# PoseLib/PoseLib

Measured on AMD Instinct MI355X. Metric: scored RANSAC hypotheses/sec (P3P@5k corrs, 5pt@5k corrs), higher is better.
Workload: dtype f64; 1 GPU; p3p_5000; correspondences=5000, problems_in_flight_per_gpu=128, distinct_scenes=64

## Files before the change

### __graft_entry__.py

```python
import os
import subprocess
import sys

ROOT = os.path.dirname(os.path.abspath(__file__))
sys.path.insert(0, ROOT)
sys.path.insert(0, os.path.join(ROOT, "tests"))


def build() -> None:
    import poselib_amd

    poselib_amd.build()
    assert os.path.exists(poselib_amd.LIB_PATH)
    subprocess.check_call(["make", "-C", os.path.join(ROOT, "oracle"), "-s", "liboracle.so"])
    subprocess.check_call(["make", "-C", os.path.join(ROOT, "tests", "hostmath"), "-s", "libhostmath.so"])
    subprocess.check_call(["make", "-C", os.path.join(ROOT, "tests", "hostmath_trig"), "-s", "libhostmath_trig.so"])
    subprocess.check_call(["make", "-C", os.path.join(ROOT, "tests", "hostmath_tangent"), "-s", "libhostmath_tangent.so"])
    subprocess.check_call(["make", "-C", os.path.join(ROOT, "tests", "hostmath_radial1d"), "-s", "libhostmath_radial1d.so"])
    if os.path.isdir("/root/reference/PoseLib"):
        subprocess.check_call(["make", "-C", os.path.join(ROOT, "oracle"), "-s", "-j8", "-f", "Makefile.ref"])
        subprocess.check_call(["make", "-C", os.path.join(ROOT, "oracle"), "-s", "-j8", "-f", "Makefile.ref", "VARIANT=fma"])
        import ref_lib

        subprocess.check_call(["make", "-C", os.path.join(ROOT, "oracle"), "-s", "-f", "Makefile.integration",
                               f"REF={ref_lib.REFERENCE_ROOT}"])
    from poselib_amd import _lib

    lib = _lib.lib()
    for sym in _lib.EXPORTED_SYMBOLS:
        getattr(lib, sym)


def smoke() -> None:
    import numpy as np

    import oracle_lib as O
    import poselib_amd as P
    from poselib_amd import synth

    d = synth.absolute_pose_scene(1500, 0.5, 4242)
    opt = {"ransac": {"seed": 3}}
    img, info = P.estimate_absolute_pose(d["p2d"], d["p3d"], d["camera"], opt)
    pose, mask, st = O.estimate_absolute_pose(d["p2d"], d["p3d"], d["camera"], opt)
    assert info["iterations"] == st["iterations"], (info["iterations"], st["iterations"])
    assert info["num_inliers"] == st["num_inliers"], (info["num_inliers"], st["num_inliers"])
    assert (np.array(info["inliers"]) == mask).all()
    got = np.r_[img.pose.q, img.pose.t]
    assert np.abs(got - pose).max() < 1e-6, np.abs(got - pose).max()
    print("smoke ok: iterations", info["iterations"], "inliers", info["num_inliers"], "max |pose diff|",
          float(np.abs(got - pose).max()))


if __name__ == "__main__":
    build()
    if len(sys.argv) > 1 and sys.argv[1] == "smoke":
        smoke()
```

### include/poselib_amd.h

```cpp
#ifndef POSELIB_AMD_H_
#define POSELIB_AMD_H_
#include <stddef.h>
#include <stdint.h>

#ifdef __cplusplus
extern "C" {
#endif

#define PL_OK 0
#define PL_ERR_NO_DEVICE (-1)
#define PL_ERR_HIP (-2)
#define PL_ERR_INVALID (-3)
#define PL_ERR_UNSUPPORTED (-4)
#define PL_ERR_COMM (-5)

typedef struct {
    uint64_t max_iterations;
    uint64_t min_iterations;
    double dyn_num_trials_mult;
    double success_prob;
    uint64_t seed;
    int32_t progressive_sampling;
    int32_t score_initial_model;
    uint64_t max_prosac_iterations;
// ... 82 lines not shown
                                  const pl_camera *camera1, const pl_camera *camera2, const pl_robust_options *opt,
                                  pl_camera_pose *pose, uint8_t *inliers, pl_ransac_stats *stats);
int pl_estimate_fundamental_dev(const pl_device_points *points2D_1, const pl_device_points *points2D_2, size_t n,
                                const pl_robust_options *opt, double *F , uint8_t *inliers,
                                pl_ransac_stats *stats);
int pl_estimate_homography_dev(const pl_device_points *points2D_1, const pl_device_points *points2D_2, size_t n,
                               const pl_robust_options *opt, double *H , uint8_t *inliers,
                               pl_ransac_stats *stats);
int pl_debug_check_device_points(const pl_device_points *d, size_t n, int cols);
int pl_debug_point_stats_dev(const pl_device_points *x1, const pl_device_points *x2, size_t n, int centroid, double *out);

int pl_undistort_points(const pl_camera *camera, const double *points2D, size_t n, double *out);

typedef struct {
    int32_t kind;
    int32_t status;
    const double *a;
    const double *b;
    size_t n;
    const pl_robust_options *opt;
    pl_camera *camera1;
    const pl_camera *camera2;
    void *model;
    uint8_t *inliers;
    pl_ransac_stats *stats;
} pl_batch_item;
int pl_estimate_batch(pl_batch_item *items, size_t count, int max_in_flight);
int pl_estimate_batch_devices(pl_batch_item *items, size_t count, const int *devices, int num_devices, int max_in_flight);
typedef struct {
    int32_t kind;
    int32_t status;
    pl_device_points a;
    pl_device_points b;
    size_t n;
    const pl_robust_options *opt;
    pl_camera *camera1;
    const pl_camera *camera2;
    void *model;
    uint8_t *inliers;
    pl_ransac_stats *stats;
} pl_batch_item_dev;
int pl_estimate_batch_dev(pl_batch_item_dev *items, size_t count, int max_in_flight);
int pl_debug_point_stats_group_dev(const pl_device_points *x1, const pl_device_points *x2, const size_t *n, size_t count, int centroid,
                                   double *out);
typedef struct {
    uint64_t items;
    uint64_t grouped;
    uint64_t focal_grouped;
    uint64_t solo;
    uint64_t fallback;
} pl_batch_report;
void pl_last_batch_report(pl_batch_report *out);

int pl_ransac_pnp(const double *x, const double *X, size_t n, const pl_robust_options *opt, pl_camera_pose *pose,
                  uint8_t *inliers, pl_ransac_stats *stats);
int pl_ransac_pnpf(const double *x, const double *X, size_t n, const pl_robust_options *opt, pl_camera_pose *pose, double *focal,
                   uint8_t *inliers, pl_ransac_stats *stats);
int pl_ransac_relpose(const double *x1, const double *x2, size_t n, const pl_robust_options *opt, pl_camera_pose *pose,
                      uint8_t *inliers, pl_ransac_stats *stats);
int pl_ransac_shared_focal_relpose(const double *x1, const double *x2, size_t n, const pl_robust_options *opt, pl_camera_pose *pose,
                                   double *focal, uint8_t *inliers, pl_ransac_stats *stats);
int pl_refine_shared_focal_relpose(const double *x1, const double *x2, size_t n, const pl_bundle_options *opt, pl_camera_pose *pose,
                                   double *focal, uint32_t *lm_iterations);

int pl_ransac_fundamental(const double *x1, const double *x2, size_t n, const pl_robust_options *opt, double *F,
                          uint8_t *inliers, pl_ransac_stats *stats);
int pl_ransac_homography(const double *x1, const double *x2, size_t n, const pl_robust_options *opt, double *H,
                         uint8_t *inliers, pl_ransac_stats *stats);
int pl_estimate_1D_radial_absolute_pose(const double *points2D, const double *points3D, size_t n, const pl_robust_options *opt,
                                        pl_camera_pose *pose, uint8_t *inliers, pl_ransac_stats *stats);
int pl_ransac_1D_radial_pnp(const double *x, const double *X, size_t n, const pl_robust_options *opt, pl_camera_pose *pose,
                            uint8_t *inliers, pl_ransac_stats *stats);

typedef struct pl_problem pl_problem;
int pl_problem_create(int kind, const double *a, const double *b, size_t n, pl_problem **out);
int pl_problem_create_tangent(const double *x1, const double *x2, size_t n, const pl_camera *camera1, const pl_camera *camera2,
                              pl_problem **out);
int pl_problem_create_dev(int kind, const pl_device_points *a, const pl_device_points *b, size_t n, pl_problem **out);
int pl_problem_create_tangent_dev(const pl_device_points *x1, const pl_device_points *x2, size_t n, const pl_camera *camera1,
                                  const pl_camera *camera2, pl_problem **out);
void pl_problem_destroy(pl_problem *p);
int pl_ransac_run(pl_problem *p, const pl_robust_options *opt, void *model, uint8_t *inliers, pl_ransac_stats *stats);

typedef struct {
    pl_problem *problem;
    const pl_robust_options *opt;
    void *model;
    uint8_t *inliers;
    pl_ransac_stats *stats;
    int32_t status;
    int32_t reserved;
} pl_ransac_item;
int pl_ransac_batch(pl_ransac_item *items, size_t count, int max_in_flight, int group_size);

typedef int (*pl_allgather_fn)(void *user, const void *send, void *recv, size_t bytes);
typedef struct pl_shard {
    int32_t rank, world;
    pl_allgather_fn allgather;
    void *user;
} pl_shard;
int pl_ransac_run_sharded(pl_problem *p, const pl_robust_options *opt, const pl_shard *shard, void *model,
                          uint8_t *inliers, pl_ransac_stats *stats);

int pl_score_model(pl_problem *p, const void *model, double max_error, uint64_t *inlier_count, double *score);
int pl_debug_inlier_mask(pl_problem *p, const void *model, double max_error, uint8_t *mask);
int pl_debug_tangent_chunk(void);
int pl_debug_radial1d_chunk(void);
int pl_debug_group_slices(int kind, uint32_t n_points, uint32_t iterations, uint32_t launch_chunks);
int pl_debug_radial1d_generate(pl_problem *p, const uint32_t *samples, size_t num_iters, uint32_t slots_per_iter, double *models,
                               uint32_t *num_models, uint32_t *totals);
int pl_debug_generate(pl_problem *p, const uint32_t *samples, uint64_t seed, uint64_t pos_base, const uint32_t *positions, size_t num_iters,
                      uint32_t slots_per_iter, int real_focal_check, int route, double *models, uint32_t *num_models, uint32_t *nan_bits,
                      uint32_t *blk_tot, uint32_t *blk_nan, uint32_t *flags);
int pl_debug_score_stream(pl_problem *p, const void *models, size_t n, double max_error, uint32_t *counts,
                          double *scores, int32_t *path_used);
int pl_debug_score_shape(int kind, uint32_t n_points, int matrix_core, int group_form, uint32_t *chunks,
                         uint32_t *points_per_lane);
typedef struct pl_debug_score_member {
    pl_problem *problem;
    const void *models;
    size_t n;
    double max_error;
    uint32_t *counts;
    double *scores;
    uint32_t slices;
    uint32_t slices_used;
    uint32_t chunks;
    int32_t path_used;
} pl_debug_score_member;
int pl_debug_score_stream_ex(int route, pl_debug_score_member *members, size_t num_members, uint32_t *idle_changed);
typedef struct pl_debug_prune_member {
    pl_problem *problem;
    const void *models;
    size_t n;
    double max_error;
    double init_min;
    uint32_t init_max;
    uint32_t cand_cap;
    uint32_t *counts;
    double *scores;
    uint8_t *kept;
    uint32_t *cand;
    uint32_t num_cand;
    uint32_t cstar, chunks, chunk_points;
    uint32_t lead;
    uint32_t lead_max;
    uint32_t num_live, num_selected;
    uint32_t slices, num_preselected;
    double lead_min;
} pl_debug_prune_member;
int pl_debug_score_pruned(int route, pl_debug_prune_member *members, size_t num_members, uint32_t *idle_changed);
int pl_debug_score_survivors(int route, pl_debug_prune_member *members, size_t num_members, uint32_t *const *survivors,
                             uint32_t *idle_changed, uint32_t *guard_changed);
int pl_debug_score_prune_gate(int kind, uint32_t n_points, uint32_t iterations);
typedef struct pl_debug_sampler_shape_info {
    uint64_t window;
    uint32_t build, tile;
    uint32_t small_flags, small_doubling, small_segments;
    uint32_t large_flags, large_doubling, large_segments;
} pl_debug_sampler_shape_info;
int pl_debug_sampler_shape(int K, uint64_t N, uint32_t B, uint64_t window, pl_debug_sampler_shape_info *out);
typedef struct pl_debug_sampler_member {
    uint64_t seed, pos_base, N;
    uint32_t B, M;
    const uint8_t *planted;
    uint32_t *positions;
    uint8_t *delta;
    uint64_t *flagbits;
    uint64_t pos_after;
    uint32_t orbit_error, M_used, build_used;
    int32_t delta_guard, ctl_clear, pad;
} pl_debug_sampler_member;
int pl_debug_sample_positions(int route, int K, int build, pl_debug_sampler_member *members, size_t num_members, uint32_t *idle_changed);
int pl_debug_device_math(int fn, const double *x, size_t n, double *out);
int pl_debug_device_math2(int fn, const double *x, const double *y, size_t n, double *out);
int pl_refine_model(pl_problem *p, const pl_bundle_options *opt, const pl_camera *camera, const uint8_t *mask,
                    void *model, uint32_t *lm_iterations);

int pl_bundle_adjust_camera(pl_problem *p, const pl_bundle_options *opt, pl_camera *camera, const uint8_t *mask,
                            pl_camera_pose *pose, uint32_t *lm_iterations);

int pl_p3p(const double *x , const double *X , pl_camera_pose *out );
int pl_p5lp_radial(const double *x , const double *X , pl_camera_pose *out , int *count );
int pl_relpose_5pt(const double *x1 , const double *x2 , pl_camera_pose *out );
int pl_essential_matrix_5pt(const double *x1, const double *x2, double *E );
int pl_relpose_7pt(const double *x1 , const double *x2 , double *F );
int pl_homography_4pt(const double *x1 , const double *x2 , double *H );
int pl_p35pf(const double *x, const double *X, pl_camera_pose *out, double *focals);
int pl_relpose_6pt_shared_focal(const double *x1, const double *x2, pl_camera_pose *out, double *focals);
int pl_solve_focal_batch(int kind, const double *in, size_t count, double *out_models, uint32_t *out_counts);
int pl_solve_batch(int kind, const double *in, size_t count, double *out_models, uint32_t *out_counts);

#ifdef __cplusplus
}
#endif
#endif
```

### poselib_amd/__init__.py

```python
from ._lib import LIB_PATH, PoseLibAmdError, build
from .api import (
    KIND_ABS, KIND_FUND, KIND_HOM, KIND_REL, KIND_RAD1D, estimate_1D_radial_absolute_pose, ransac_1D_radial_pnp, p5lp_radial, radial1d_generate, debug_generate, score_shape, score_stream_group, Batch, RansacBatch, ransac_batch, device_math, device_math2, BundleOptions, Camera, CameraPose, Image, Problem, TangentProblem, inlier_mask, RansacOptions,
    device_count, essential_matrix_5pt, estimate_absolute_pose, estimate_batch, last_batch_report, estimate_fundamental, estimate_homography,
    estimate_relative_pose, homography_4pt, p3p, p5p, ransac_fundamental, ransac_homography, ransac_pnp, ransac_pnpf,
    ransac_relpose, ransac_shared_focal_relpose, estimate_shared_focal_relative_pose, refine_shared_focal_relpose, ImagePair, p35pf, relpose_6pt_shared_focal, solve_focal_batch, relpose_5pt, relpose_7pt, set_device, set_lm_mode, solve_batch, undistort_points,
    check_device_points, point_stats_dev, point_stats_group_dev, score_pruned, score_survivors, score_prune_gate, sampler_shape, sample_positions,
)

__version__ = "0.1.0"
```

### poselib_amd/_lib.py

```python
from __future__ import annotations

import ctypes as C
import os
import subprocess

_PKG = os.path.dirname(os.path.abspath(__file__))
_CSRC = os.path.join(_PKG, "csrc")
LIB_PATH = os.path.join(_PKG, "lib", "libposelib_amd.so")
if os.environ.get("POSELIB_AMD_LIB"):
    LIB_PATH = os.environ["POSELIB_AMD_LIB"]

u64, i32, u32, f64 = C.c_uint64, C.c_int32, C.c_uint32, C.c_double

PL_OK, PL_ERR_NO_DEVICE, PL_ERR_HIP, PL_ERR_INVALID, PL_ERR_UNSUPPORTED, PL_ERR_COMM = 0, -1, -2, -3, -4, -5


class RansacOptions(C.Structure):
    _fields_ = [("max_iterations", u64), ("min_iterations", u64), ("dyn_num_trials_mult", f64), ("success_prob", f64),
                ("seed", u64), ("progressive_sampling", i32), ("score_initial_model", i32),
                ("max_prosac_iterations", u64)]


class BundleOptions(C.Structure):
    _fields_ = [("max_iterations", u64), ("loss_type", i32), ("lambda_update", i32), ("damping", i32), ("verbose", i32),
# ... 33 lines not shown

class BatchReport(C.Structure):
    _fields_ = [("items", C.c_uint64), ("grouped", C.c_uint64), ("focal_grouped", C.c_uint64), ("solo", C.c_uint64),
                ("fallback", C.c_uint64)]


class RansacItem(C.Structure):
    _fields_ = [("problem", C.c_void_p), ("opt", C.POINTER(RobustOptions)), ("model", C.c_void_p), ("inliers", C.c_void_p),
                ("stats", C.POINTER(RansacStats)), ("status", i32), ("reserved", i32)]


ALLGATHER_FN = C.CFUNCTYPE(C.c_int, C.c_void_p, C.c_void_p, C.c_void_p, C.c_size_t)


class Shard(C.Structure):
    _fields_ = [("rank", i32), ("world", i32), ("allgather", ALLGATHER_FN), ("user", C.c_void_p)]


class DebugScoreMember(C.Structure):
    _fields_ = [("problem", C.c_void_p), ("models", C.c_void_p), ("n", C.c_size_t), ("max_error", f64), ("counts", C.c_void_p),
                ("scores", C.c_void_p), ("slices", u32), ("slices_used", u32), ("chunks", u32), ("path_used", i32)]


class DebugPruneMember(C.Structure):
    _fields_ = [("problem", C.c_void_p), ("models", C.c_void_p), ("n", C.c_size_t), ("max_error", f64), ("init_min", f64),
                ("init_max", u32), ("cand_cap", u32), ("counts", C.c_void_p), ("scores", C.c_void_p), ("kept", C.c_void_p),
                ("cand", C.c_void_p), ("num_cand", u32), ("cstar", u32), ("chunks", u32), ("chunk_points", u32), ("lead", u32),
                ("lead_max", u32), ("num_live", u32), ("num_selected", u32), ("slices", u32), ("num_preselected", u32), ("lead_min", f64)]


class DebugSamplerShape(C.Structure):
    _fields_ = [("window", u64), ("build", u32), ("tile", u32), ("small_flags", u32), ("small_doubling", u32), ("small_segments", u32),
                ("large_flags", u32), ("large_doubling", u32), ("large_segments", u32)]


class DebugSamplerMember(C.Structure):
    _fields_ = [("seed", u64), ("pos_base", u64), ("N", u64), ("B", u32), ("M", u32), ("planted", C.c_void_p), ("positions", C.c_void_p),
                ("delta", C.c_void_p), ("flagbits", C.c_void_p), ("pos_after", u64), ("orbit_error", u32), ("M_used", u32),
                ("build_used", u32), ("delta_guard", i32), ("ctl_clear", i32), ("pad", i32)]


PL_F64, PL_F32 = 0, 1


class DevicePoints(C.Structure):
    _fields_ = [("data", C.c_void_p), ("row_stride", C.c_int64), ("dtype", i32), ("cols", i32)]


class BatchItemDev(C.Structure):
    _fields_ = [("kind", i32), ("status", i32), ("a", DevicePoints), ("b", DevicePoints), ("n", C.c_size_t),
                ("opt", C.POINTER(RobustOptions)), ("camera1", C.POINTER(Camera)), ("camera2", C.POINTER(Camera)),
                ("model", C.c_void_p), ("inliers", C.c_void_p), ("stats", C.POINTER(RansacStats))]


class PoseLibAmdError(RuntimeError):
    pass


def build(force: bool = False, verbose: bool = False) -> str:
    srcs = [os.path.join(_CSRC, f) for f in os.listdir(_CSRC) if f.endswith((".h", ".hip", ".cc", ".inc", "Makefile"))]
    srcs.append(os.path.join(os.path.dirname(_PKG), "include", "poselib_amd.h"))
    stale = (not os.path.exists(LIB_PATH)) or any(os.path.getmtime(s) > os.path.getmtime(LIB_PATH) for s in srcs)
    if force or stale:
        cmd = ["make", "-C", _CSRC]
        if not verbose:
            cmd.append("-s")
        subprocess.check_call(cmd)
    return LIB_PATH


_lib = None


def lib():
    global _lib
    if _lib is None:
        if not os.path.exists(LIB_PATH):
            raise PoseLibAmdError(
                f"{LIB_PATH} is missing: build it with `python -c 'import poselib_amd; poselib_amd.build()'` "
                "(there is no CPU fallback)")
        if not os.environ.get("POSELIB_AMD_KEEP_ENV"):
            os.environ.setdefault("GPU_MAX_HW_QUEUES", "16")
        L = C.CDLL(LIB_PATH)
        _declare(L)
        _lib = L
    return _lib


def _declare(L):
    vp, sz, dbl, cint = C.c_void_p, C.c_size_t, C.c_double, C.c_int
    P = C.POINTER
    opt, stats, cam, pose = P(RobustOptions), P(RansacStats), P(Camera), P(CameraPose)
    dpts = P(DevicePoints)
    sig = {
        "pl_default_ransac_options": (None, [P(RansacOptions)]),
        "pl_default_bundle_options": (None, [P(BundleOptions)]),
        "pl_default_robust_options": (None, [opt, cint]),
        "pl_device_count": (cint, []),
        "pl_set_lm_mode": (cint, [cint]),
        "pl_set_device": (cint, [cint]),
        "pl_last_error": (C.c_char_p, []),
        "pl_version": (C.c_char_p, []),
        "pl_abi_version": (cint, []),
        "pl_estimate_absolute_pose": (cint, [vp, vp, sz, opt, cam, pose, vp, stats]),
        "pl_estimate_relative_pose": (cint, [vp, vp, sz, cam, cam, opt, pose, vp, stats]),
        "pl_estimate_fundamental": (cint, [vp, vp, sz, opt, vp, vp, stats]),
        "pl_estimate_homography": (cint, [vp, vp, sz, opt, vp, vp, stats]),
        "pl_estimate_absolute_pose_dev": (cint, [dpts, dpts, sz, opt, cam, pose, vp, stats]),
        "pl_estimate_relative_pose_dev": (cint, [dpts, dpts, sz, cam, cam, opt, pose, vp, stats]),
        "pl_estimate_fundamental_dev": (cint, [dpts, dpts, sz, opt, vp, vp, stats]),
        "pl_estimate_homography_dev": (cint, [dpts, dpts, sz, opt, vp, vp, stats]),
        "pl_problem_create_dev": (cint, [cint, dpts, dpts, sz, P(vp)]),
        "pl_problem_create_tangent_dev": (cint, [dpts, dpts, sz, cam, cam, P(vp)]),
        "pl_debug_check_device_points": (cint, [dpts, sz, cint]),
        "pl_debug_point_stats_dev": (cint, [dpts, dpts, sz, cint, vp]),
        "pl_estimate_batch": (cint, [P(BatchItem), sz, cint]),
        "pl_estimate_batch_devices": (cint, [P(BatchItem), sz, P(C.c_int), cint, cint]),
        "pl_estimate_batch_dev": (cint, [P(BatchItemDev), sz, cint]),
        "pl_debug_point_stats_group_dev": (cint, [dpts, dpts, P(sz), sz, cint, vp]),
        "pl_last_batch_report": (None, [P(BatchReport)]),
        "pl_ransac_batch": (cint, [P(RansacItem), sz, cint, cint]),
        "pl_undistort_points": (cint, [cam, vp, sz, vp]),
        "pl_ransac_pnp": (cint, [vp, vp, sz, opt, pose, vp, stats]),
        "pl_ransac_pnpf": (cint, [vp, vp, sz, opt, pose, P(dbl), vp, stats]),
        "pl_ransac_relpose": (cint, [vp, vp, sz, opt, pose, vp, stats]),
        "pl_ransac_shared_focal_relpose": (cint, [vp, vp, sz, opt, pose, P(dbl), vp, stats]),
        "pl_solve_focal_batch": (cint, [cint, vp, sz, vp, vp]),
        "pl_p35pf": (cint, [vp, vp, vp, vp]),
        "pl_relpose_6pt_shared_focal": (cint, [vp, vp, vp, vp]),
        "pl_refine_shared_focal_relpose": (cint, [vp, vp, sz, P(BundleOptions), pose, P(dbl), P(C.c_uint32)]),
        "pl_estimate_shared_focal_relative_pose": (cint, [vp, vp, sz, vp, opt, pose, P(dbl), vp, stats]),
        "pl_ransac_fundamental": (cint, [vp, vp, sz, opt, vp, vp, stats]),
        "pl_ransac_homography": (cint, [vp, vp, sz, opt, vp, vp, stats]),
        "pl_problem_create": (cint, [cint, vp, vp, sz, P(vp)]),
        "pl_problem_create_tangent": (cint, [vp, vp, sz, cam, cam, P(vp)]),
        "pl_debug_inlier_mask": (cint, [vp, vp, dbl, vp]),
        "pl_debug_tangent_chunk": (cint, []),
        "pl_debug_radial1d_chunk": (cint, []),
        "pl_debug_group_slices": (cint, [cint, C.c_uint32, C.c_uint32, C.c_uint32]),
        "pl_debug_radial1d_generate": (cint, [vp, vp, sz, C.c_uint32, vp, vp, vp]),
        "pl_debug_generate": (cint, [vp, vp, u64, u64, vp, sz, C.c_uint32, cint, cint, vp, vp, vp, vp, vp, vp]),
        "pl_estimate_1D_radial_absolute_pose": (cint, [vp, vp, sz, opt, pose, vp, stats]),
        "pl_ransac_1D_radial_pnp": (cint, [vp, vp, sz, opt, pose, vp, stats]),
        "pl_p5lp_radial": (cint, [vp, vp, P(CameraPose), P(cint)]),
        "pl_problem_destroy": (None, [vp]),
        "pl_ransac_run": (cint, [vp, opt, vp, vp, stats]),
        "pl_ransac_run_sharded": (cint, [vp, opt, P(Shard), vp, vp, stats]),
        "pl_score_model": (cint, [vp, vp, dbl, P(C.c_uint64), P(dbl)]),
        "pl_debug_score_stream": (cint, [vp, vp, sz, dbl, vp, vp, P(C.c_int32)]),
        "pl_debug_score_shape": (cint, [cint, C.c_uint32, cint, cint, P(C.c_uint32), P(C.c_uint32)]),
        "pl_debug_score_stream_ex": (cint, [cint, P(DebugScoreMember), sz, P(C.c_uint32)]),
        "pl_debug_score_pruned": (cint, [cint, P(DebugPruneMember), sz, P(C.c_uint32)]),
        "pl_debug_score_survivors": (cint, [cint, P(DebugPruneMember), sz, P(C.c_void_p), P(C.c_uint32), P(C.c_uint32)]),
        "pl_debug_score_prune_gate": (cint, [cint, C.c_uint32, C.c_uint32]),
        "pl_debug_sampler_shape": (cint, [cint, u64, C.c_uint32, u64, P(DebugSamplerShape)]),
        "pl_debug_sample_positions": (cint, [cint, cint, cint, P(DebugSamplerMember), sz, P(C.c_uint32)]),
        "pl_debug_device_math": (cint, [cint, vp, sz, vp]),
        "pl_debug_device_math2": (cint, [cint, vp, vp, sz, vp]),
        "pl_refine_model": (cint, [vp, P(BundleOptions), cam, vp, vp, P(C.c_uint32)]),
        "pl_bundle_adjust_camera": (cint, [vp, P(BundleOptions), cam, vp, P(CameraPose), P(C.c_uint32)]),
        "pl_p3p": (cint, [vp, vp, P(CameraPose)]),
        "pl_relpose_5pt": (cint, [vp, vp, P(CameraPose)]),
        "pl_essential_matrix_5pt": (cint, [vp, vp, vp]),
        "pl_relpose_7pt": (cint, [vp, vp, vp]),
        "pl_homography_4pt": (cint, [vp, vp, vp]),
        "pl_solve_batch": (cint, [cint, vp, sz, vp, vp]),
    }
    missing = [name for name in EXPORTED_SYMBOLS if name not in sig]
    assert not missing, f"no signature declared for {missing}"
    for name, (res, args) in sig.items():
        fn = getattr(L, name)
        fn.restype = res
        fn.argtypes = args
    if L.pl_abi_version() != ABI_VERSION:
        raise PoseLibAmdError(f"{LIB_PATH} has record layout version {L.pl_abi_version()}, this binding was written for {ABI_VERSION}: rebuild")


def check(rc: int):
    if rc < 0:
        msg = lib().pl_last_error().decode()
        raise PoseLibAmdError(f"poselib_amd error {rc}: {msg}")
    return rc


ABI_VERSION = 5
EXPORTED_SYMBOLS = [
    "pl_default_ransac_options", "pl_default_bundle_options", "pl_default_robust_options", "pl_device_count",
    "pl_set_device", "pl_last_error", "pl_version", "pl_estimate_absolute_pose", "pl_estimate_relative_pose",
    "pl_estimate_fundamental", "pl_estimate_homography", "pl_ransac_pnp", "pl_ransac_relpose", "pl_ransac_fundamental",
    "pl_ransac_homography", "pl_problem_create", "pl_problem_destroy", "pl_ransac_run", "pl_ransac_run_sharded", "pl_score_model", "pl_debug_score_stream", "pl_refine_model", "pl_bundle_adjust_camera", "pl_p3p", "pl_relpose_5pt",
    "pl_essential_matrix_5pt", "pl_relpose_7pt", "pl_homography_4pt", "pl_solve_batch", "pl_estimate_batch", "pl_estimate_batch_devices", "pl_last_batch_report", "pl_undistort_points",
    "pl_ransac_batch", "pl_debug_device_math", "pl_debug_device_math2", "pl_ransac_pnpf", "pl_ransac_shared_focal_relpose", "pl_refine_shared_focal_relpose",
    "pl_estimate_shared_focal_relative_pose", "pl_solve_focal_batch", "pl_p35pf", "pl_relpose_6pt_shared_focal", "pl_set_lm_mode",
    "pl_abi_version", "pl_problem_create_tangent", "pl_debug_inlier_mask", "pl_debug_tangent_chunk",
    "pl_p5lp_radial", "pl_debug_radial1d_chunk", "pl_debug_radial1d_generate", "pl_debug_group_slices", "pl_debug_generate",
    "pl_debug_score_shape", "pl_debug_score_stream_ex", "pl_debug_score_pruned", "pl_debug_score_survivors", "pl_debug_score_prune_gate",
    "pl_estimate_absolute_pose_dev", "pl_estimate_relative_pose_dev", "pl_estimate_fundamental_dev", "pl_estimate_homography_dev",
    "pl_problem_create_dev", "pl_problem_create_tangent_dev", "pl_debug_check_device_points", "pl_debug_point_stats_dev",
    "pl_debug_sampler_shape", "pl_debug_sample_positions", "pl_estimate_batch_dev", "pl_debug_point_stats_group_dev",
]
```

### poselib_amd/api.py

```python
from __future__ import annotations

import ctypes as C
import sys
import threading

import numpy as np

from . import _lib as L

LAMBDA_UPDATES = {"NIELSEN": 0, "FIXED_FACTOR": 1}
DAMPINGS = {"LEVENBERG": 0, "MARQUARDT": 1}
LOSS_TYPES = {"TRIVIAL": 0, "TRUNCATED": 1, "HUBER": 2, "CAUCHY": 3, "TRUNCATED_CAUCHY": 4, "TRUNCATED_LE_ZACH": 5}
CAMERA_MODEL_IDS = {"NULL": -1, "SIMPLE_PINHOLE": 0, "PINHOLE": 1, "SIMPLE_RADIAL": 2, "RADIAL": 3, "OPENCV": 4,
                    "OPENCV_FISHEYE": 5, "SIMPLE_RADIAL_FISHEYE": 8, "RADIAL_FISHEYE": 9}
_CAMERA_NAMES = {v: k for k, v in CAMERA_MODEL_IDS.items()}
KIND_ABS, KIND_REL, KIND_FUND, KIND_HOM = 0, 1, 2, 3
KIND_SHARED_FOCAL = 4
KIND_RAD1D = 5
_POSE_KINDS = (KIND_ABS, KIND_REL, KIND_RAD1D)


class CameraPose:

    def __init__(self, q=None, t=None):
# ... 462 lines not shown

    def results(self, first=None):
        out = []
        for pr, o, model, inl, st in (self.keep if first is None else self.keep[:first]):
            if pr.kind in _POSE_KINDS:
                out.append((_pypose(model), _info(st, inl[: pr.n])))
            else:
                out.append((model.reshape(3, 3).T.copy(), _info(st, inl[: pr.n])))
        return out


def device_math(fn: int, x):
    x = np.ascontiguousarray(x, dtype=np.float64)
    out = np.zeros_like(x)
    L.check(L.lib().pl_debug_device_math(int(fn), _ptr(x), C.c_size_t(x.size), _ptr(out)))
    return out


def device_math2(fn: int, x, y=None):
    x = np.ascontiguousarray(x, dtype=np.float64)
    if y is not None:
        y = np.ascontiguousarray(y, dtype=np.float64)
        if y.shape != x.shape:
            raise ValueError("x and y differ in shape")
    out = np.zeros_like(x)
    L.check(L.lib().pl_debug_device_math2(int(fn), _ptr(x), None if y is None else _ptr(y), C.c_size_t(x.size), _ptr(out)))
    return out


def group_slices(kind: int, n_points: int, iterations: int, launch_chunks: int) -> int:
    return L.check(L.lib().pl_debug_group_slices(int(kind), int(n_points), int(iterations), int(launch_chunks)))


def score_shape(kind: int, n_points: int, matrix_core: bool, group_form: bool):
    chunks, per_lane = C.c_uint32(0), C.c_uint32(0)
    rc = L.lib().pl_debug_score_shape(int(kind), int(n_points), int(bool(matrix_core)), int(bool(group_form)), C.byref(chunks),
                                      C.byref(per_lane))
    if rc == L.PL_ERR_UNSUPPORTED:
        return None
    L.check(rc)
    return chunks.value, per_lane.value


def score_stream_group(members):
    arr = (L.DebugScoreMember * max(len(members), 1))()
    keep = []
    for i, (problem, models, max_error, slices) in enumerate(members):
        n, flat = problem._flat_models(models)
        cnt = np.zeros(max(n, 1), dtype=np.uint32)
        sc = np.zeros(max(n, 1), dtype=np.float64)
        keep.append((n, flat, cnt, sc))
        arr[i] = L.DebugScoreMember(problem._h, _ptr(flat), n, float(max_error), _ptr(cnt), _ptr(sc), int(slices), 0, 0, 0)
    idle = C.c_uint32(0)
    L.check(L.lib().pl_debug_score_stream_ex(2, arr, C.c_size_t(len(members)), C.byref(idle)))
    out = [{"counts": cnt[:n], "scores": sc[:n], "path": arr[i].path_used, "slices": arr[i].slices_used, "chunks": arr[i].chunks}
           for i, (n, _, cnt, sc) in enumerate(keep)]
    return out, idle.value


def sampler_shape(K: int, N: int, B: int, window: int = 0):
    s = L.DebugSamplerShape()
    L.check(L.lib().pl_debug_sampler_shape(int(K), int(N), int(B), int(window), C.byref(s)))
    return {"window": int(s.window), "build": "small" if s.build == 1 else "large", "tile": int(s.tile),
            "small": {"flags": s.small_flags, "doubling": s.small_doubling, "segments": s.small_segments},
            "large": {"flags": s.large_flags, "doubling": s.large_doubling, "segments": s.large_segments}}


_SAMPLER_BUILDS = {None: 0, "small": 1, "large": 2}


def sample_positions(K: int, members, build=None, group: bool = False):
    arr = (L.DebugSamplerMember * max(len(members), 1))()
    keep = []
    for i, m in enumerate(members):
        planted = m.get("planted")
        if planted is not None:
            planted = np.ascontiguousarray(planted, dtype=np.uint8)
            M = int(planted.size)
            if m.get("M", 0) not in (0, M):
                raise ValueError("a planted table has M bytes")
        else:
            M = int(m.get("M", 0)) or sampler_shape(K, m["N"], m["B"])["window"]
        pos = np.zeros(max(int(m["B"]), 1), dtype=np.uint32)
        cap = M if M < (1 << 31) else 0
        delta = np.zeros(cap + 1, dtype=np.uint8)
        bits = np.zeros(cap // 64 + 2, dtype=np.uint64)
        keep.append((planted, pos, delta, bits))
        arr[i] = L.DebugSamplerMember(int(m.get("seed", 0)), int(m.get("pos_base", 0)), int(m["N"]), int(m["B"]), M,
                                      None if planted is None else _ptr(planted), _ptr(pos), _ptr(delta), _ptr(bits))
    idle = C.c_uint32(0)
    L.check(L.lib().pl_debug_sample_positions(2 if group else 0, int(K), _SAMPLER_BUILDS[build], arr, C.c_size_t(len(members)),
                                              C.byref(idle)))
    out = []
    for i, (_, pos, delta, bits) in enumerate(keep):
        a = arr[i]
        words = (a.M_used + 63) // 64
        out.append({"positions": pos, "delta": delta[:a.M_used], "flagbits": bits[:words], "guard": bits[words:a.M_used // 64 + 2],
                    "pos_after": int(a.pos_after), "orbit_error": int(a.orbit_error), "M": int(a.M_used),
                    "build": "small" if a.build_used == 1 else "large", "delta_guard": bool(a.delta_guard),
                    "ctl_clear": bool(a.ctl_clear)})
    return out, idle.value


def score_prune_gate(kind: int, n_points: int, iterations: int) -> bool:
    return bool(L.check(L.lib().pl_debug_score_prune_gate(int(kind), int(n_points), int(iterations))))


def score_pruned(members, route=0):
    arr = (L.DebugPruneMember * max(len(members), 1))()
    keep = []
    cap = 4096
    for i, (problem, models, max_error, init_max, init_min) in enumerate(members):
        n, flat = problem._flat_models(models)
        cnt = np.zeros(max(n, 1), dtype=np.uint32)
        sc = np.zeros(max(n, 1), dtype=np.float64)
        kp = np.zeros(max(n, 1), dtype=np.uint8)
        cand = np.zeros(cap, dtype=np.uint32)
        keep.append((n, flat, cnt, sc, kp, cand))
        arr[i] = L.DebugPruneMember(problem._h, _ptr(flat), n, float(max_error), float(init_min), int(init_max), cap, _ptr(cnt),
                                    _ptr(sc), _ptr(kp), _ptr(cand))
    idle = C.c_uint32(0)
    L.check(L.lib().pl_debug_score_pruned(int(route), arr, C.c_size_t(len(members)), C.byref(idle)))
    out = []
    for i, (n, _, cnt, sc, kp, cand) in enumerate(keep):
        a = arr[i]
        out.append({"counts": cnt[:n], "scores": sc[:n], "kept": kp[:n].astype(bool), "cand": cand[:min(a.num_cand, cap)].copy(),
                    "num_cand": a.num_cand, "cstar": a.cstar, "chunks": a.chunks, "chunk_points": a.chunk_points, "lead": a.lead,
                    "lead_max": a.lead_max, "lead_min": a.lead_min, "num_live": a.num_live, "num_selected": a.num_selected, "num_preselected": a.num_preselected,
                    "slices": a.slices})
    return out, idle.value


def score_survivors(members, route=0):
    arr = (L.DebugPruneMember * max(len(members), 1))()
    outs = (C.c_void_p * max(len(members), 1))()
    keep = []
    for i, (problem, models, max_error) in enumerate(members):
        n, flat = problem._flat_models(models)
        chunks = score_shape(problem.kind, problem.n, True, route == 2)[0]
        sv = np.zeros((chunks, max(n, 1)), dtype=np.uint32)
        keep.append((n, flat, sv))
        arr[i] = L.DebugPruneMember(problem._h, _ptr(flat), n, float(max_error))
        outs[i] = sv.ctypes.data
    idle, guard = C.c_uint32(0), C.c_uint32(0)
    L.check(L.lib().pl_debug_score_survivors(int(route), arr, C.c_size_t(len(members)), outs, C.byref(idle), C.byref(guard)))
    out = []
    for i, (n, _, sv) in enumerate(keep):
        a = arr[i]
        assert a.chunks == sv.shape[0], (a.chunks, sv.shape)
        out.append({"survivors": sv[:, :n], "chunks": a.chunks, "chunk_points": a.chunk_points, "num_live": a.num_live, "slices": a.slices})
    return out, idle.value, guard.value


def ransac_batch(problems, opts, max_in_flight=4, group_size=16):
    b = RansacBatch(problems, opts)
    b.run(max_in_flight, group_size)
    return b.results()


def estimate_fundamental(points2D_1, points2D_2, opt=None, initial_F=None):
    return _estimate_matrix("pl_estimate_fundamental", KIND_FUND, points2D_1, points2D_2, opt, initial_F)


def estimate_homography(points2D_1, points2D_2, opt=None, initial_H=None):
    return _estimate_matrix("pl_estimate_homography", KIND_HOM, points2D_1, points2D_2, opt, initial_H)


def _ransac(fn, kind, a, b, dim_b, opt, initial):
    a, b = _pts(a, 2), _pts(b, dim_b)
    o = _robust_options(opt, kind, initial is not None)
    n = a.shape[0]
    inl = np.zeros(max(n, 1), dtype=np.uint8)
    st = L.RansacStats()
    if kind in _POSE_KINDS:
        pose = _cpose(initial if initial is not None else CameraPose())
        L.check(getattr(L.lib(), fn)(_ptr(a), _ptr(b), C.c_size_t(n), C.byref(o), C.byref(pose), _ptr(inl), C.byref(st)))
        return _pypose(pose), _info(st, inl[:n])
    M = np.ascontiguousarray((np.eye(3) if initial is None else np.asarray(initial, dtype=np.float64)).T.reshape(9))
    L.check(getattr(L.lib(), fn)(_ptr(a), _ptr(b), C.c_size_t(n), C.byref(o), _ptr(M), _ptr(inl), C.byref(st)))
    return M.reshape(3, 3).T.copy(), _info(st, inl[:n])


def ransac_pnp(x, X, opt=None, initial_pose=None):
    return _ransac("pl_ransac_pnp", KIND_ABS, x, X, 3, opt, initial_pose)


def ransac_1D_radial_pnp(x, X, opt=None, initial_pose=None):
    return _ransac("pl_ransac_1D_radial_pnp", KIND_RAD1D, x, X, 3, opt, initial_pose)


def estimate_1D_radial_absolute_pose(points2D, points3D, opt=None, initial_pose=None):
    return _ransac("pl_estimate_1D_radial_absolute_pose", KIND_RAD1D, points2D, points3D, 3, opt, initial_pose)


def ransac_pnpf(x, X, opt=None):
    x, X = _pts(x, 2), _pts(X, 3)
    o = _robust_options(opt, KIND_ABS, False)
    n = x.shape[0]
    inl = np.zeros(max(n, 1), dtype=np.uint8)
    st = L.RansacStats()
    pose = _cpose(CameraPose())
    focal = C.c_double(1.0)
    L.check(L.lib().pl_ransac_pnpf(_ptr(x), _ptr(X), C.c_size_t(n), C.byref(o), C.byref(pose), C.byref(focal), _ptr(inl), C.byref(st)))
    return Image(_pypose(pose), Camera("SIMPLE_PINHOLE", [focal.value, 0.0, 0.0])), _info(st, inl[:n])


class ImagePair:

    def __init__(self, pose=None, camera1=None, camera2=None):
        self.pose = pose or CameraPose()
        self.camera1 = camera1 or Camera("SIMPLE_PINHOLE", [1.0, 0.0, 0.0])
        self.camera2 = camera2 or Camera("SIMPLE_PINHOLE", list(self.camera1.params))


def _shared_focal_pair(pose, focal, pp):
    return ImagePair(_pypose(pose), Camera("SIMPLE_PINHOLE", [focal, pp[0], pp[1]]), Camera("SIMPLE_PINHOLE", [focal, pp[0], pp[1]]))


def ransac_shared_focal_relpose(x1, x2, opt=None, initial_pair=None):
    x1, x2 = _pts(x1, 2), _pts(x2, 2)
    o = _robust_options(opt, KIND_REL, initial_pair is not None)
    n = x1.shape[0]
    inl = np.zeros(max(n, 1), dtype=np.uint8)
    st = L.RansacStats()
    pose = _cpose(initial_pair.pose if initial_pair is not None else CameraPose())
    focal = C.c_double(initial_pair.camera1.focal() if initial_pair is not None else 1.0)
    L.check(L.lib().pl_ransac_shared_focal_relpose(_ptr(x1), _ptr(x2), C.c_size_t(n), C.byref(o), C.byref(pose), C.byref(focal),
                                                   _ptr(inl), C.byref(st)))
    return _shared_focal_pair(pose, focal.value, (0.0, 0.0)), _info(st, inl[:n])


def estimate_shared_focal_relative_pose(points2D_1, points2D_2, pp, opt=None, initial_pair=None):
    x1, x2 = _pts(points2D_1, 2), _pts(points2D_2, 2)
    o = _robust_options(opt, KIND_REL, initial_pair is not None)
    n = x1.shape[0]
    inl = np.zeros(max(n, 1), dtype=np.uint8)
    st = L.RansacStats()
    pose = _cpose(initial_pair.pose if initial_pair is not None else CameraPose())
    focal = C.c_double(initial_pair.camera1.focal() if initial_pair is not None else 1.0)
    ppa = np.ascontiguousarray(pp, dtype=np.float64)
    L.check(L.lib().pl_estimate_shared_focal_relative_pose(_ptr(x1), _ptr(x2), C.c_size_t(n), _ptr(ppa), C.byref(o), C.byref(pose),
                                                           C.byref(focal), _ptr(inl), C.byref(st)))
    return _shared_focal_pair(pose, focal.value, ppa), _info(st, inl[:n])


def refine_shared_focal_relpose(x1, x2, pair, bundle=None):
    x1, x2 = _pts(x1, 2), _pts(x2, 2)
    o = _robust_options({"bundle": bundle or {}}, KIND_REL, False)
    pose = _cpose(pair.pose)
    focal = C.c_double(pair.camera1.focal())
    its = C.c_uint32(0)
    L.check(L.lib().pl_refine_shared_focal_relpose(_ptr(x1), _ptr(x2), C.c_size_t(x1.shape[0]), C.byref(o.bundle), C.byref(pose),
                                                   C.byref(focal), C.byref(its)))
    return _shared_focal_pair(pose, focal.value, (0.0, 0.0)), its.value


def solve_focal_batch(kind, inputs):
    k = {"p35pf": 0, "relpose_6pt_shared_focal": 1}[kind]
    a = np.ascontiguousarray(inputs, dtype=np.float64)
    per, slots = (20, 10) if k == 0 else (36, 60)
    if a.ndim != 2 or a.shape[1] != per:
        raise ValueError(f"expected a (count, {per}) array")
    models = np.zeros((a.shape[0], slots, 8))
    counts = np.zeros(max(a.shape[0], 1), dtype=np.uint32)
    L.check(L.lib().pl_solve_focal_batch(C.c_int(k), _ptr(a), C.c_size_t(a.shape[0]), _ptr(models), _ptr(counts)))
    return models, counts[: a.shape[0]]


def p35pf(x, X):
    models, counts = solve_focal_batch("p35pf", np.r_[_pts(x, 2).reshape(-1), _pts(X, 3).reshape(-1)][None, :])
    return [(CameraPose(m[:4], m[4:7]), float(m[7])) for m in models[0, : counts[0]]]


def relpose_6pt_shared_focal(x1, x2):
    models, counts = solve_focal_batch("relpose_6pt_shared_focal", np.r_[_pts(x1, 3).reshape(-1), _pts(x2, 3).reshape(-1)][None, :])
    return [(CameraPose(m[:4], m[4:7]), float(m[7])) for m in models[0, : counts[0]]]


def ransac_relpose(x1, x2, opt=None, initial_pose=None):
    return _ransac("pl_ransac_relpose", KIND_REL, x1, x2, 2, opt, initial_pose)


def ransac_fundamental(x1, x2, opt=None, initial_F=None):
    return _ransac("pl_ransac_fundamental", KIND_FUND, x1, x2, 2, opt, initial_F)


def ransac_homography(x1, x2, opt=None, initial_H=None):
    return _ransac("pl_ransac_homography", KIND_HOM, x1, x2, 2, opt, initial_H)


class Problem:

    def __init__(self, kind: int, a, b):
        self.kind = kind
        pts = _Points(a, b, 2, 3 if kind in (KIND_ABS, KIND_RAD1D) else 2)
        self.n = pts.n
        self._h = C.c_void_p()
        L.check(pts.fn("pl_problem_create")(kind, pts.a, pts.b, C.c_size_t(self.n), C.byref(self._h)))

    def run(self, opt=None, initial=None):
        o = _robust_options(opt, self.kind, initial is not None)
        inl = np.zeros(max(self.n, 1), dtype=np.uint8)
        st = L.RansacStats()
        if self.kind in _POSE_KINDS:
            model = _cpose(initial if initial is not None else CameraPose())
            L.check(L.lib().pl_ransac_run(self._h, C.byref(o), C.byref(model), _ptr(inl), C.byref(st)))
# ... 289 lines not shown
```

### poselib_amd/csrc/driver.cc

```cpp
#include "../../include/poselib_amd.h"
#include "pl_focal.h"
#include "pl_kernels.h"
#include "pl_refine_cam.h"
#include "pl_sfocal.h"
#include "pl_solver_6ptf.h"
#include "pl_solver_p35pf.h"
#include "pl_sampler.h"
#include "pl_svd3.h"

#include <algorithm>
#include <atomic>
#include <chrono>
#include <condition_variable>
#include <cmath>
#include <cstdio>
#include <cstdlib>
#include <cstring>
#include <functional>
#include <limits>
#include <mutex>
#include <string>
#include <thread>
#include <vector>

// ... 442 lines not shown
    double *models, *compact64, *part_score, *score, *rec_models;
    uint32_t *part_count, *count;
    RecordMeta *rec_meta;
    char *shadow16, *points16, *blk_best, *gen_stage;
    uint32_t *prune_sel;
    uint8_t *prune_kept;
    char *prune_state;
    RecordMeta *host_meta;
    double *host_models;
    BatchCtl *host_ctl;
};
uint32_t batch_blocks(uint32_t Bl) { return (Bl + 1023) / 1024; }
size_t batch_ctl_bytes(uint32_t Bl, uint32_t chunks) {
    static_assert(sizeof(BatchCtl) % 4 == 0, "zeroed as 32-bit words");
    return sizeof(BatchCtl) + sizeof(uint32_t) * (2 * (size_t)batch_blocks(Bl) + 2 + chunks);
}
constexpr size_t kPruneTilesOffset = 256;
static_assert(sizeof(PruneState) <= kPruneTilesOffset, "prune_state layout");
constexpr size_t kBlkMinOffset = 1024;

BatchSizes batch_step_sizes(int kind, const BatchShape &s) {
    const size_t iters = std::max<uint32_t>(s.Bl, 1u), hcap = iters * s.slots;
    const bool abs16 = s.use_mfma && kind == EST_ABS;
    BatchSizes z;
    z.positions = sizeof(uint32_t) * s.B;
    z.delta = (size_t)s.M + 64;
    z.flags = sizeof(uint64_t) * ((size_t)s.M / 64 + 2);
    z.samples = sizeof(uint32_t) * (size_t)s.B * sample_size(kind);
    z.models = sizeof(double) * kModelStride * hcap;
    z.num_models = sizeof(uint32_t) * iters;
    z.nan_bits = abs16 ? sizeof(uint32_t) * iters : 0;
    z.slots = sizeof(uint32_t) * hcap;
    z.offsets = sizeof(uint32_t) * iters;
    z.ctl = batch_ctl_bytes(s.Bl, s.chunks);
    z.shadow = sizeof(float) * 16 * hcap;
    z.compact64 = sizeof(double) * kModelDoubles * hcap;
    z.shadow16 = !s.use_mfma        ? 0
                 : kind == EST_ABS ? (hcap + kAbs16Pad) * kAbs16Bytes
                 : kind == EST_HOM ? (hcap + kHom16Pad) * kHom16Bytes
                                   : (hcap + kSampson16Pad) * kSampson16Bytes;
    z.live = z.rank = abs16 ? sizeof(uint32_t) * hcap : 0;
    z.points16 = abs16 ? kAbs16PointBytes * s.point_rows : 0;
    z.part_count = sizeof(uint32_t) * s.chunks * hcap;
    z.part_score = sizeof(double) * s.chunks * hcap;
    z.count = sizeof(uint32_t) * hcap;
    z.score = sizeof(double) * hcap;
    z.blk_best = kBlkMinOffset + sizeof(double) * 256;
    z.rec_meta = sizeof(RecordMeta) * kRecordCap;
    z.rec_models = sizeof(double) * kModelStride * kRecordCap;
    z.gen_stage = generate_stage_bytes(kind, s.Bl);
    z.prune_sel = abs16 ? sizeof(uint32_t) * hcap : 0;
    z.prune_kept = abs16 ? hcap : 0;
    z.prune_state = abs16 ? kPruneTilesOffset + sizeof(uint32_t) * ((hcap + 1023) / 1024) : 0;
    return z;
}

struct BatchRun {
    int kind;
    PointSet pts;
    uint64_t seed, pos;
    double thr2;
    PrefilterArgs pf;
    uint32_t init_max;
    double init_min;
    int32_t real_focal_check;
    bool explicit_samples;
};

void wire_batch_step(GroupArgs &a, const BatchRun &r, const BatchShape &s, const BatchBuffers &b) {
    std::memset(&a, 0, sizeof(a));
    const size_t hcap = (size_t)std::max<uint32_t>(s.Bl, 1u) * s.slots;
    const uint32_t nblk = batch_blocks(s.Bl);
    uint32_t *const blk_tot = reinterpret_cast<uint32_t *>(b.ctl + 1);
    const bool live_list = s.use_mfma && r.kind == EST_ABS;
    a.active = 1;
    a.use_mfma = s.use_mfma ? 1u : 0u;
    a.chunks = s.chunks;
    a.samp.seed = r.seed, a.samp.pos_base = r.pos, a.samp.N = r.pts.n, a.samp.B = s.B, a.samp.M = s.M;
    a.samp.delta = b.delta;
    a.samp.flagbits = b.flags;
    a.samp.positions = b.positions;
    a.samp.ctl = b.ctl;
    a.samp.zero_words = (uint32_t)(batch_ctl_bytes(s.Bl, s.chunks) / 4);
    GenerateArgs &ga = a.gen;
    ga.pts = r.pts;
    ga.seed = r.seed;
    ga.pos_base = r.pos;
    ga.positions = b.positions + s.lo;
    ga.samples = r.explicit_samples ? b.samples : nullptr;
    ga.num_iters = s.Bl;
    ga.slots_per_iter = s.slots;
    ga.ctl = b.ctl;
    ga.models = b.models;
    ga.num_models = b.num_models;
    ga.real_focal_check = r.real_focal_check;
    ga.blk_tot = blk_tot;
    ga.blk_nan = blk_tot + nblk;
    ga.nan_bits = live_list ? b.nan_bits : nullptr;
    ga.stage = generate_stage_bytes(r.kind, s.Bl) ? b.gen_stage : nullptr;
    CompactArgs &ca = a.comp;
    ca.num_models = b.num_models;
    ca.B = s.Bl;
    ca.maxm = (int32_t)s.slots;
    ca.blk_tot = blk_tot;
    ca.slots = b.slots;
    ca.offsets = b.offsets;
    ca.models = b.models;
    ca.shadow = b.shadow;
    ca.compact64 = b.compact64;
    ca.ctl = b.ctl;
    if (live_list) {
        ca.s16.out = b.shadow16;
        ca.s16.g16 = r.pf.g16, ca.s16.c16 = r.pf.c16, ca.s16.thr = r.pf.thr;
        ca.s16.live = b.live, ca.s16.rank = b.rank, ca.s16.nan_bits = ga.nan_bits;
        ca.s16.points16 = b.points16, ca.s16.point_rows = s.point_rows;
    } else if (s.use_mfma && r.kind == EST_HOM) {
        ca.s16.out = b.shadow16;
        ca.s16.sampson = 2;
        ca.s16.thr = r.pf.h16;
    } else if (s.use_mfma) {
        ca.s16.out = b.shadow16;
        ca.s16.sampson = 1;
    }
    ca.host_offsets = nullptr;
    ScoreArgs &sa = a.score;
    sa.pts = r.pts;
    sa.models = b.models;
    sa.slots = b.slots;
    sa.shadow = b.shadow;
    sa.compact64 = b.compact64;
    sa.shadow16 = ca.s16.out;
    sa.num_hyp = &b.ctl->num_hyp;
    if (live_list) {
        sa.slots = b.live;
        sa.num_hyp = &b.ctl->num_live;
        sa.points16 = b.points16;
    }
    sa.hyp_capacity = (uint32_t)hcap;
    sa.thr2 = r.thr2;
    sa.pf = r.pf;
    sa.part_count = b.part_count;
    sa.part_score = b.part_score;
    sa.tickets = blk_tot + 2 * (size_t)nblk + 2;
    if (s.prune && live_list) {
        PruneArgs &pa = sa.prune;
        pa.st = reinterpret_cast<PruneState *>(b.prune_state);
        pa.blk_kept = reinterpret_cast<uint32_t *>(b.prune_state + kPruneTilesOffset);
        pa.sel = b.prune_sel;
        pa.kept = b.prune_kept;
        pa.chunks = s.chunks;
        pa.chunk_points = s.point_rows / s.chunks;
        pa.init_max = r.init_max, pa.init_min = r.init_min;
        pa.lead = kPruneLead;
    }
    RecordsArgs &ra = a.rec;
    ra.f.num_hyp = &b.ctl->num_hyp;
    ra.f.rank = ca.s16.rank;
    ra.f.hyp_capacity = (uint32_t)hcap;
    ra.f.chunks = s.chunks;
    ra.f.n_points = r.pts.n;
    ra.f.thr2 = r.thr2;
    ra.f.part_count = b.part_count;
    ra.f.part_score = b.part_score;
    ra.f.count = b.count;
    ra.f.score = b.score;
    ra.f.kept = sa.prune.kept;
    ra.slots = b.slots;
    ra.models = b.models;
    ra.blk_max = reinterpret_cast<uint32_t *>(b.blk_best);
    ra.blk_min = reinterpret_cast<double *>(b.blk_best + kBlkMinOffset);
    ra.init_max = r.init_max;
    ra.init_min = r.init_min;
    ra.rec_meta = b.rec_meta;
    ra.rec_models = b.rec_models;
    ra.rec_cap = kRecordCap;
    ra.ctl = b.ctl;
    ra.host_meta = b.host_meta;
    ra.host_models = b.host_models;
    ra.host_cap = kRecordFirst;
    SeqScoreArgs &qa = a.seq;
    qa.pts = r.pts;
    qa.models = b.models;
    qa.cand = b.rec_meta;
    qa.num = &b.ctl->num_records;
    qa.cap = kRecordCap;
    qa.thr2 = r.thr2;
    qa.host_cand = b.host_meta;
    qa.host_cap = kRecordFirst;
    qa.ctl_src = b.ctl;
    qa.ctl_host = b.host_ctl;
}

void group_dims_sampler(GroupDims &d, uint32_t M, uint32_t n, uint32_t B) {
    d.max_M = std::max(d.max_M, M);
    d.min_n = std::min(d.min_n, n);
    d.max_B = std::max(d.max_B, B);
}

int context_batch_buffers(Context *c, const BatchSizes &z, BatchBuffers &b) {
    auto grown = [](DevBuf &d, size_t bytes, auto *&ptr) {
        const hipError_t e = d.ensure(bytes);
        ptr = static_cast<std::remove_reference_t<decltype(ptr)>>(d.p);
        return e;
    };
    HIP_TRY(grown(c->positions, z.positions, b.positions));
    HIP_TRY(grown(c->delta, z.delta, b.delta));
    HIP_TRY(grown(c->flags, z.flags, b.flags));
    HIP_TRY(grown(c->samples, z.samples, b.samples));
    HIP_TRY(grown(c->models, z.models, b.models));
    HIP_TRY(grown(c->num_models, z.num_models, b.num_models));
    HIP_TRY(grown(c->nan_bits, z.nan_bits, b.nan_bits));
    HIP_TRY(grown(c->slots, z.slots, b.slots));
    HIP_TRY(grown(c->offsets, z.offsets, b.offsets));
    HIP_TRY(grown(c->ctl, z.ctl, b.ctl));
    HIP_TRY(grown(c->shadow, z.shadow, b.shadow));
    HIP_TRY(grown(c->compact64, z.compact64, b.compact64));
    HIP_TRY(grown(c->shadow16, z.shadow16, b.shadow16));
    HIP_TRY(grown(c->live, z.live, b.live));
    HIP_TRY(grown(c->rank, z.rank, b.rank));
    HIP_TRY(grown(c->points16, z.points16, b.points16));
    HIP_TRY(grown(c->part_count, z.part_count, b.part_count));
    HIP_TRY(grown(c->part_score, z.part_score, b.part_score));
    HIP_TRY(grown(c->count, z.count, b.count));
    HIP_TRY(grown(c->score, z.score, b.score));
    HIP_TRY(grown(c->blk_best, z.blk_best, b.blk_best));
    HIP_TRY(grown(c->rec_meta, z.rec_meta, b.rec_meta));
    HIP_TRY(grown(c->rec_models, z.rec_models, b.rec_models));
    HIP_TRY(grown(c->gen_stage, z.gen_stage, b.gen_stage));
    HIP_TRY(grown(c->prune_sel, z.prune_sel, b.prune_sel));
    HIP_TRY(grown(c->prune_kept, z.prune_kept, b.prune_kept));
    HIP_TRY(grown(c->prune_state, z.prune_state, b.prune_state));
    HIP_TRY(c->h_small.ensure(sizeof(BatchCtl) + 64));
    HIP_TRY(c->h_rec_meta.ensure(sizeof(RecordMeta) * kRecordCap));
    HIP_TRY(c->h_gather_out.ensure(sizeof(double) * kModelStride * kRecordCap));
    b.host_meta = c->h_rec_meta.dev<RecordMeta>();
    b.host_models = c->h_gather_out.dev<double>();
    b.host_ctl = c->h_small.dev<BatchCtl>();
    return PL_OK;
}

struct RefineJob {
    double record_in[kModelStride];
    LMOptions opt;
    CameraParams cam;
    double point_scale = 1.0;
    double prefilter_thr2 = 0.0;
    const uint8_t *d_mask = nullptr;
    int cam_flags = 0;
    CameraParams cam_out;
    double record_out[kModelStride];
    double params_out[kParamDoubles];
    uint32_t count = 0;
    double score = 0;
    bool skipped = false;
};

struct MaskTail {
    double incumbent_score;
    const double *incumbent_rec;
    double thr2;
    uint8_t *host_mask;
};

int run_refinements(Context *c, const pl_problem *p, std::vector<RefineJob> &jobs, bool rescore, double thr2,
                    const MaskTail *tail = nullptr) {
    const uint32_t nj = (uint32_t)jobs.size();
    if (nj == 0)
        return PL_OK;
    static_assert(sizeof(LMTask) % sizeof(double) == 0, "records follow the tasks");
    const size_t stage_bytes = sizeof(LMTask) * nj + sizeof(double) * kModelStride * (nj + 1);
    HIP_TRY(c->h_tasks.ensure(stage_bytes));
    HIP_TRY(c->lm_scratch.ensure((size_t)p->n * nj + 16));
    HIP_TRY(c->lm_records.ensure(sizeof(double) * kModelStride * nj));
    static const bool latency_mode = [] {
        const char *e = std::getenv("POSELIB_AMD_LATENCY_MODE");
        return e && e[0] == '1';
    }();
    uint32_t max_it = 0;
    bool same_it = true;
    for (uint32_t j = 0; j < nj; ++j) {
        same_it = same_it && (j == 0 || jobs[j].opt.max_iterations == max_it);
        max_it = std::max(max_it, jobs[j].opt.max_iterations);
    }
    const uint32_t lm2_min_points = (p->kind == EST_ABS) ? 8192u : 2560u;
    bool with_camera = false;
    for (uint32_t j = 0; j < nj; ++j)
        with_camera = with_camera || jobs[j].cam_flags != 0;
    if (with_camera && p->kind != EST_ABS)
        return fail(PL_ERR_INVALID, "camera intrinsics are refined with absolute poses only");
    const bool use_lm2 = !with_camera && latency_mode && p->kind != EST_REL && p->kind != EST_RELT && p->kind != EST_RAD1D && !lm_sums_ordered(p->kind) && same_it && max_it >= 1 && max_it <= 32 && p->n >= lm2_min_points;
    if (use_lm2)
        HIP_TRY(c->lm_tasks.ensure(stage_bytes));
    LMTask *ht = c->h_tasks.as<LMTask>();
    double *hr = reinterpret_cast<double *>(ht + nj);
    LMTask *d_tasks = use_lm2 ? c->lm_tasks.as<LMTask>() : c->h_tasks.dev<LMTask>();
    double *d_records_in = reinterpret_cast<double *>(d_tasks + nj);
    for (uint32_t j = 0; j < nj; ++j) {
        LMTask &t = ht[j];
        std::memset(&t, 0, sizeof(t));
        t.pts = p->ps;
        lm_params_from_record(p->kind, jobs[j].record_in, t.params);
        t.opt = jobs[j].opt;
        t.cam = jobs[j].cam;
        t.point_scale = jobs[j].point_scale;
        t.cam_flags = jobs[j].cam_flags;
        t.prefilter_thr2 = jobs[j].prefilter_thr2;
// ... 1688 lines not shown
    const BatchSizes z = batch_step_sizes(p->kind, s);
    BatchBuffers bb;
    rc = context_batch_buffers(c, z, bb);
    if (rc != PL_OK)
        return rc;
    bb.nan_bits = nullptr;
    GroupArgs a;
    wire_batch_step(a, run, s, bb);
    rc = debug_score_prepare(c, p, a, bb, z, recs, ident, H);
    if (rc != PL_OK)
        return rc;
    const int path = a.comp.s16.out ? 2 : (run.pf.enabled ? 1 : 0);
    const uint32_t per = (uint32_t)kStreamWaves * 64u / (uint32_t)kScoreThreads;
    const uint32_t slices = slices_in ? slices_in * per : std::max<uint32_t>(1u, std::min<uint32_t>(1536u / s.chunks, H));
    HIP_TRY(launch_score(p->kind, a.score, slices, c->stream));
    HIP_TRY(launch_finalize(a.rec.f, c->stream));
    if (counts)
        HIP_TRY(hipMemcpyAsync(counts, c->count.p, sizeof(uint32_t) * H, hipMemcpyDeviceToHost, c->stream));
    if (scores)
        HIP_TRY(hipMemcpyAsync(scores, c->score.p, sizeof(double) * H, hipMemcpyDeviceToHost, c->stream));
    HIP_TRY(wait_stream(c));
    if (path_used)
        *path_used = path;
    if (slices_used)
        *slices_used = std::max<uint32_t>(1u, slices / per);
    if (chunks_used)
        *chunks_used = chunks;
    return PL_OK;
}
constexpr size_t kDebugScoreMembers = 4;
int debug_score_group(pl_debug_score_member *m, size_t count, uint32_t *idle_changed) {
    if (!m || count == 0 || count > kDebugScoreMembers)
        return fail(PL_ERR_INVALID, "the group form takes 1 .. 4 members");
    for (size_t i = 0; i < count; ++i) {
        if (!m[i].problem || !m[i].models || m[i].n == 0 || m[i].n > (1u << 22) || m[i].problem->n == 0)
            return fail(PL_ERR_INVALID, "member: problem / models missing, no correspondences, or n outside 1 .. 2^22");
        if (m[i].problem->kind != m[0].problem->kind)
            return fail(PL_ERR_INVALID, "the members of a group are of one kind");
    }
    const int kind = m[0].problem->kind;
    if (kind != EST_ABS && kind != EST_REL && kind != EST_FUND && kind != EST_HOM)
        return fail(PL_ERR_INVALID, "tangent and 1D-radial problems have no group form");
    Context *c;
    int rc = get_context(&c);
    if (rc != PL_OK)
        return rc;
    for (size_t i = 0; i < count; ++i)
        if (m[i].problem->device != c->device)
            return fail(PL_ERR_INVALID, "problem lives on another device than the calling thread's");
    struct Slot {
        BatchRun run{};
        BatchShape s{};
        BatchSizes z{};
        BatchBuffers b{};
        size_t bytes = 0;
        char *arena = nullptr;
        ~Slot() {
            if (arena)
                (void)hipFree(arena);
        }
    } slot[1 + kDebugScoreMembers];
    struct Scratch {
        void *p = nullptr;
        ~Scratch() {
            if (p)
                (void)hipFree(p);
        }
    } dtable;
    GroupArgs ha[1 + kDebugScoreMembers];
    GroupDims dims{};
    dims.G = (uint32_t)count + 1;
    dims.P = group_points_per_lane(kind);
    uint32_t launch_chunks = 0;
    for (size_t i = 0; i < count; ++i) {
        Slot &t = slot[i + 1];
        const pl_problem *p = m[i].problem;
        t.run.kind = kind;
        t.run.pts = p->ps;
        t.run.thr2 = m[i].max_error * m[i].max_error;
        t.run.pf = problem_prefilter(p, t.run.thr2);
        t.run.init_max = 0xffffffffu;
        t.s.Bl = (uint32_t)m[i].n, t.s.slots = 1;
        t.s.use_mfma = score_uses_mfma(kind, p->n, t.run.pf);
        t.s.chunks = group_member_chunks(kind, t.s.use_mfma, p->n);
        t.s.point_rows = t.s.chunks * 64u * (uint32_t)dims.P;
        if (m[i].slices > score_slice_limit(kind, t.s.chunks, false))
            return fail(PL_ERR_INVALID, "slices beyond what the scorer's launch takes for this member");
        t.z = batch_step_sizes(kind, t.s);
        if (t.s.use_mfma)
            launch_chunks += t.s.chunks;
    }
    slot[0].run = slot[1].run, slot[0].s = slot[1].s, slot[0].z = slot[1].z;
    for (size_t k = 0; k <= count; ++k) {
        Slot &t = slot[k];
        BatchBuffers unused;
        t.bytes = pack_batch_buffers(nullptr, t.z, unused);
        HIP_TRY(hipMalloc((void **)&t.arena, t.bytes));
        HIP_TRY(hipMemsetAsync(t.arena, k == 0 ? 0xa5 : 0, t.bytes, c->stream));
        pack_batch_buffers(t.arena, t.z, t.b);
        t.b.nan_bits = nullptr;
        t.b.host_meta = nullptr, t.b.host_models = nullptr, t.b.host_ctl = nullptr;
        wire_batch_step(ha[k], t.run, t.s, t.b);
    }
    ha[0].active = 0;
    for (size_t i = 0; i < count; ++i) {
        GroupArgs &a = ha[i + 1];
        const Slot &t = slot[i + 1];
        const uint32_t H = t.s.Bl;
        a.slices = m[i].slices ? m[i].slices
                               : group_score_slices(kind, t.s.use_mfma, group_expected_hypotheses(kind, H, H), H, t.s.chunks, launch_chunks);
        dims.max_B = std::max(dims.max_B, H);
        dims.max_hcap = std::max(dims.max_hcap, a.score.hyp_capacity);
        dims.max_chunks = std::max(dims.max_chunks, a.chunks);
        dims.max_slices = std::max(dims.max_slices, a.slices);
        dims.any_mfma |= a.use_mfma;
        dims.any_queue |= a.use_mfma ? 0u : 1u;
        std::vector<double> recs;
        std::vector<uint32_t> ident(H);
        for (uint32_t k = 0; k < H; ++k)
            ident[k] = k;
        debug_score_records(m[i].problem, m[i].models, H, recs);
        rc = debug_score_prepare(c, m[i].problem, a, t.b, t.z, recs, ident, H);
        if (rc != PL_OK)
            return rc;
        HIP_TRY(hipStreamSynchronize(c->stream));
    }
    ha[0].slices = ha[1].slices;
    HIP_TRY(hipMalloc(&dtable.p, sizeof(GroupArgs) * dims.G));
    HIP_TRY(hipMemcpyAsync(dtable.p, ha, sizeof(GroupArgs) * dims.G, hipMemcpyHostToDevice, c->stream));
    HIP_TRY(launch_group_score(kind, static_cast<const GroupArgs *>(dtable.p), dims, c->stream));
    HIP_TRY(launch_group_finalize_records(static_cast<const GroupArgs *>(dtable.p), dims, c->stream));
    for (size_t i = 0; i < count; ++i) {
        const Slot &t = slot[i + 1];
        if (m[i].counts)
            HIP_TRY(hipMemcpyAsync(m[i].counts, t.b.count, sizeof(uint32_t) * t.s.Bl, hipMemcpyDeviceToHost, c->stream));
        if (m[i].scores)
            HIP_TRY(hipMemcpyAsync(m[i].scores, t.b.score, sizeof(double) * t.s.Bl, hipMemcpyDeviceToHost, c->stream));
    }
    std::vector<uint32_t> idle(slot[0].bytes / 4);
    HIP_TRY(hipMemcpyAsync(idle.data(), slot[0].arena, idle.size() * 4, hipMemcpyDeviceToHost, c->stream));
    HIP_TRY(wait_stream(c));
    uint32_t changed = 0;
    for (uint32_t w : idle)
        changed += w != 0xa5a5a5a5u ? 1u : 0u;
    if (idle_changed)
        *idle_changed = changed;
    for (size_t i = 0; i < count; ++i) {
        m[i].path_used = ha[i + 1].comp.s16.out ? 2 : (slot[i + 1].run.pf.enabled ? 1 : 0);
        m[i].slices_used = ha[i + 1].slices;
        m[i].chunks = ha[i + 1].chunks;
    }
    return PL_OK;
}
int debug_score_pruned(int route, pl_debug_prune_member *m, size_t count, uint32_t *idle_changed, uint32_t *const *survivors = nullptr,
                       uint32_t *guard_changed = nullptr) {
    if (route != 0 && route != 2)
        return fail(PL_ERR_INVALID, "route: 0 single launch, 2 group form");
    if (!m || count == 0 || count > (route == 0 ? 1 : kDebugScoreMembers))
        return fail(PL_ERR_INVALID, "the single launch takes one member, the group form 1 .. 4");
    for (size_t i = 0; i < count; ++i) {
        if (!m[i].problem || !m[i].models || m[i].n == 0 || m[i].n > (1u << 22) || m[i].problem->n == 0)
            return fail(PL_ERR_INVALID, "member: problem / models missing, no correspondences, or n outside 1 .. 2^22");
        if (m[i].problem->kind != EST_ABS)
            return fail(PL_ERR_INVALID, "the pruned scorer is the absolute-pose one");
        if (m[i].cand_cap && !m[i].cand)
            return fail(PL_ERR_INVALID, "member: cand_cap without cand");
    }
    Context *c;
    int rc = get_context(&c);
    if (rc != PL_OK)
        return rc;
    for (size_t i = 0; i < count; ++i)
        if (m[i].problem->device != c->device)
            return fail(PL_ERR_INVALID, "problem lives on another device than the calling thread's");
    struct Slot {
        BatchRun run{};
        BatchShape s{};
        BatchSizes z{};
        BatchBuffers b{};
        size_t bytes = 0;
        char *arena = nullptr;
        ~Slot() {
            if (arena)
                (void)hipFree(arena);
        }
    } slot[1 + kDebugScoreMembers];
    struct Scratch {
        void *p = nullptr;
        ~Scratch() {
            if (p)
                (void)hipFree(p);
        }
    } dtable;
    GroupArgs ha[1 + kDebugScoreMembers];
    GroupDims dims{};
    dims.G = (uint32_t)count + 1;
    dims.P = group_points_per_lane(EST_ABS);
    uint32_t launch_chunks = 0;
    for (size_t i = 0; i < count; ++i) {
        Slot &t = slot[i + 1];
        const pl_problem *p = m[i].problem;
        t.run.kind = EST_ABS;
        t.run.pts = p->ps;
        t.run.thr2 = m[i].max_error * m[i].max_error;
        t.run.pf = problem_prefilter(p, t.run.thr2);
        t.run.init_max = m[i].init_max;
        t.run.init_min = m[i].init_min;
        t.s.Bl = (uint32_t)m[i].n, t.s.slots = 1;
        t.s.use_mfma = score_uses_mfma(EST_ABS, p->n, t.run.pf);
        if (!t.s.use_mfma)
            return fail(PL_ERR_UNSUPPORTED, "member: not scored on the matrix cores (size, threshold or coordinates out of range)");
        if (route == 0) {
            t.s.chunks = score_chunks(EST_ABS, p->n, true, true);
            t.s.point_rows = abs16_point_rows(p->n);
        } else {
            t.s.chunks = group_member_chunks(EST_ABS, true, p->n);
            t.s.point_rows = t.s.chunks * 64u * (uint32_t)dims.P;
        }
        t.s.prune = true;
        t.z = batch_step_sizes(EST_ABS, t.s);
        launch_chunks += t.s.chunks;
    }
    slot[0].run = slot[1].run, slot[0].s = slot[1].s, slot[0].z = slot[1].z;
    for (size_t k = (route == 0 ? 1 : 0); k <= count; ++k) {
        Slot &t = slot[k];
        BatchBuffers unused;
        t.bytes = pack_batch_buffers(nullptr, t.z, unused);
        HIP_TRY(hipMalloc((void **)&t.arena, t.bytes));
        HIP_TRY(hipMemsetAsync(t.arena, k == 0 ? 0xa5 : 0, t.bytes, c->stream));
        pack_batch_buffers(t.arena, t.z, t.b);
        t.b.nan_bits = nullptr;
        t.b.host_meta = nullptr, t.b.host_models = nullptr, t.b.host_ctl = nullptr;
        wire_batch_step(ha[k], t.run, t.s, t.b);
    }
    ha[0].active = 0;
    for (size_t i = 0; i < count; ++i) {
        GroupArgs &a = ha[i + 1];
        const Slot &t = slot[i + 1];
        const uint32_t H = t.s.Bl;
        a.slices = group_score_slices(EST_ABS, true, group_expected_hypotheses(EST_ABS, H, H), H, t.s.chunks, launch_chunks);
        dims.max_B = std::max(dims.max_B, H);
        dims.max_hcap = std::max(dims.max_hcap, a.score.hyp_capacity);
        dims.max_chunks = std::max(dims.max_chunks, a.chunks);
        dims.max_slices = std::max(dims.max_slices, a.slices);
        dims.any_mfma = dims.any_prune = 1;
        std::vector<double> recs;
        std::vector<uint32_t> ident(H);
        for (uint32_t k = 0; k < H; ++k)
            ident[k] = k;
        debug_score_records(m[i].problem, m[i].models, H, recs);
        rc = debug_score_prepare(c, m[i].problem, a, t.b, t.z, recs, ident, H);
        if (rc != PL_OK)
            return rc;
        HIP_TRY(hipStreamSynchronize(c->stream));
    }
    uint32_t single_slices = 0;
    if (route == 0) {
        const GroupArgs &a = ha[1];
        const uint32_t slices = std::max<uint32_t>(1u, std::min<uint32_t>(1536u / a.chunks, a.score.hyp_capacity));
        single_slices = std::max<uint32_t>(1u, std::min<uint32_t>(slices * (uint32_t)kScoreThreads / (64u * (uint32_t)kStreamWaves),
                                                                  score_slice_limit(EST_ABS, a.chunks, true)));
        if (survivors) {
            HIP_TRY(launch_score_count(a.score, slices, c->stream));
        } else {
            HIP_TRY(launch_score_pruned(a.score, slices, c->stream));
            HIP_TRY(launch_prune_label(a.score, c->stream));
            HIP_TRY(launch_finalize_records(a.rec, c->stream));
        }
    } else {
        ha[0].slices = ha[1].slices;
        HIP_TRY(hipMalloc(&dtable.p, sizeof(GroupArgs) * dims.G));
        HIP_TRY(hipMemcpyAsync(dtable.p, ha, sizeof(GroupArgs) * dims.G, hipMemcpyHostToDevice, c->stream));
        if (survivors) {
            HIP_TRY(launch_group_score_count(static_cast<const GroupArgs *>(dtable.p), dims, c->stream));
        } else {
            HIP_TRY(launch_group_score(EST_ABS, static_cast<const GroupArgs *>(dtable.p), dims, c->stream));
            for (size_t i = 0; i < count; ++i)
                HIP_TRY(launch_prune_label(ha[i + 1].score, c->stream));
            HIP_TRY(launch_group_finalize_records(static_cast<const GroupArgs *>(dtable.p), dims, c->stream));
        }
    }
    std::vector<std::vector<uint32_t>> part(count);
    std::vector<std::vector<uint32_t>> rank(count);
    std::vector<std::vector<uint8_t>> kept(count);
    std::vector<std::vector<RecordMeta>> meta(count);
    std::vector<PruneState> st(count);
    std::vector<BatchCtl> ctl(count);
    for (size_t i = 0; i < count; ++i) {
        const Slot &t = slot[i + 1];
        const uint32_t H = t.s.Bl;
        if (m[i].counts && !survivors)
            HIP_TRY(hipMemcpyAsync(m[i].counts, t.b.count, sizeof(uint32_t) * H, hipMemcpyDeviceToHost, c->stream));
        if (m[i].scores && !survivors)
            HIP_TRY(hipMemcpyAsync(m[i].scores, t.b.score, sizeof(double) * H, hipMemcpyDeviceToHost, c->stream));
        rank[i].resize(H), kept[i].resize(H), meta[i].resize(kRecordCap);
        HIP_TRY(hipMemcpyAsync(rank[i].data(), t.b.rank, sizeof(uint32_t) * H, hipMemcpyDeviceToHost, c->stream));
        HIP_TRY(hipMemcpyAsync(kept[i].data(), t.b.prune_kept, H, hipMemcpyDeviceToHost, c->stream));
        HIP_TRY(hipMemcpyAsync(meta[i].data(), t.b.rec_meta, sizeof(RecordMeta) * kRecordCap, hipMemcpyDeviceToHost, c->stream));
        HIP_TRY(hipMemcpyAsync(&st[i], t.b.prune_state, sizeof(PruneState), hipMemcpyDeviceToHost, c->stream));
        HIP_TRY(hipMemcpyAsync(&ctl[i], t.b.ctl, sizeof(BatchCtl), hipMemcpyDeviceToHost, c->stream));
        if (survivors) {
            part[i].resize((size_t)t.s.chunks * ha[i + 1].score.hyp_capacity);
            HIP_TRY(hipMemcpyAsync(part[i].data(), t.b.part_count, sizeof(uint32_t) * part[i].size(), hipMemcpyDeviceToHost, c->stream));
        }
    }
    std::vector<uint32_t> idle(route == 2 ? slot[0].bytes / 4 : 0);
    if (!idle.empty())
        HIP_TRY(hipMemcpyAsync(idle.data(), slot[0].arena, idle.size() * 4, hipMemcpyDeviceToHost, c->stream));
    HIP_TRY(wait_stream(c));
    uint32_t changed = 0;
    for (uint32_t w : idle)
        changed += w != 0xa5a5a5a5u ? 1u : 0u;
    if (idle_changed)
        *idle_changed = changed;
    uint32_t guard = 0;
    for (size_t i = 0; i < count; ++i) {
        const uint32_t H = slot[i + 1].s.Bl, chunks = slot[i + 1].s.chunks;
        m[i].chunks = chunks;
        m[i].chunk_points = slot[i + 1].s.point_rows / chunks;
        m[i].num_live = ctl[i].num_live;
        m[i].slices = route == 0 ? single_slices : ha[i + 1].slices;
        if (survivors) {
            const uint32_t hcap = ha[i + 1].score.hyp_capacity;
            for (uint32_t ch = 0; ch < chunks; ++ch) {
                for (uint32_t k = 0; k < H; ++k)
                    survivors[i][(size_t)ch * H + k] = rank[i][k] == kNoRank ? 0u : part[i][(size_t)ch * hcap + rank[i][k]];
                for (uint32_t p = ctl[i].num_live; p < hcap; ++p)
                    guard += part[i][(size_t)ch * hcap + p] != 0xffffffffu ? 1u : 0u;
            }
            continue;
        }
        const bool split = st[i].cstar < chunks;
        uint32_t selected = 0;
        for (uint32_t k = 0; k < H; ++k) {
            const bool live = rank[i][k] != kNoRank;
            const bool kp = !split || !live || kept[i][rank[i][k]] == kKept;
            selected += (split && live && kp) ? 1u : 0u;
            if (m[i].kept)
                m[i].kept[k] = kp ? 1 : 0;
        }
        m[i].num_cand = ctl[i].num_records;
        for (uint32_t r = 0; r < std::min<uint32_t>({ctl[i].num_records, m[i].cand_cap, kRecordCap}); ++r)
            m[i].cand[r] = meta[i][r].k;
        m[i].cstar = st[i].cstar;
        m[i].lead = kPruneLead;
        m[i].lead_max = st[i].lead_max;
        m[i].lead_min = st[i].lead_min;
        m[i].num_selected = selected;
        m[i].num_preselected = st[i].sel_len;
    }
    if (guard_changed)
        *guard_changed = guard;
    return PL_OK;
}
}
int pl_debug_score_pruned(int route, pl_debug_prune_member *members, size_t num_members, uint32_t *idle_changed) {
    if (idle_changed)
        *idle_changed = 0;
    return debug_score_pruned(route, members, num_members, idle_changed);
}
int pl_debug_score_survivors(int route, pl_debug_prune_member *members, size_t num_members, uint32_t *const *survivors,
                             uint32_t *idle_changed, uint32_t *guard_changed) {
    if (idle_changed)
        *idle_changed = 0;
    if (guard_changed)
        *guard_changed = 0;
    if (!survivors)
        return fail(PL_ERR_INVALID, "pl_debug_score_survivors: survivors missing");
    for (size_t i = 0; i < num_members; ++i)
        if (!survivors[i])
            return fail(PL_ERR_INVALID, "pl_debug_score_survivors: a member without an output array");
    return debug_score_pruned(route, members, num_members, idle_changed, survivors, guard_changed);
}
int pl_debug_score_prune_gate(int kind, uint32_t n_points, uint32_t iterations) {
    PrefilterArgs pf{};
    pf.enabled = 1;
    pf.g16 = pf.t16 = pf.h16 = 1.0f, pf.thr = 1.0f;
    if (n_points == 0)
        return fail(PL_ERR_INVALID, "pl_debug_score_prune_gate: n_points > 0");
    const bool mfma = score_uses_mfma(kind, n_points, pf);
    return score_prune_gate(kind, mfma, iterations, kind == EST_ABS ? score_chunks(kind, n_points, true, mfma) : 1u) ? 1 : 0;
}
int pl_debug_score_stream(pl_problem *p, const void *models, size_t n, double max_error, uint32_t *counts,
                          double *scores, int32_t *path_used) {
    return debug_score_single(p, models, n, max_error, 0, counts, scores, path_used, nullptr, nullptr);
}
int pl_debug_score_stream_ex(int route, pl_debug_score_member *members, size_t num_members, uint32_t *idle_changed) {
    if (idle_changed)
        *idle_changed = 0;
    if (route != 0 && route != 2)
        return fail(PL_ERR_INVALID, "route: 0 single launch, 2 group form");
    if (route == 2)
        return debug_score_group(members, num_members, idle_changed);
    if (!members || num_members != 1)
        return fail(PL_ERR_INVALID, "the single launch takes one member");
    pl_debug_score_member &m = members[0];
    return debug_score_single(m.problem, m.models, m.n, m.max_error, m.slices, m.counts, m.scores, &m.path_used, &m.slices_used, &m.chunks);
}
int pl_debug_score_shape(int kind, uint32_t n_points, int matrix_core, int group_form, uint32_t *chunks, uint32_t *points_per_lane) {
    const bool four = kind == EST_ABS || kind == EST_REL || kind == EST_FUND || kind == EST_HOM;
    if (!(four || kind == EST_RELT || kind == EST_RAD1D) || n_points == 0 || !chunks || !points_per_lane)
        return fail(PL_ERR_INVALID, "pl_debug_score_shape: kind 0 .. 5, n_points > 0, output pointers");
    if (!four && (matrix_core || group_form))
        return fail(PL_ERR_INVALID, "tangent and 1D-radial problems have neither a matrix-core nor a group form");
    if (matrix_core) {
        PrefilterArgs pf{};
        pf.enabled = 1;
        pf.g16 = pf.t16 = pf.h16 = 1.0f, pf.thr = 1.0f;
        if (!score_uses_mfma(kind, n_points, pf))
            return fail(PL_ERR_UNSUPPORTED, "no problem of this kind and size is scored on the matrix cores");
    }
    if (group_form) {
        *chunks = group_member_chunks(kind, matrix_core != 0, n_points);
        *points_per_lane = (uint32_t)((matrix_core && (kind == EST_REL || kind == EST_FUND)) ? group_mfma2_points_per_lane(kind)
                                                                                           : group_points_per_lane(kind));
    } else {
        *chunks = score_chunks(kind, n_points, true, matrix_core != 0);
        *points_per_lane = (uint32_t)score_points_per_lane(kind, n_points, true, matrix_core != 0);
    }
    return PL_OK;
}

int pl_debug_sampler_shape(int K, uint64_t N, uint32_t B, uint64_t window, pl_debug_sampler_shape_info *out) {
    if ((K != 3 && K != 4 && K != 5 && K != 7) || N < (uint64_t)K || N > 0xffffffffull || B == 0 || !out)
        return fail(PL_ERR_INVALID, "pl_debug_sampler_shape: K in {3, 4, 5, 7}, K <= N < 2^32, B > 0, output pointer");
    const uint64_t M = window ? window : sampler_window((uint32_t)N, K, B);
    const OrbitShape sm = orbit_build_shape(true), lg = orbit_build_shape(false);
    out->window = M;
    out->build = (M <= 0xffffffffull && orbit_small_build((uint32_t)M, N, K)) ? 1u : 2u;
    out->tile = sm.tile;
    out->small_flags = sm.flags, out->small_doubling = sm.doubling, out->small_segments = sm.segments;
    out->large_flags = lg.flags, out->large_doubling = lg.doubling, out->large_segments = lg.segments;
    return PL_OK;
}
int pl_debug_sample_positions(int route, int K, int build, pl_debug_sampler_member *m, size_t count, uint32_t *idle_changed) {
    if (idle_changed)
        *idle_changed = 0;
    if (route != 0 && route != 2)
        return fail(PL_ERR_INVALID, "route: 0 single launches, 2 group form");
    if (build < 0 || build > 2)
        return fail(PL_ERR_INVALID, "build: 0 the launcher's choice, 1 small, 2 large");
    if (K != 3 && K != 4 && K != 5 && K != 7)
        return fail(PL_ERR_INVALID, "K: 3, 4, 5 or 7");
    constexpr size_t kMembers = 4;
    if (!m || count == 0 || count > kMembers)
        return fail(PL_ERR_INVALID, "1 .. 4 members");
    const int kind = K == 3 ? EST_ABS : K == 5 ? EST_REL : K == 7 ? EST_FUND : EST_HOM;
    uint64_t window[kMembers];
    for (size_t i = 0; i < count; ++i) {
        if (m[i].N < (uint64_t)K || m[i].N > 0xffffffffull || m[i].B == 0 || m[i].B > (1u << 20) || !m[i].positions)
            return fail(PL_ERR_INVALID, "member: K <= N < 2^32, B in 1 .. 2^20, positions");
        window[i] = m[i].M ? m[i].M : sampler_window((uint32_t)m[i].N, K, m[i].B);
        if (window[i] > 0x7fffffffull || m[i].pos_base + window[i] >= 0xffffffffull || m[i].pos_base >= 0xffffffffull)
            return fail(PL_ERR_INVALID, "member: a window beyond 2^31 - 1 positions, or one that ends at or beyond draw 2^32 - 1");
        if (route == 2 && (m[i].planted != nullptr) != (m[0].planted != nullptr))
            return fail(PL_ERR_INVALID, "a group is drawn or planted as a whole");
    }
    Context *c;
    int rc = get_context(&c);
    if (rc != PL_OK)
        return rc;
    struct Slot {
        BatchRun run{};
        BatchShape s{};
        BatchSizes z{};
        BatchBuffers b{};
        size_t bytes = 0;
        char *arena = nullptr;
        ~Slot() {
            if (arena)
                (void)hipFree(arena);
        }
    } slot[1 + kMembers];
    struct Scratch {
        void *p = nullptr;
        ~Scratch() {
            if (p)
                (void)hipFree(p);
        }
    } dtable;
    GroupArgs ha[1 + kMembers];
    GroupDims dims{};
    dims.G = (uint32_t)count + 1;
    dims.min_n = 0xffffffffu;
    for (size_t i = 0; i < count; ++i) {
        Slot &t = slot[i + 1];
        t.run.kind = kind;
        t.run.pts.n = (uint32_t)m[i].N;
        t.run.seed = m[i].seed, t.run.pos = m[i].pos_base;
        t.s.B = t.s.Bl = m[i].B, t.s.M = (uint32_t)window[i], t.s.slots = 1, t.s.chunks = 1;
        const BatchSizes full = batch_step_sizes(kind, t.s);
        t.z.positions = full.positions, t.z.delta = full.delta, t.z.flags = full.flags, t.z.ctl = full.ctl;
    }
    slot[0].run = slot[1].run, slot[0].s = slot[1].s, slot[0].z = slot[1].z;
    std::vector<uint64_t> bits;
    for (size_t k = (route == 0 ? 1 : 0); k <= count; ++k) {
        Slot &t = slot[k];
        BatchBuffers unused;
        t.bytes = pack_batch_buffers(nullptr, t.z, unused);
        t.bytes += 256;
        HIP_TRY(hipMalloc((void **)&t.arena, t.bytes));
        HIP_TRY(hipMemsetAsync(t.arena, 0xa5, t.bytes, c->stream));
        pack_batch_buffers(t.arena, t.z, t.b);
        t.b.host_meta = nullptr, t.b.host_models = nullptr, t.b.host_ctl = nullptr;
        wire_batch_step(ha[k], t.run, t.s, t.b);
        if (k == 0)
            continue;
        const pl_debug_sampler_member &mi = m[k - 1];
        group_dims_sampler(dims, t.s.M, t.run.pts.n, t.s.B);
        HIP_TRY(hipMemsetAsync(t.b.positions, 0xff, t.z.positions, c->stream));
        if (mi.planted) {
            const uint32_t M = t.s.M, words = (M + 63u) / 64u;
            bits.assign(words, 0ull);
            for (uint32_t p = 0; p < M; ++p)
                if (mi.planted[p] != (uint8_t)K)
                    bits[p >> 6] |= 1ull << (p & 63u);
            HIP_TRY(hipMemcpyAsync(t.b.delta, mi.planted, M, hipMemcpyHostToDevice, c->stream));
            HIP_TRY(hipMemcpyAsync(t.b.flags, bits.data(), sizeof(uint64_t) * words, hipMemcpyHostToDevice, c->stream));
            HIP_TRY(hipMemsetAsync(t.b.ctl, 0, t.z.ctl, c->stream));
            HIP_TRY(hipStreamSynchronize(c->stream));
        }
    }
    const bool planted = m[0].planted != nullptr;
    uint32_t build_used[1 + kMembers] = {};
    if (route == 0) {
// ... 953 lines not shown
```

### poselib_amd/csrc/driver_group.inc

```

constexpr uint32_t kGroupMax = 128;
constexpr uint32_t kGroupMaxAuto = 256;
constexpr uint32_t kGroupMaxPoints = 16384;

struct GroupLayout {
    BatchSizes batch;
    size_t pts, pts2, mask, tmp_model, absmax, total;
};

struct GroupContext {
    int device = -1;
    size_t budget = 0;
    int budget_threads = 0;
    DevBuf arena, raw, args, lm_records, lm_scratch, seq_count, seq_score, sel_count;
    HostBuf h_raw, h_args, h_ctl, h_meta, h_recm, h_offsets, h_mask, h_tasks, h_count, h_score, h_tail;
    HostBuf h_samples, h_absmax;
    HostBuf h_raw_alt, h_prep_args;
    HostBuf h_ingest, h_pstats_args, h_pstats;
    const void *staged_first = nullptr;
    void release() {
        for (DevBuf *b : {&arena, &raw, &args, &lm_records, &lm_scratch, &seq_count, &seq_score, &sel_count}) {
            if (b->p)
                (void)hipFree(b->p);
            b->p = nullptr, b->cap = 0;
// ... 579 lines not shown
        HIP_TRY(launch_lm_tasks(kind, d_tasks, total_jobs, max_n, c->stream));
        HIP_TRY(launch_group_score_seq(kind, gc.args.as<SeqScoreArgs>(), count, max_jobs, c->stream));
        HIP_TRY(wait_stream(c));
        for (uint32_t i = 0; i < count; ++i) {
            GroupItem &g = (*pit[i]);
            if (!g.active)
                continue;
            RansacRun &r = *g.run;
            for (uint32_t j = 0; j < (uint32_t)r.jobs.size(); ++j) {
                const uint32_t t = g.job0 + j;
                RefineJob &job = r.jobs[j];
                job.skipped = ht[t].skipped != 0;
                std::memcpy(job.params_out, ht[t].params, sizeof(double) * kParamDoubles);
                if (job.skipped)
                    std::memcpy(job.record_out, job.record_in, sizeof(double) * kModelStride);
                else
                    record_from_lm_params(kind, ht[t].params, job.record_out);
                job.count = gc.h_count.as<uint32_t>()[t];
                job.score = gc.h_score.as<double>()[t];
            }
        }
        return PL_OK;
    };

    if (!warm_members.empty()) {
        const uint32_t nw = (uint32_t)warm_members.size();
        HIP_TRY(gc.h_tasks.ensure(resident ? sizeof(double) * kModelStride * nw : raise_hw(g_hw_tasks, sizeof(double) * kModelStride * nw)));
        HIP_TRY(gc.lm_records.ensure(sizeof(double) * kModelStride * nw));
        HIP_TRY(gc.seq_count.ensure(sizeof(uint32_t) * nw));
        HIP_TRY(gc.seq_score.ensure(sizeof(double) * nw));
        HIP_TRY(gc.h_count.ensure(sizeof(uint32_t) * nw));
        HIP_TRY(gc.h_score.ensure(sizeof(double) * nw));
        double *hrec = gc.h_tasks.as<double>();
        SeqScoreArgs *hs = gc.h_args.as<SeqScoreArgs>();
        for (uint32_t i = 0; i < count; ++i)
            std::memset(&hs[i], 0, sizeof(SeqScoreArgs));
        for (uint32_t w = 0; w < nw; ++w) {
            GroupItem &g = (*pit[warm_members[w]]);
            std::memcpy(hrec + (size_t)w * kModelStride, g.rec, sizeof(double) * kModelStride);
            hs[warm_members[w]] = plain_seq_args(c, g.prob.ps, gc.lm_records.as<double>() + (size_t)w * kModelStride, 1, g.run->thr2,
                                                 gc.seq_count.as<uint32_t>() + w, gc.seq_score.as<double>() + w,
                                                 gc.h_count.dev<uint32_t>() + w, gc.h_score.dev<double>() + w);
        }
        HIP_TRY(hipMemcpyAsync(gc.lm_records.p, hrec, sizeof(double) * kModelStride * nw, hipMemcpyHostToDevice, c->stream));
        HIP_TRY(hipMemcpyAsync(gc.args.p, hs, sizeof(SeqScoreArgs) * count, hipMemcpyHostToDevice, c->stream));
        HIP_TRY(launch_group_score_seq(kind, gc.args.as<SeqScoreArgs>(), count, 1, c->stream));
        HIP_TRY(wait_stream(c));
        std::vector<uint32_t> cnts(nw);
        std::vector<double> scs(nw);
        for (uint32_t w = 0; w < nw; ++w)
            cnts[w] = gc.h_count.as<uint32_t>()[w], scs[w] = gc.h_score.as<double>()[w];
        for (uint32_t i = 0; i < count; ++i)
            if ((*pit[i]).run)
                (*pit[i]).run->jobs.clear();
        for (uint32_t w = 0; w < nw; ++w) {
            RansacRun &r = *(*pit[warm_members[w]]).run;
            const uint64_t cnt = cnts[w];
            const double sc = scs[w];
            const bool more = cnt > r.best_min_inl, better = sc < r.best_min_score;
            if (!(more || better))
                continue;
            if (more)
                r.best_min_inl = cnt;
            if (better)
                r.best_min_score = sc;
            if (sc < r.st->model_score) {
                r.st->model_score = sc;
                r.st->num_inliers = cnt;
            }
            r.jobs.push_back(r.make_lo_job(r.best_record));
        }
        {
            const int rc_jobs = run_queued_jobs();
            if (rc_jobs != PL_OK)
                return rc_jobs;
        }
        for (uint32_t w = 0; w < nw; ++w) {
            RansacRun &r = *(*pit[warm_members[w]]).run;
            if (!r.jobs.empty()) {
                const int rc_lo = r.after_lo(r.jobs[0]);
                if (rc_lo != PL_OK)
                    return rc_lo;
            }
            r.jobs.clear();
            r.begin_loop();
        }
    }

    std::vector<size_t> hexp_of;
    for (uint32_t step = 0;; ++step) {
        if (max_steps && step >= max_steps) {
            for (uint32_t i = 0; i < count; ++i) {
                GroupItem &g = (*pit[i]);
                if (g.active && !g.run->stopped && g.run->it < g.run->ro.max_iterations && !(g.run->it > g.run->ro.min_iterations && g.run->it > g.run->dyn_max))
                    g.deferred = true, g.active = false;
            }
            break;
        }
        std::unique_ptr<PhaseTimer> ptArgs(new PhaseTimer(g_t_args));
        GroupArgs *ha = gc.h_args.as<GroupArgs>();
        GroupDims dims;
        std::memset(&dims, 0, sizeof(dims));
        dims.G = count;
        dims.P = P;
        dims.min_n = 0xffffffffu;
        uint32_t nactive = 0;
        std::vector<uint32_t> prosac_members;
        hexp_of.assign(count, 0);
        for (uint32_t i = 0; i < count; ++i) {
            GroupItem &g = (*pit[i]);
            GroupArgs &a = ha[i];
            std::memset(&a, 0, sizeof(a));
            if (!g.active)
                continue;
            RansacRun &r = *g.run;
            if (!r.plan_batch(g.b)) {
                g.active = false;
                continue;
            }
            if (resume)
                g.b.B = g.b.hi_g = g.b.Bl = (uint32_t)std::min<uint64_t>(std::max<uint64_t>(g.b.B, r.needed_now()), 32768);
            else if (step > 0)
                g.b.B = g.b.hi_g = g.b.Bl = (uint32_t)std::min<uint64_t>(std::max<uint64_t>(g.b.B, r.needed_now()), max_B);
            if (g.b.B > max_B)
                g.b.B = g.b.hi_g = g.b.Bl = max_B;
            const uint32_t B = g.b.B;
            const uint32_t N = g.n;
            const uint64_t M64 = sampler_window(N, K, B);
            if (M64 > max_M || r.pos + M64 >= 0xffffffffull) {
                g.active = false, g.fallback = true;
                continue;
            }
            const BatchRun run = r.batch_run();
            BatchShape s;
            s.B = s.Bl = B, s.lo = 0, s.M = (uint32_t)M64, s.slots = (uint32_t)r.MAXM;
            s.use_mfma = score_uses_mfma(kind, N, run.pf);
            s.chunks = group_member_chunks(kind, s.use_mfma, N);
            s.point_rows = s.chunks * 64u * (uint32_t)P;
            s.prune = score_prune_gate(kind, s.use_mfma, B, s.chunks);
            const BatchBuffers bb = slot_buffers(i);
            wire_batch_step(a, run, s, bb);
            if (r.prosac) {
                g.b.prosac_at_batch_start = r.prosac_sampler;
                prosac_members.push_back(i);
            }
            const uint32_t hcap = a.score.hyp_capacity;
            hexp_of[i] = group_expected_hypotheses(kind, B, hcap);
            group_dims_sampler(dims, a.samp.M, g.n, B);
            dims.max_hcap = std::max(dims.max_hcap, hcap);
            dims.max_chunks = std::max(dims.max_chunks, a.chunks);
            dims.any_mfma |= a.use_mfma;
            dims.any_queue |= a.use_mfma ? 0u : 1u;
            dims.any_prune |= a.score.prune.st ? 1u : 0u;
            ++nactive;
        }
        if (nactive == 0)
            break;
        {
            uint32_t launch_chunks = 0;
            for (uint32_t i = 0; i < count; ++i)
                if (ha[i].active && ha[i].use_mfma)
                    launch_chunks += ha[i].chunks;
            for (uint32_t i = 0; i < count; ++i) {
                GroupArgs &a = ha[i];
                if (!a.active)
                    continue;
                a.slices = group_score_slices(kind, a.use_mfma != 0, hexp_of[i], a.gen.num_iters, a.chunks, launch_chunks);
                dims.max_slices = std::max(dims.max_slices, a.slices);
            }
        }
        if (!prosac_members.empty()) {
            size_t words = 0;
            for (uint32_t i : prosac_members)
                words += (size_t)(*pit[i]).b.B * K;
            HIP_TRY(gc.h_samples.ensure(sizeof(uint32_t) * words));
            uint32_t *hs = gc.h_samples.as<uint32_t>();
            for (uint32_t i : prosac_members) {
                GroupItem &g = (*pit[i]);
                if (!g.active)
                    continue;
                RansacRun &r = *g.run;
                for (uint32_t bb = 0; bb < g.b.B; ++bb)
                    r.prosac_sampler.generate(hs + (size_t)bb * K);
                g.b.pos_after = r.prosac_sampler.pos;
                HIP_TRY(hipMemcpyAsync(slot_buffers(i).samples, hs, sizeof(uint32_t) * (size_t)g.b.B * K, hipMemcpyHostToDevice, c->stream));
                hs += (size_t)g.b.B * K;
            }
        }
        ptArgs.reset();
        HIP_TRY(hipMemcpyAsync(gc.args.p, ha, sizeof(GroupArgs) * count, hipMemcpyHostToDevice, c->stream));
        HIP_TRY(launch_group_batch(kind, gc.args.as<GroupArgs>(), dims, c->stream, c->ev0, c->ev1));
        HIP_TRY(wait_stream(c));
        {
            float ms = 0.f;
            HIP_TRY(hipEventElapsedTime(&ms, c->ev0, c->ev1));
            for (uint32_t i = 0; i < count; ++i)
                if ((*pit[i]).active) {
                    (*pit[i]).st->score_kernel_ms += (double)ms / nactive;
                    (*pit[i]).st->score_kernel_launches++;
                }
        }

        std::unique_ptr<PhaseTimer> ptImp(new PhaseTimer(g_t_imp));
        for (uint32_t i = 0; i < count; ++i) {
            GroupItem &g = (*pit[i]);
            if (!g.active)
                continue;
            RansacRun &r = *g.run;
            const BatchCtl &hc = gc.h_ctl.as<BatchCtl>()[i];
            if ((hc.orbit_error && !r.prosac) || hc.gen_overflow || hc.num_records > kRecordFirst) {
                g.active = false, g.fallback = true;
                continue;
            }
            if (!r.prosac)
                g.b.pos_after = hc.pos_after;
            g.b.device_positions = !r.prosac;
            g.b.overflow = false;
            g.b.H = g.b.H_local = hc.num_hyp;
            g.b.h_rec = gc.h_recm.as<double>() + (size_t)i * kRecordFirst * kModelStride;
            g.st->nan_hypotheses += hc.nan_hyp;
            const RecordMeta *meta = gc.h_meta.as<RecordMeta>() + (size_t)i * kRecordFirst;
            r.list_improving(meta, hc.num_records, (uint32_t)r.it);
            r.make_jobs(g.b);
        }
        ptImp.reset();
        {
            const int rc_jobs = run_queued_jobs();
            if (rc_jobs != PL_OK)
                return rc_jobs;
        }
        PhaseTimer ptReplay(g_t_replay);
        for (uint32_t i = 0; i < count; ++i) {
            GroupItem &g = (*pit[i]);
            if (!g.active)
                continue;
            g.run->defer_offset = true;
            g.run->deferred_offset = -1;
            const int rc = g.run->replay(g.b, nullptr);
            if (rc != PL_OK)
                return rc;
        }
        for (uint32_t i = 0; i < count; ++i) {
            GroupItem &g = (*pit[i]);
            if (g.active && g.run->deferred_offset >= 0) {
                g.off_fetch = g.run->deferred_offset;
                g.run->deferred_offset = -1;
            }
        }
    }

    PhaseTimer ptTail(g_t_tail);
    const bool merged_tail = !resident && kind != EST_FUND;
    const uint64_t min_inl = front_min_inliers(kind);
    uint32_t ne = 0, ne_cam = 0;
    auto fill_bundle_task = [&](uint32_t i, GroupItem &g, LMTask &T) {
        const FrontBundle fb = front_bundle(g.fe);
        std::memset(&T, 0, sizeof(T));
        T.pts = g.prob.ps;
        if (kind == EST_ABS) {
            double *soa2 = reinterpret_cast<double *>(slot(i, L.pts2));
            for (int d = 0; d < nd; ++d)
                T.pts.a[d] = soa2 + (size_t)d * g.n;
        }
        T.opt = fb.opt;
        T.cam = fb.cam;
        T.cam_flags = fb.cam_flags;
        T.point_scale = fb.point_scale;
        T.prefilter_thr2 = 0.0;
        T.mask = reinterpret_cast<uint8_t *>(slot(i, L.mask));
        T.scratch = nullptr;
        T.record_in = nullptr;
        T.record_out = nullptr;
    };
    auto fill_prepare2 = [&](uint32_t i, GroupItem &g, PrepareGroupArgs &h) {
        CameraParams raw_cam;
        std::memset(&raw_cam, 0, sizeof(raw_cam));
        raw_cam.model_id = CAM_NULL;
        h.a_raw = g.raw_a;
        h.b_raw = g.raw_b;
        h.n = g.n;
        h.args = prepare_unproject(raw_cam, nullptr);
        h.soa = reinterpret_cast<double *>(slot(i, L.pts2));
        h.absmax_bits = nullptr;
    };
    {
        uint32_t nt = 0;
        for (uint32_t i = 0; i < count; ++i)
            if (!(*pit[i]).fallback && !(*pit[i]).deferred && (*pit[i]).looped)
                (*pit[i]).job0 = nt++;
        const size_t tail_bytes = (sizeof(LMTask) + 2 * sizeof(double) * kModelStride) * std::max<uint32_t>(nt, 1u);
        HIP_TRY(gc.h_tasks.ensure(tail_bytes));
        HIP_TRY(gc.lm_records.ensure(sizeof(double) * kModelStride * std::max<uint32_t>(nt, 1u)));
        HIP_TRY(gc.lm_scratch.ensure((size_t)max_n * std::max<uint32_t>(nt, 1u) + 16));
        HIP_TRY(gc.seq_count.ensure(sizeof(uint32_t) * std::max<uint32_t>(nt, 1u)));
        HIP_TRY(gc.seq_score.ensure(sizeof(double) * std::max<uint32_t>(nt, 1u)));
        HIP_TRY(gc.h_count.ensure(sizeof(uint32_t) * std::max<uint32_t>(nt, 1u)));
        HIP_TRY(gc.h_score.ensure(sizeof(double) * std::max<uint32_t>(nt, 1u)));
        if (merged_tail)
            HIP_TRY(gc.sel_count.ensure(sizeof(uint32_t) * count));
        LMTask *ht = gc.h_tasks.as<LMTask>();
        double *hr = reinterpret_cast<double *>(ht + nt);
        LMTask *d_tasks = gc.h_tasks.dev<LMTask>();
        double *d_rec = reinterpret_cast<double *>(d_tasks + nt);
        char *hb = gc.h_args.as<char>();
        SeqScoreArgs *hs = reinterpret_cast<SeqScoreArgs *>(hb);
        SelectArgs *hsel = reinterpret_cast<SelectArgs *>(hb + sizeof(SeqScoreArgs) * count);
// ... 191 lines not shown
```

### poselib_amd/csrc/kernels.hip

```cpp
#include "pl_kernels.h"
#include "pl_global.h"
#include "pl_lm_chain.inc"
#include "pl_device.h"
#include <atomic>
#include "pl_prefilter.h"
#include <cstdlib>
#include "pl_sampler.h"
#include "pl_solver_h4.h"
#include "pl_solver_p3p.h"
#include "pl_solver_p5lp_radial.h"
#include "pl_solver_rel.h"

namespace pl {

typedef const float __attribute__((address_space(4))) *uniform_f32_ptr;
typedef const double __attribute__((address_space(4))) *uniform_f64_ptr;
typedef const uint32_t __attribute__((address_space(4))) *uniform_u32_ptr;
__device__ __forceinline__ uniform_f32_ptr as_uniform(const float *p) { return (uniform_f32_ptr)(uintptr_t)p; }
__device__ __forceinline__ uniform_f64_ptr as_uniform(const double *p) { return (uniform_f64_ptr)(uintptr_t)p; }
__device__ __forceinline__ uniform_u32_ptr as_uniform(const uint32_t *p) { return (uniform_u32_ptr)(uintptr_t)p; }

__device__ __forceinline__ double wave_sum(double v) {
#pragma unroll
    for (int off = 32; off > 0; off >>= 1)
// ... 1446 lines not shown
__global__ __launch_bounds__(kMfmaThreads) __attribute__((amdgpu_waves_per_eu(4, 8))) void k_score_mfma_pr_g(const GroupArgs *ga) {
    const GroupArgs &g = ga[blockIdx.z];
    uint32_t slice, chunk;
    const uint32_t ns = pruned_slices<MODE>(g.slices);
    if (!g.active || !g.use_mfma || !slice_chunk_of_workgroup(ns, g.chunks, slice, chunk))
        return;
    score_mfma_pruned<PG, MODE>(globalised(g.score), slice, chunk, ns);
}

__device__ __forceinline__ void prune_lead_body(const ScoreArgs &a) {
    __shared__ uint32_t wmax[4];
    __shared__ double wmin[4];
    const PruneArgs &pr = a.prune;
    const uint32_t n = min(*a.num_hyp, pr.lead), N = a.pts.n;
    uint32_t bmax = 0;
    double bmin = 1.7976931348623157e308;
    for (uint32_t p = threadIdx.x; p < n; p += 256) {
        uint32_t c = 0;
        double s = 0.0;
        for (uint32_t ch = 0; ch < pr.chunks; ++ch) {
            c += a.part_count[(size_t)ch * a.hyp_capacity + p];
            s += a.part_score[(size_t)ch * a.hyp_capacity + p];
        }
        bmax = max(bmax, c);
        bmin = fmin(bmin, s + (double)(N - c) * a.thr2);
    }
#pragma unroll
    for (int off = 32; off > 0; off >>= 1) {
        bmax = max(bmax, (uint32_t)__shfl_xor(bmax, off, 64));
        bmin = fmin(bmin, __shfl_xor(bmin, off, 64));
    }
    if ((threadIdx.x & 63) == 0) {
        wmax[threadIdx.x >> 6] = bmax;
        wmin[threadIdx.x >> 6] = bmin;
    }
    __syncthreads();
    if (threadIdx.x == 0) {
        uint32_t lmax = pr.init_max;
        double lmin = pr.init_min;
        for (int w = 0; w < 4; ++w) {
            lmax = max(lmax, wmax[w]);
            lmin = fmin(lmin, wmin[w]);
        }
        const double need = fmax(lmin / a.thr2, (double)(N - min(lmax, N))) + (double)kPruneMargin;
        uint32_t cstar = pr.chunks;
        if (need < (double)N)
            cstar = (uint32_t)ceil(need / (double)pr.chunk_points);
        pr.st->lead_max = lmax;
        pr.st->lead_min = lmin;
        pr.st->cstar = max(1u, min(cstar, pr.chunks));
        pr.st->sel_len = 0;
        pr.st->pad = 0;
    }
}
__global__ __launch_bounds__(256) void k_prune_lead(ScoreArgs a) { prune_lead_body(a); }
__global__ __launch_bounds__(256) void k_prune_lead_g(const GroupArgs *ga) {
    const GroupArgs &g = ga[blockIdx.z];
    if (!g.active || !g.use_mfma || !g.score.prune.st)
        return;
    prune_lead_body(globalised(g.score));
}

__device__ __forceinline__ bool prune_rule(uint32_t cs, double sum, uint32_t S, uint32_t N, double thr2, const PruneState &st) {
    return cs + (N - S) <= st.lead_max && sum + (double)(S - cs) * thr2 > st.lead_min * (1.0 + kPruneScoreMargin);
}
__device__ __forceinline__ uint32_t prune_keeps(const ScoreArgs &a, uint32_t p, uint32_t H, uint32_t cstar) {
    const PruneArgs &pr = a.prune;
    if (p >= H)
        return 0u;
    if (p < pr.lead || cstar >= pr.chunks)
        return 1u;
    const uint32_t N = a.pts.n, S = min(cstar * pr.chunk_points, N);
    uint32_t cs = 0;
    for (uint32_t ch = 0; ch < cstar; ++ch)
        cs += a.part_count[(size_t)ch * a.hyp_capacity + p];
    return prune_rule(cs, 0.0, S, N, a.thr2, *pr.st) ? 0u : 1u;
}
__global__ __launch_bounds__(256) void k_prune_label(ScoreArgs a) {
    const PruneArgs &pr = a.prune;
    const uint32_t H = *a.num_hyp, cstar = pr.st->cstar, p = blockIdx.x * 256u + threadIdx.x;
    if (p >= H || p < pr.lead || cstar >= pr.chunks || pr.kept[p] != kKept)
        return;
    const uint32_t N = a.pts.n, S = min(cstar * pr.chunk_points, N);
    uint32_t cs = 0;
    double sum = 0.0;
    for (uint32_t ch = 0; ch < cstar; ++ch) {
        cs += a.part_count[(size_t)ch * a.hyp_capacity + p];
        sum += a.part_score[(size_t)ch * a.hyp_capacity + p];
    }
    if (prune_rule(cs, sum, S, N, a.thr2, *pr.st))
        pr.kept[p] = kPrunedExact;
}
__device__ __forceinline__ void prune_flags_body(const ScoreArgs &a) {
    __shared__ uint32_t wt[16];
    const PruneArgs &pr = a.prune;
    const uint32_t H = *a.num_hyp, cstar = pr.st->cstar;
    if (blockIdx.x * 1024u >= H)
        return;
    const uint32_t p = blockIdx.x * 1024u + threadIdx.x;
    const uint32_t keep = prune_keeps(a, p, H, cstar);
    if (p < H)
        pr.kept[p] = (uint8_t)keep;
    const uint32_t tot = wave_sum_u32(keep);
    if ((threadIdx.x & 63) == 0)
        wt[threadIdx.x >> 6] = tot;
    __syncthreads();
    if (threadIdx.x == 0) {
        uint32_t t = 0;
        for (int w = 0; w < 16; ++w)
            t += wt[w];
        pr.blk_kept[blockIdx.x] = t;
    }
}
__device__ __forceinline__ void prune_list_body(const ScoreArgs &a) {
    __shared__ uint32_t wt[16], wb[16];
    const PruneArgs &pr = a.prune;
    const uint32_t H = *a.num_hyp;
    if (blockIdx.x * 1024u >= H)
        return;
    const int lane = threadIdx.x & 63, wave = threadIdx.x >> 6;
    uint32_t before = 0;
    for (uint32_t j = threadIdx.x; j < blockIdx.x; j += 1024u)
        before += pr.blk_kept[j];
    before = wave_sum_u32(before);
    const uint32_t p = blockIdx.x * 1024u + threadIdx.x;
    const uint32_t keep = p < H ? (uint32_t)pr.kept[p] : 0u;
    const uint32_t inc = wave_scan_u32(keep);
    if (lane == 63)
        wt[wave] = inc;
    if (lane == 0)
        wb[wave] = before;
    __syncthreads();
    uint32_t at = inc - keep;
    for (int w = 0; w < 16; ++w)
        at += wb[w] + (w < wave ? wt[w] : 0u);
    if (keep)
        pr.sel[at] = p;
    if (p == H - 1u)
        pr.st->sel_len = at + keep;
}
__global__ __launch_bounds__(1024) void k_prune_flags(ScoreArgs a) { prune_flags_body(a); }
__global__ __launch_bounds__(1024) void k_prune_list(ScoreArgs a) { prune_list_body(a); }
__global__ __launch_bounds__(1024) void k_prune_flags_g(const GroupArgs *ga) {
    const GroupArgs &g = ga[blockIdx.z];
    if (!g.active || !g.use_mfma || !g.score.prune.st)
        return;
    prune_flags_body(globalised(g.score));
}
__global__ __launch_bounds__(1024) void k_prune_list_g(const GroupArgs *ga) {
    const GroupArgs &g = ga[blockIdx.z];
    if (!g.active || !g.use_mfma || !g.score.prune.st)
        return;
    prune_list_body(globalised(g.score));
}



template <int EST, int PG>
__device__ __forceinline__ void score_mfma2_body(const PointSet &pts, const uint4 *__restrict__ hypop,
                                                 const double *__restrict__ models, const uint32_t *__restrict__ slots,
                                                 const uint32_t *__restrict__ num_hyp_ptr, uint32_t hyp_capacity,
                                                 double thr2, const PrefilterArgs &pf, uint32_t *__restrict__ part_count,
                                                 double *__restrict__ part_score, uint32_t slice, uint32_t chunk,
                                                 uint32_t nslices) {
    static_assert(EST == EST_REL || EST == EST_FUND, "Sampson scores");
    constexpr int kWaves = kMfmaThreads / 64;
    constexpr int NPW = 32 * PG;
    constexpr int NBR = (EST == EST_REL) ? 6 : 1;
    __shared__ double s_pts[4][NPW];
    __shared__ double s_bear[NBR][(EST == EST_REL) ? NPW : 1];
    __shared__ uint16_t s_queue[kWaves][kMfmaQueueCap];
    __shared__ double s_acc_s[kWaves][64];
    __shared__ uint32_t s_acc_c[kWaves][64];
    __shared__ uint32_t s_next_unit;
    __shared__ uint4 s_bop[PG][3][64];
    const int lane = threadIdx.x & 63;
    const int wave = __builtin_amdgcn_readfirstlane((int)(threadIdx.x >> 6));
    const int col = lane & 31, half = lane >> 5;

    for (uint32_t j = threadIdx.x; j < (uint32_t)NPW; j += kMfmaThreads) {
        const uint32_t i = chunk * NPW + j;
        const uint32_t ic = i < pts.n ? i : 0u;
        const double a0 = pts.a[0][ic], a1 = pts.a[1][ic], b0 = pts.a[2][ic], b1 = pts.a[3][ic];
        s_pts[0][j] = a0, s_pts[1][j] = a1, s_pts[2][j] = b0, s_pts[3][j] = b1;
        if constexpr (EST == EST_REL) {
            const Vec3 u1 = bearing(a0, a1), u2 = bearing(b0, b1);
            s_bear[0][j] = u1.x, s_bear[1][j] = u1.y, s_bear[2][j] = u1.z;
            s_bear[3][j] = u2.x, s_bear[4][j] = u2.y, s_bear[5][j] = u2.z;
        }
    }
    uint32_t validbits = 0;
#pragma unroll
    for (int g = 0; g < PG; ++g)
        validbits |= (chunk * NPW + g * 32 + col < pts.n) ? (1u << (PG - 1 - g)) : 0u;
    for (uint32_t j = threadIdx.x; j < (uint32_t)NPW; j += kMfmaThreads) {
        const uint32_t i = chunk * NPW + j;
        const bool valid = i < pts.n;
        const uint32_t ic = valid ? i : 0u;
        Sampson16Operand o;
        pf16_sampson_point(pts.a[0][ic], pts.a[1][ic], pts.a[2][ic], pts.a[3][ic], valid, pf.t16, o);
#pragma unroll
        for (int b = 0; b < 6; ++b) {
            const uint16_t *h = b < 4 ? o.c + 8 * b : o.s + 8 * (b - 4);
            s_bop[j >> 5][b >> 1][(j & 31) + 32 * (b & 1)] =
                make_uint4((uint32_t)h[0] | ((uint32_t)h[1] << 16), (uint32_t)h[2] | ((uint32_t)h[3] << 16),
                           (uint32_t)h[4] | ((uint32_t)h[5] << 16), (uint32_t)h[6] | ((uint32_t)h[7] << 16));
        }
    }
    if (threadIdx.x == 0)
        s_next_unit = 0;
    __syncthreads();

    const uint32_t H = *as_uniform(num_hyp_ptr);
    const float t16 = pf.t16;
    uint16_t *const queue = s_queue[wave];
    double *const acc_s = s_acc_s[wave];
    uint32_t *const acc_c = s_acc_c[wave];
    const uint32_t waves_per_chunk = nslices * kWaves;
    auto request_ticket = [&]() -> uint32_t {
        uint32_t t = 0;
        if (lane == 0) {
            const uint32_t k = atomicAdd(&s_next_unit, 1u);
            t = slice * kWaves + (k % kWaves) + (k / kWaves) * waves_per_chunk;
        }
        return t;
    };
    uint32_t ticket = (uint32_t)__builtin_amdgcn_readfirstlane((int)request_ticket());
    uint32_t kb, gn;
    while (unit_of_ticket(ticket, H, waves_per_chunk, kb, gn)) {
        const uint32_t pending = request_ticket();
        const uint32_t unit_slots = slots[kb + min((uint32_t)lane, gn - 1u)];
        acc_s[lane] = 0.0;
        acc_c[lane] = 0;
        uint32_t qhead = 0, qtail = 0;

        auto drain = [&](uint32_t n) {
            __builtin_amdgcn_fence(__ATOMIC_ACQ_REL, "wavefront");
            const bool act = (uint32_t)lane < n;
            const uint32_t e = act ? (uint32_t)queue[(qhead + lane) & (kMfmaQueueCap - 1)] : 0xffffu;
            const uint32_t g = e >> 9, pi = act ? (e & 0x1ffu) : 0u;
            const double x0 = s_pts[0][pi], x1 = s_pts[1][pi], x2 = s_pts[2][pi], x3 = s_pts[3][pi];
            const double *Mp = models + (size_t)(uint32_t)__shfl((int)unit_slots, (int)(act ? g : 0u), 64) * kModelStride;
            double M[kModelDoubles];
#pragma unroll
            for (int i = 0; i < kModelDoubles; ++i)
                M[i] = Mp[i];
            double r2 = sampson_sq(M + kMatOff, x0, x1, x2, x3);
            bool in = r2 < thr2;
            if constexpr (EST == EST_REL) {
                if (in) {
                    Quat q;
                    q.w = M[0], q.x = M[1], q.y = M[2], q.z = M[3];
                    in = check_cheirality(q, v3(M[4], M[5], M[6]), v3(s_bear[0][pi], s_bear[1][pi], s_bear[2][pi]),
                                          v3(s_bear[3][pi], s_bear[4][pi], s_bear[5][pi]), 0.01);
                }
            }
            in = in && act;
            double v = in ? r2 : 0.0;
            const uint64_t inmask = __builtin_amdgcn_ballot_w64(in);
            const uint32_t g0 = (uint32_t)__builtin_amdgcn_readfirstlane((int)g);
            if (inmask && !__builtin_amdgcn_ballot_w64(act && g != g0)) {
                const double tot = wave_sum_dpp(v);
                if (lane == 0) {
                    acc_s[g0] += tot;
                    acc_c[g0] += (uint32_t)__popcll(inmask);
                }
            } else if (inmask) {
                add_run_totals(v, inmask, g, act, lane, acc_s, acc_c);
            }
            qhead += n;
        };

        const uint32_t ngroups32 = (gn + 31u) / 32u;
        auto load_a = [&](uint32_t hg, uint4 (&A)[3]) {
            const uint4 *row = hypop + (size_t)(kb + 32u * hg + (uint32_t)col) * 6;
#pragma unroll
            for (int j = 0; j < 3; ++j)
                A[j] = row[2 * j + half];
        };
        uint4 Araw[3];
        load_a(0, Araw);
        for (uint32_t hg = 0; hg < ngroups32; ++hg) {
            half8_t Aop[3];
#pragma unroll
            for (int j = 0; j < 3; ++j)
                __builtin_memcpy(&Aop[j], &Araw[j], 16);
            if (hg + 1 < ngroups32)
                load_a(hg + 1, Araw);
            uint32_t out[16];
#pragma unroll
            for (int v = 0; v < 16; ++v)
                out[v] = 0u;
            const float16_t kZero = {0, 0, 0, 0, 0, 0, 0, 0, 0, 0, 0, 0, 0, 0, 0, 0};
#pragma unroll 2
            for (int g = 0; g < PG; ++g) {
                half8_t Bop[3];
#pragma unroll
                for (int j = 0; j < 3; ++j) {
                    const uint4 braw = s_bop[g][j][lane];
                    __builtin_memcpy(&Bop[j], &braw, 16);
                }
                float16_t C = __builtin_amdgcn_mfma_f32_32x32x16_f16(Aop[0], Bop[0], kZero, 0, 0, 0);
                C = __builtin_amdgcn_mfma_f32_32x32x16_f16(Aop[1], Bop[1], C, 0, 0, 0);
                const float16_t S = __builtin_amdgcn_mfma_f32_32x32x16_f16(Aop[2], Bop[2], kZero, 0, 0, 0);
#pragma unroll
                for (int v = 0; v < 16; ++v) {
// ... 1793 lines not shown
    return std::max<uint32_t>(1u, round / std::max<uint32_t>(1u, chunks));
}

static uint32_t xcd_slices(uint32_t s) { return std::max<uint32_t>(1u, s); }

template <int E>
static hipError_t launch_score_est(const ScoreArgs &a, uint32_t slices, hipStream_t stream) {
    uint32_t chunks;
    int P;
    const PrefilterArgs pf = a.pf;
    const bool streaming = (a.shadow && a.compact64) || a.shadow16;
    score_shape(E, a.pts.n, streaming, a.shadow16 != nullptr, chunks, P);
    if constexpr (E == EST_REL || E == EST_FUND) {
        if (streaming && a.shadow16) {
            const uint32_t mslices = std::min<uint32_t>(slices * (uint32_t)kScoreThreads / (uint32_t)kMfmaThreads,
                                                        score_slice_limit(E, chunks, true));
            const dim3 mgrid(xcd_slices(mslices), chunks);
            const dim3 mblock(kMfmaThreads);
#define PL_M2_CASE(PP)                                                                                                 \
    case PP:                                                                                                           \
        k_score_mfma2<E, 2 * PP><<<mgrid, mblock, 0, stream>>>(a.pts, static_cast<const uint4 *>(a.shadow16), a.models, \
                                                              a.slots, a.num_hyp, a.hyp_capacity, a.thr2, pf,          \
                                                              a.part_count, a.part_score);                             \
        break;
            switch (P) {
                PL_M2_CASE(1)
                PL_M2_CASE(2)
                PL_M2_CASE(3)
                PL_M2_CASE(4)
                PL_M2_CASE(5)
                PL_M2_CASE(6)
            default:
                return hipErrorInvalidValue;
            }
#undef PL_M2_CASE
            return hipGetLastError();
        }
    }
    if constexpr (E == EST_HOM) {
        if (streaming && a.shadow16) {
            const dim3 mgrid(xcd_slices(slices * (uint32_t)kScoreThreads / (uint32_t)kMfmaThreads), chunks);
            const dim3 mblock(kMfmaThreads);
#define PL_MH_CASE(PP)                                                                                                 \
    case PP:                                                                                                           \
        k_score_mfmah<2 * PP><<<mgrid, mblock, 0, stream>>>(a.pts, static_cast<const uint4 *>(a.shadow16), a.models,    \
                                                          a.slots, a.num_hyp, a.hyp_capacity, a.thr2, pf, a.part_count, \
                                                          a.part_score);                                                \
        break;
            switch (P) {
                PL_MH_CASE(1)
                PL_MH_CASE(2)
                PL_MH_CASE(3)
                PL_MH_CASE(4)
                PL_MH_CASE(5)
            default:
                return hipErrorInvalidValue;
            }
#undef PL_MH_CASE
            return hipGetLastError();
        }
    }
    if constexpr (E == EST_ABS) {
        if (streaming && a.shadow16) {
            const uint32_t mslices = std::min<uint32_t>(slices * (uint32_t)kScoreThreads / (uint32_t)kMfmaThreads,
                                                        score_slice_limit(E, chunks, true));
            const dim3 mgrid(xcd_slices(mslices), chunks);
            const dim3 mblock(kMfmaThreads);
            if (!a.points16)
                return hipErrorInvalidValue;
#define PL_M_CASE(PP)                                                                                                  \
    case PP:                                                                                                           \
        k_score_mfma<2 * PP><<<mgrid, mblock, 0, stream>>>(a.pts, static_cast<const uint4 *>(a.shadow16),                \
                                                         static_cast<const uint4 *>(a.points16), a.models, a.slots,    \
                                                         a.num_hyp, a.hyp_capacity, a.thr2, a.part_count, a.part_score, \
                                                         a.tickets);                                                   \
        break;
            switch (P) {
                PL_M_CASE(1)
                PL_M_CASE(2)
                PL_M_CASE(3)
                PL_M_CASE(4)
                PL_M_CASE(5)
            default:
                return hipErrorInvalidValue;
            }
#undef PL_M_CASE
            return hipGetLastError();
        }
    }
    if (streaming) {
        const dim3 qgrid(std::max<uint32_t>(1u, slices * (uint32_t)kScoreThreads / (uint32_t)kQueueThreads), chunks);
        const dim3 qblock(kQueueThreads);
#define PL_Q_CASE(PP)                                                                                                  \
    case PP:                                                                                                           \
        k_score_queue<E, PP><<<qgrid, qblock, 0, stream>>>(a.pts, a.shadow, a.compact64, a.num_hyp, a.hyp_capacity,      \
                                                         a.thr2, pf, a.part_count, a.part_score, a.tickets);           \
        break;
        switch (P) {
            PL_Q_CASE(1)
            PL_Q_CASE(2)
            PL_Q_CASE(3)
            PL_Q_CASE(4)
            PL_Q_CASE(5)
            PL_Q_CASE(6)
        default:
            return hipErrorInvalidValue;
        }
#undef PL_Q_CASE
        return hipGetLastError();
    }
    return hipErrorInvalidValue;
}

hipError_t launch_score_seq(int est, const SeqScoreArgs &a, hipStream_t stream) {
    if (a.cap == 0)
        return hipSuccess;
    const dim3 grid(std::min<uint32_t>(a.cap, 128u)), block(kSeqThreads);
    PL_DISPATCH_EST_0TO5(est, k_score_seq<E><<<grid, block, 0, stream>>>(a));
    return hipGetLastError();
}
int tangent_score_chunk() { return kTangentChunk; }
int radial1d_score_chunk() { return kRadialChunk; }
hipError_t launch_prune_lead(const ScoreArgs &a, hipStream_t stream) {
    k_prune_lead<<<dim3(1), dim3(256), 0, stream>>>(a);
    return hipGetLastError();
}
hipError_t launch_prune_select(const ScoreArgs &a, hipStream_t stream) {
    const uint32_t nb = std::max<uint32_t>(1u, (a.hyp_capacity + 1023u) / 1024u);
    k_prune_flags<<<dim3(nb), dim3(1024), 0, stream>>>(a);
    k_prune_list<<<dim3(nb), dim3(1024), 0, stream>>>(a);
    return hipGetLastError();
}
hipError_t launch_group_prune_lead(const GroupArgs *args, const GroupDims &d, hipStream_t stream) {
    k_prune_lead_g<<<dim3(1, 1, d.G), dim3(256), 0, stream>>>(args);
    return hipGetLastError();
}
hipError_t launch_group_prune_select(const GroupArgs *args, const GroupDims &d, hipStream_t stream) {
    const uint32_t nb = std::max<uint32_t>(1u, (d.max_hcap + 1023u) / 1024u);
    k_prune_flags_g<<<dim3(nb, 1, d.G), dim3(1024), 0, stream>>>(args);
    k_prune_list_g<<<dim3(nb, 1, d.G), dim3(1024), 0, stream>>>(args);
    return hipGetLastError();
}
template <int PG> static hipError_t launch_score_pruned_pg(const ScoreArgs &a, dim3 grid, hipStream_t stream) {
    const dim3 block(kMfmaThreads);
    const dim3 lead_grid(pruned_slices<kScoreLead>(grid.x), grid.y), sel_grid(pruned_slices<kScoreSel>(grid.x), grid.y);
    k_score_mfma_pr<PG, kScoreLead><<<lead_grid, block, 0, stream>>>(a);
    hipError_t e = launch_prune_lead(a, stream);
    if (e != hipSuccess)
        return e;
    k_score_mfma_pr<PG, kScoreCount><<<grid, block, 0, stream>>>(a);
    e = launch_prune_select(a, stream);
    if (e != hipSuccess)
        return e;
    k_score_mfma_pr<PG, kScoreSel><<<sel_grid, block, 0, stream>>>(a);
    return hipGetLastError();
}
static hipError_t pruned_grid(const ScoreArgs &a, uint32_t slices, dim3 &grid, int &P) {
    uint32_t chunks;
    score_shape(EST_ABS, a.pts.n, true, true, chunks, P);
    if (!a.shadow16 || !a.points16 || !a.prune.st || a.prune.chunks != chunks || a.prune.chunk_points != 64u * (uint32_t)P)
        return hipErrorInvalidValue;
    const uint32_t mslices = std::min<uint32_t>(slices * (uint32_t)kScoreThreads / (uint32_t)kMfmaThreads,
                                                score_slice_limit(EST_ABS, chunks, true));
    grid = dim3(xcd_slices(mslices), chunks);
    return (P == 4 || P == 5) ? hipSuccess : hipErrorInvalidValue;
}
hipError_t launch_score_pruned(const ScoreArgs &a, uint32_t slices, hipStream_t stream) {
    dim3 grid;
    int P;
    const hipError_t e = pruned_grid(a, slices, grid, P);
    if (e != hipSuccess)
        return e;
    return P == 4 ? launch_score_pruned_pg<8>(a, grid, stream) : launch_score_pruned_pg<10>(a, grid, stream);
}
hipError_t launch_score_count(const ScoreArgs &a, uint32_t slices, hipStream_t stream) {
    dim3 grid;
    int P;
    const hipError_t e = pruned_grid(a, slices, grid, P);
    if (e != hipSuccess)
        return e;
    if (P == 4)
        k_score_mfma_pr<8, kScoreCountAll><<<grid, dim3(kMfmaThreads), 0, stream>>>(a);
    else
        k_score_mfma_pr<10, kScoreCountAll><<<grid, dim3(kMfmaThreads), 0, stream>>>(a);
    return hipGetLastError();
}
hipError_t launch_prune_label(const ScoreArgs &a, hipStream_t stream) {
    k_prune_label<<<dim3(std::max<uint32_t>(1u, (a.hyp_capacity + 255u) / 256u)), dim3(256), 0, stream>>>(a);
    return hipGetLastError();
}

hipError_t launch_score(int est, const ScoreArgs &a, uint32_t slices, hipStream_t stream) {
    if (est == EST_RAD1D) {
        if (!a.shadow || !a.compact64)
            return hipErrorInvalidValue;
        const uint32_t chunks = score_chunks(est, a.pts.n, true, false);
        const dim3 qgrid(std::max<uint32_t>(1u, slices * (uint32_t)kScoreThreads / (uint32_t)kQueueThreads), chunks);
        k_score_radial1d<<<qgrid, dim3(kQueueThreads), 0, stream>>>(a.pts, a.shadow, a.compact64, a.num_hyp, a.hyp_capacity, a.thr2, a.pf,
                                                                    a.part_count, a.part_score);
        return hipGetLastError();
    }
    if (est == EST_RELT) {
        if (!a.shadow || !a.compact64)
            return hipErrorInvalidValue;
        const uint32_t chunks = score_chunks(est, a.pts.n, true, false);
        const dim3 qgrid(std::max<uint32_t>(1u, slices * (uint32_t)kScoreThreads / (uint32_t)kQueueThreads), chunks);
        k_score_tangent<<<qgrid, dim3(kQueueThreads), 0, stream>>>(a.pts, a.shadow, a.compact64, a.num_hyp, a.hyp_capacity, a.thr2, a.pf,
                                                                   a.part_count, a.part_score);
        return hipGetLastError();
    }
    PL_DISPATCH_EST(est, return launch_score_est<E>(a, slices, stream));
    return hipSuccess;
}


hipError_t launch_lm(int est, const PointSet &pts, LMTask *tasks, uint32_t num_tasks, hipStream_t stream) {
    const size_t want = sizeof(double) * point_doubles(est) * (size_t)pts.n;
    return launch_lm_tasks(est, tasks, num_tasks, want <= 128 * 1024 ? pts.n : 0u, stream);
}
static std::atomic<int> g_lm_mode{-1};
void set_lm_mode(int mode) { g_lm_mode.store((mode == 1 || mode == 2) ? mode : 0, std::memory_order_release); }
int get_lm_mode() {
    int m = g_lm_mode.load(std::memory_order_acquire);
    if (m < 0) {
        const char *e = std::getenv("POSELIB_AMD_LM_ORDERED");
        m = (e && e[0] == '1') ? 1 : (e && e[0] == '2') ? 2 : 0;
        g_lm_mode.store(m, std::memory_order_release);
    }
    return m;
}
static thread_local int tl_lm_force_ordered = 0;
void set_lm_force_ordered(int on) { tl_lm_force_ordered = on; }
bool lm_sums_ordered(int est) {
    if (tl_lm_force_ordered)
        return true;
    const int m = get_lm_mode();
    return est != EST_RELT && (m == 1 || (m == 0 && est == EST_FUND));
}
#ifdef PL_LM_PROFILE
extern "C" int pl_debug_lm_profile(unsigned long long *out16, int reset) {
    if (hipMemcpyFromSymbol(out16, HIP_SYMBOL(g_lm_prof), sizeof(unsigned long long) * 16) != hipSuccess)
        return -1;
    if (reset) {
        unsigned long long z[16] = {0};
        if (hipMemcpyToSymbol(HIP_SYMBOL(g_lm_prof), z, sizeof(z)) != hipSuccess)
            return -1;
    }
    return 0;
}
#endif
hipError_t launch_lm_tasks(int est, LMTask *tasks, uint32_t num_tasks, uint32_t max_points, hipStream_t stream) {
    if (num_tasks == 0)
        return hipSuccess;
    if (est < 0 || est > EST_RAD1D)
        return hipErrorInvalidValue;
    const int ordered = lm_sums_ordered(est) ? 1 : 0;
    static std::atomic<int> dyn_limit[2][6] = {{{-1}, {-1}, {-1}, {-1}, {-1}, {-1}}, {{-1}, {-1}, {-1}, {-1}, {-1}, {-1}}};
    int limit = dyn_limit[ordered][est].load(std::memory_order_acquire);
    if (limit < 0) {
        hipFuncAttributes fa;
        hipError_t e = hipSuccess;
        if (ordered) {
            PL_DISPATCH_EST_0123_5(est, e = hipFuncGetAttributes(&fa, reinterpret_cast<const void *>(&k_lm_ordered<E>)));
        } else {
            PL_DISPATCH_EST_0TO5(est, e = hipFuncGetAttributes(&fa, reinterpret_cast<const void *>(&k_lm<E>)));
        }
        if (e != hipSuccess)
            return e;
        limit = std::max<int>(0, 160 * 1024 - (int)fa.sharedSizeBytes - 1024);
        limit = std::min<int>(limit, 128 * 1024);
        if (limit > 48 * 1024) {
            if (ordered) {
                PL_DISPATCH_EST_0123_5(est, e = hipFuncSetAttribute(reinterpret_cast<const void *>(&k_lm_ordered<E>),
                                                             hipFuncAttributeMaxDynamicSharedMemorySize, limit));
            } else {
                PL_DISPATCH_EST_0TO5(est, e = hipFuncSetAttribute(reinterpret_cast<const void *>(&k_lm<E>),
                                                              hipFuncAttributeMaxDynamicSharedMemorySize, limit));
            }
            if (e != hipSuccess)
                return e;
        }
        dyn_limit[ordered][est].store(limit, std::memory_order_release);
    }
    const size_t want = sizeof(double) * point_doubles(est) * (size_t)max_points;
    const size_t bytes = want <= (size_t)limit ? want : 0;
    if (ordered) {
        PL_DISPATCH_EST_0123_5(est, k_lm_ordered<E><<<dim3(num_tasks), dim3(kLMThreads), bytes, stream>>>(tasks, (uint32_t)bytes));
    } else {
        PL_DISPATCH_EST_0TO5(est, k_lm<E><<<dim3(num_tasks), dim3(kLMThreads), bytes, stream>>>(tasks, (uint32_t)bytes));
    }
    return hipGetLastError();
}

__global__ void k_task_records(int est, const LMTask *tasks, const double *records_in, double *records_out,
                               uint32_t num_tasks, LMTask *host_tasks) {
    const uint32_t j = blockIdx.x * blockDim.x + threadIdx.x;
    if (j >= num_tasks)
        return;
    if (host_tasks) {
        for (int i = 0; i < kParamDoubles; ++i)
            host_tasks[j].params[i] = tasks[j].params[i];
        host_tasks[j].iterations = tasks[j].iterations;
        host_tasks[j].skipped = tasks[j].skipped;
        host_tasks[j].cost = tasks[j].cost;
        host_tasks[j].initial_cost = tasks[j].initial_cost;
    }
    double *out = records_out + (size_t)j * kModelStride;
    if (tasks[j].skipped) {
        for (int i = 0; i < kModelStride; ++i)
            out[i] = records_in[(size_t)j * kModelStride + i];
    } else {
        record_from_lm_params(est, tasks[j].params, out);
    }
}
__global__ void k_select_record(const double *score_refined, double incumbent_score, const double *rec_refined,
                                const double *rec_incumbent, double *out) {
    const double *src = (*score_refined < incumbent_score) ? rec_refined : rec_incumbent;
    if (threadIdx.x < kModelStride)
        out[threadIdx.x] = src[threadIdx.x];
}
__global__ void k_select_record_g(const SelectArgs *arr) {
    const SelectArgs a = globalised(arr[blockIdx.z]);
    if (!a.out)
        return;
    const double *src = (*a.score_refined < a.incumbent_score) ? a.rec_refined : a.rec_incumbent;
    if (threadIdx.x < kModelStride)
        a.out[threadIdx.x] = src[threadIdx.x];
    if (threadIdx.x == 63 && a.fetch_src)
        *a.fetch_dst = *a.fetch_src;
    if (threadIdx.x == 62 && a.count_out)
        *a.count_out = (*a.score_refined < a.incumbent_score) ? *a.count_refined : a.count_incumbent;
}
hipError_t launch_group_select(const SelectArgs *args, uint32_t G, hipStream_t stream) {
    if (G == 0)
        return hipSuccess;
    k_select_record_g<<<dim3(1, 1, G), dim3(64), 0, stream>>>(args);
    return hipGetLastError();
}
hipError_t launch_group_mask(int est, const MaskArgs *args, uint32_t G, uint32_t max_n, hipStream_t stream) {
    if (G == 0 || max_n == 0)
        return hipSuccess;
    const dim3 grid((max_n + 255) / 256, 1, G), block(256);
    PL_DISPATCH_EST(est, k_mask_g<E><<<grid, block, 0, stream>>>(args));
    return hipGetLastError();
}
hipError_t launch_group_score_seq(int est, const SeqScoreArgs *args, uint32_t G, uint32_t max_cap, hipStream_t stream) {
    if (G == 0 || max_cap == 0)
        return hipSuccess;
    const dim3 grid(std::min<uint32_t>(max_cap, 128u), 1, G), block(kSeqThreads);
    PL_DISPATCH_EST(est, k_score_seq_g<E><<<grid, block, 0, stream>>>(args));
    return hipGetLastError();
}

int group_points_per_lane(int est) { return (est == EST_REL || est == EST_FUND) ? 6 : 5; }

template <int E> static hipError_t launch_group_score_est(const GroupArgs *args, const GroupDims &d, hipStream_t stream) {
    const dim3 grid(std::max<uint32_t>(1u, d.max_slices), std::max<uint32_t>(1u, d.max_chunks), d.G);
    if constexpr (E == EST_ABS) {
        if (d.any_mfma && d.any_prune) {
            const dim3 lead_grid(pruned_slices<kScoreLead>(grid.x), grid.y, grid.z), sel_grid(pruned_slices<kScoreSel>(grid.x), grid.y, grid.z);
            k_score_mfma_pr_g<10, kScoreLead><<<lead_grid, dim3(kMfmaThreads), 0, stream>>>(args);
            hipError_t e = launch_group_prune_lead(args, d, stream);
            if (e != hipSuccess)
                return e;
            k_score_mfma_pr_g<10, kScoreCount><<<grid, dim3(kMfmaThreads), 0, stream>>>(args);
            e = launch_group_prune_select(args, d, stream);
            if (e != hipSuccess)
                return e;
            k_score_mfma_pr_g<10, kScoreSel><<<sel_grid, dim3(kMfmaThreads), 0, stream>>>(args);
        } else if (d.any_mfma)
            k_score_mfma_g<10><<<grid, dim3(kMfmaThreads), 0, stream>>>(args);
        if (d.any_queue)
            k_score_queue_g<EST_ABS, 5><<<grid, dim3(kQueueThreads), 0, stream>>>(args);
    } else if constexpr (E == EST_HOM) {
        if (d.any_mfma)
            k_score_mfmah_g<10><<<grid, dim3(kMfmaThreads), 0, stream>>>(args);
        if (d.any_queue)
            k_score_queue_g<EST_HOM, 5><<<grid, dim3(kQueueThreads), 0, stream>>>(args);
    } else {
        if (d.any_mfma)
            k_score_mfma2_g<E, 2 * group_mfma2_points_per_lane(E)><<<grid, dim3(kMfmaThreads), 0, stream>>>(args);
        if (d.any_queue)
            k_score_queue_g<E, 6><<<grid, dim3(kQueueThreads), 0, stream>>>(args);
    }
    return hipGetLastError();
}

hipError_t launch_group_score_count(const GroupArgs *args, const GroupDims &d, hipStream_t stream) {
    const dim3 grid(std::max<uint32_t>(1u, d.max_slices), std::max<uint32_t>(1u, d.max_chunks), d.G);
    k_score_mfma_pr_g<10, kScoreCountAll><<<grid, dim3(kMfmaThreads), 0, stream>>>(args);
    return hipGetLastError();
}
hipError_t launch_group_score(int est, const GroupArgs *args, const GroupDims &d, hipStream_t stream) {
    if (d.G == 0)
        return hipSuccess;
    hipError_t e = hipSuccess;
    PL_DISPATCH_EST(est, e = launch_group_score_est<E>(args, d, stream));
    return e;
}

hipError_t launch_group_generate(int est, const GroupArgs *args, uint32_t max_B, uint32_t G, hipStream_t stream) {
    if (G == 0 || max_B == 0)
        return hipSuccess;
    if (est == EST_REL)
        return launch_group_generate_rel(args, max_B, G, stream);
    const dim3 ggrid((max_B + 63) / 64, 1, G), gblock(64);
    PL_DISPATCH_EST(est, k_generate_g<E><<<ggrid, gblock, 0, stream>>>(args));
    return hipGetLastError();
}

hipError_t launch_group_batch(int est, const GroupArgs *args, const GroupDims &d, hipStream_t stream, hipEvent_t ev0,
                              hipEvent_t ev1) {
    if (d.G == 0)
        return hipSuccess;
    hipError_t e = launch_group_positions(sample_size(est), args, d, stream);
    if (e != hipSuccess)
        return e;
    e = launch_group_generate(est, args, d.max_B, d.G, stream);
    if (e != hipSuccess)
        return e;
    e = launch_group_compact(args, d, stream);
    if (e != hipSuccess)
        return e;
    if (ev0 && (e = hipEventRecord(ev0, stream)) != hipSuccess)
        return e;
    e = launch_group_score(est, args, d, stream);
    if (e != hipSuccess)
        return e;
    if (ev1 && (e = hipEventRecord(ev1, stream)) != hipSuccess)
        return e;
    e = launch_group_finalize_records(args, d, stream);
    if (e != hipSuccess)
        return e;
    const uint32_t per_problem = std::max<uint32_t>(16u, std::min<uint32_t>(128u, 4096u / std::max<uint32_t>(1u, d.G)));
    const dim3 sgrid(per_problem, 1, d.G), sblock(kSeqThreads);
    PL_DISPATCH_EST(est, k_score_seq_gb<E><<<sgrid, sblock, 0, stream>>>(args));
    return hipGetLastError();
}

hipError_t launch_task_records(int est, const LMTask *tasks, const double *records_in, double *records_out,
                               uint32_t num_tasks, LMTask *host_tasks, hipStream_t stream) {
    if (num_tasks == 0)
        return hipSuccess;
    k_task_records<<<dim3((num_tasks + 63) / 64), dim3(64), 0, stream>>>(est, tasks, records_in, records_out, num_tasks,
                                                                         host_tasks);
    return hipGetLastError();
}
hipError_t launch_select_record(const double *score_refined, double incumbent_score, const double *rec_refined,
                                const double *rec_incumbent, double *out, hipStream_t stream) {
    k_select_record<<<dim3(1), dim3(64), 0, stream>>>(score_refined, incumbent_score, rec_refined, rec_incumbent, out);
    return hipGetLastError();
}

size_t lm2_state_bytes(uint32_t num_tasks) { return sizeof(LM2State) * 2 * (size_t)num_tasks; }
size_t lm2_partial_bytes(uint32_t num_tasks, uint32_t slices) { return sizeof(double) * 2 * (size_t)num_tasks * slices * 48; }
hipError_t launch_lm2(int est, const PointSet &pts, LMTask *tasks, uint32_t num_tasks, uint32_t slices,
                      uint32_t max_iterations, void *states, double *partials, hipStream_t stream) {
    if (num_tasks == 0)
        return hipSuccess;
    if (est == EST_REL)
        return hipErrorInvalidValue;
    const dim3 grid(slices, num_tasks), block(kLM2Threads);
    const uint32_t launches = max_iterations + 2;
    for (uint32_t l = 0; l < launches; ++l) {
        switch (est) {
        case EST_ABS:
            k_lm2<EST_ABS><<<grid, block, 0, stream>>>(pts, tasks, static_cast<LM2State *>(states), partials, (int)(l & 1), l == 0);
            break;
        case EST_FUND:
            k_lm2<EST_FUND><<<grid, block, 0, stream>>>(pts, tasks, static_cast<LM2State *>(states), partials, (int)(l & 1), l == 0);
            break;
        default:
            k_lm2<EST_HOM><<<grid, block, 0, stream>>>(pts, tasks, static_cast<LM2State *>(states), partials, (int)(l & 1), l == 0);
            break;
        }
    }
    return hipGetLastError();
}

hipError_t launch_mask(int est, const PointSet &pts, const double *model, double thr2, uint8_t *mask,
                       uint8_t *host_mask, hipStream_t stream) {
    if (pts.n == 0)
        return hipSuccess;
    const dim3 grid((pts.n + 255) / 256), block(256);
    PL_DISPATCH_EST_0TO5(est, k_mask<E><<<grid, block, 0, stream>>>(pts, model, thr2, mask, host_mask));
    return hipGetLastError();
}

}
```

### poselib_amd/csrc/pl_global.h

```cpp
#pragma once
#include "pl_kernels.h"

namespace pl {

template <class T> __device__ __forceinline__ T *as_global(T *p) {
    typedef __attribute__((address_space(1))) T GlobalT;
    return (T *)(GlobalT *)(uintptr_t)p;
}

__device__ __forceinline__ PointSet globalised(PointSet p) {
    for (int d = 0; d < 5; ++d)
        p.a[d] = as_global(p.a[d]);
    return p;
}
__device__ __forceinline__ SampleArgs globalised(SampleArgs s) {
    s.delta = as_global(s.delta);
    s.flagbits = as_global(s.flagbits);
    s.positions = as_global(s.positions);
    s.ctl = as_global(s.ctl);
    return s;
}
__device__ __forceinline__ GenerateArgs globalised(GenerateArgs g) {
    g.pts = globalised(g.pts);
    g.positions = as_global(g.positions);
    g.samples = as_global(g.samples);
    g.ctl = as_global(g.ctl);
    g.models = as_global(g.models);
    g.num_models = as_global(g.num_models);
    g.blk_tot = as_global(g.blk_tot);
    g.blk_nan = as_global(g.blk_nan);
    g.nan_bits = as_global(g.nan_bits);
    g.stage = as_global(g.stage);
    return g;
}
__device__ __forceinline__ Shadow16Params globalised(Shadow16Params s) {
    s.out = as_global(s.out);
    s.live = as_global(s.live);
    s.rank = as_global(s.rank);
    s.nan_bits = as_global(s.nan_bits);
    s.points16 = as_global(s.points16);
    return s;
}
__device__ __forceinline__ CompactArgs globalised(CompactArgs c) {
    c.num_models = as_global(c.num_models);
    c.blk_tot = as_global(c.blk_tot);
    c.slots = as_global(c.slots);
    c.offsets = as_global(c.offsets);
    c.models = as_global(c.models);
    c.shadow = as_global(c.shadow);
    c.compact64 = as_global(c.compact64);
    c.ctl = as_global(c.ctl);
    c.s16 = globalised(c.s16);
    c.host_offsets = as_global(c.host_offsets);
    return c;
}
__device__ __forceinline__ ScoreArgs globalised(ScoreArgs a) {
    a.pts = globalised(a.pts);
    a.models = as_global(a.models);
    a.slots = as_global(a.slots);
    a.shadow = as_global(a.shadow);
    a.compact64 = as_global(a.compact64);
    a.shadow16 = as_global(a.shadow16);
    a.points16 = as_global(a.points16);
    a.num_hyp = as_global(a.num_hyp);
    a.part_count = as_global(a.part_count);
    a.part_score = as_global(a.part_score);
    a.tickets = as_global(a.tickets);
    a.prune.st = as_global(a.prune.st);
    a.prune.blk_kept = as_global(a.prune.blk_kept);
    a.prune.sel = as_global(a.prune.sel);
    a.prune.kept = as_global(a.prune.kept);
    return a;
}
__device__ __forceinline__ FinalizeArgs globalised(FinalizeArgs f) {
    f.num_hyp = as_global(f.num_hyp);
    f.rank = as_global(f.rank);
    f.part_count = as_global(f.part_count);
    f.part_score = as_global(f.part_score);
    f.count = as_global(f.count);
    f.score = as_global(f.score);
    f.kept = as_global(f.kept);
    return f;
}
__device__ __forceinline__ RecordsArgs globalised(RecordsArgs r) {
    r.f = globalised(r.f);
    r.slots = as_global(r.slots);
    r.models = as_global(r.models);
    r.blk_max = as_global(r.blk_max);
    r.blk_min = as_global(r.blk_min);
    r.rec_meta = as_global(r.rec_meta);
    r.rec_models = as_global(r.rec_models);
    r.ctl = as_global(r.ctl);
    r.host_meta = as_global(r.host_meta);
    r.host_models = as_global(r.host_models);
    return r;
}
__device__ __forceinline__ SeqScoreArgs globalised(SeqScoreArgs a) {
    a.pts = globalised(a.pts);
    a.models = as_global(a.models);
    a.cand = as_global(a.cand);
    a.num = as_global(a.num);
    a.count = as_global(a.count);
    a.score = as_global(a.score);
    a.host_count = as_global(a.host_count);
    a.host_score = as_global(a.host_score);
    a.host_cand = as_global(a.host_cand);
    a.ctl_src = as_global(a.ctl_src);
    a.ctl_host = as_global(a.ctl_host);
    return a;
}
__device__ __forceinline__ MaskArgs globalised(MaskArgs m) {
    m.pts = globalised(m.pts);
    m.model = as_global(m.model);
    m.mask = as_global(m.mask);
    m.host_mask = as_global(m.host_mask);
    return m;
}
__device__ __forceinline__ SelectArgs globalised(SelectArgs s) {
    s.score_refined = as_global(s.score_refined);
    s.rec_refined = as_global(s.rec_refined);
    s.rec_incumbent = as_global(s.rec_incumbent);
    s.out = as_global(s.out);
    s.count_refined = as_global(s.count_refined);
    s.count_out = as_global(s.count_out);
    s.fetch_src = as_global(s.fetch_src);
    s.fetch_dst = as_global(s.fetch_dst);
    return s;
}
__device__ __forceinline__ PrepareGroupArgs globalised(PrepareGroupArgs p) {
    p.a_raw = as_global(p.a_raw);
    p.b_raw = as_global(p.b_raw);
    p.soa = as_global(p.soa);
    p.absmax_bits = as_global(p.absmax_bits);
    return p;
}

struct LMTaskPointers {
    PointSet pts;
    const uint8_t *mask;
    uint8_t *scratch;
    const double *record_in;
    double *record_out;
    const double *start_record;
    const uint32_t *gate_count;
};
__device__ __forceinline__ LMTaskPointers globalised(const LMTask &T) {
    LMTaskPointers g;
    g.pts = globalised(T.pts);
    g.mask = as_global(T.mask);
    g.scratch = as_global(T.scratch);
    g.record_in = as_global(T.record_in);
    g.record_out = as_global(T.record_out);
    g.start_record = as_global(T.start_record);
    g.gate_count = as_global(T.gate_count);
    return g;
}

}
```

### poselib_amd/csrc/pl_kernels.h

```cpp
#pragma once
#include "pl_prefilter.h"
#include "pl_refine.h"

#include <hip/hip_runtime.h>
#include <stdint.h>

namespace pl {

struct PointSet {
    const double *a[5];
    uint32_t n;
    float xy_absmax;
};

constexpr int kScoreThreads = 256;
constexpr int kStreamWaves = 8;
constexpr int kLMSeqPoints = 256;
#ifndef PL_LM_THREADS
#define PL_LM_THREADS 512
#endif
constexpr int kLMThreads = PL_LM_THREADS;

PL_HD constexpr int sample_size(int est) { return est == EST_ABS ? 3 : (est == EST_REL || est == EST_RELT || est == EST_RAD1D) ? 5 : est == EST_FUND ? 7 : 4; }
PL_HD constexpr int max_models(int est) { return (est == EST_ABS || est == EST_RAD1D) ? 4 : (est == EST_REL || est == EST_RELT) ? 40 : est == EST_FUND ? 3 : 1; }
PL_HD constexpr int point_doubles(int est) { return (est == EST_ABS || est == EST_RAD1D) ? 5 : est == EST_RELT ? 18 : 4; }

struct BatchCtl;
struct GenerateArgs {
    PointSet pts;
    uint64_t seed;
    uint64_t pos_base;
    const uint32_t *positions;
    const uint32_t *samples;
    uint32_t num_iters;
    uint32_t slots_per_iter;
    struct BatchCtl *ctl;
    double *models;
    uint32_t *num_models;
    int32_t real_focal_check;
    uint32_t *blk_tot = nullptr;
    uint32_t *blk_nan = nullptr;
    uint32_t *nan_bits = nullptr;
    void *stage = nullptr;
};

constexpr uint32_t kPruneLead = 2048;
constexpr uint32_t kPruneMargin = 32;
constexpr double kPruneScoreMargin = 1e-6;
struct PruneState {
    uint32_t lead_max;
    uint32_t cstar;
    uint32_t sel_len;
    uint32_t pad;
    double lead_min;
};
struct PruneArgs {
    PruneState *st = nullptr;
    uint32_t *blk_kept = nullptr;
    uint32_t *sel = nullptr;
    uint8_t *kept = nullptr;
    uint32_t chunks = 0, chunk_points = 0;
    uint32_t init_max = 0, lead = 0;
    double init_min = 0.0;
};
constexpr uint8_t kDropped = 0, kKept = 1, kPrunedExact = 2;

struct ScoreArgs {
    PointSet pts;
    const double *models;
    const uint32_t *slots;
    const float *shadow;
    const double *compact64;
    const void *shadow16;
    const void *points16 = nullptr;
    const uint32_t *num_hyp;
    uint32_t hyp_capacity;
    double thr2;
    PrefilterArgs pf;
    uint32_t *part_count;
    double *part_score;
    uint32_t *tickets;
    PruneArgs prune;
};
constexpr uint32_t kMaxScoreChunks = 4096;

constexpr uint32_t kNoRank = 0xffffffffu;
struct FinalizeArgs {
    const uint32_t *num_hyp;
    const uint32_t *rank = nullptr;
    uint32_t hyp_capacity, chunks, n_points;
    double thr2;
    const uint32_t *part_count;
    const double *part_score;
    uint32_t *count;
    double *score;
    const uint8_t *kept = nullptr;
};

struct LMTask {
    PointSet pts;
    double params[kParamDoubles];
    LMOptions opt;
    CameraParams cam;
    double point_scale;
    double prefilter_thr2;
    const uint8_t *mask;
    uint8_t *scratch;
    const double *record_in;
    double *record_out;
    int32_t cam_flags;
    int32_t pad0;
    const double *start_record;
    const uint32_t *gate_count;
    uint32_t gate_min;
    uint32_t pad1;
    uint32_t iterations, skipped;
    double cost, initial_cost;
};

struct BatchCtl {
    uint32_t num_hyp;
    uint32_t num_records;
    uint32_t orbit_error;
    uint32_t gen_overflow;
    uint64_t pos_after;
    uint32_t nan_hyp;
    uint32_t num_live;
};
struct RecordMeta {
    uint32_t k, slot, count, pad;
    double score;
};

struct SeqScoreArgs {
    PointSet pts;
    const double *models;
    RecordMeta *cand;
    const uint32_t *num;
    uint32_t cap;
    double thr2;
    uint32_t *count;
    double *score;
    uint32_t *host_count;
    double *host_score;
    RecordMeta *host_cand;
    uint32_t host_cap;
    const BatchCtl *ctl_src = nullptr;
    BatchCtl *ctl_host = nullptr;
};
hipError_t launch_score_seq(int est, const SeqScoreArgs &a, hipStream_t stream);

hipError_t launch_generate(int est, const GenerateArgs &a, hipStream_t stream);
size_t generate_stage_bytes(int est, uint32_t num_iters);
size_t rel_stage_bytes(uint32_t num_iters);
hipError_t launch_generate_rel(const GenerateArgs &a, hipStream_t stream, bool tangent = false);
struct GroupArgs;
hipError_t launch_group_generate_rel(const GroupArgs *args, uint32_t max_B, uint32_t G, hipStream_t stream);
hipError_t launch_group_generate(int est, const GroupArgs *args, uint32_t max_B, uint32_t G, hipStream_t stream);
struct PrepareArgs {
    int32_t mode;
    int32_t centred;
    CameraParams cam1, cam2;
    double c1x, c1y, c2x, c2y, scale;
};
hipError_t launch_prepare(const double *a_raw, const double *b_raw, uint32_t n, const PrepareArgs &args, double *soa,
                          unsigned long long *absmax_bits, hipStream_t stream);
constexpr int kDeviceMathFns = 12;
hipError_t launch_device_math(int fn, const double *x, uint32_t n, double *out, hipStream_t stream);
constexpr int kDeviceMath2Fns = 2;
hipError_t launch_device_math2(int fn, const double *x, const double *y, uint32_t n, double *out, hipStream_t stream);
hipError_t launch_undistort(const double *in, uint32_t n, const CameraParams &cam, double fx, double fy, double cx,
                            double cy, double *out, hipStream_t stream);
struct IngestSrc {
    const void *data;
    int64_t row_stride;
    int32_t f32;
    int32_t cols;
};
hipError_t launch_ingest(const IngestSrc &a, const IngestSrc &b, uint32_t n, double *out_a, double *out_b, hipStream_t stream);
hipError_t launch_ingest_soa(const IngestSrc &a, const IngestSrc &b, uint32_t n, int b_in_max, double *soa,
                             unsigned long long *absmax_bits, hipStream_t stream);
struct PointStatsArgs {
    int32_t norm, centred, bound, pad;
    double cx1, cy1, fx1, fy1, cx2, cy2, fx2, fy2;
    double n_as_double, scale_divisor;
};
struct PointStatsRecord {
    double c1x, c1y, c2x, c2y, scale, absmax, reserved[2];
};
hipError_t launch_point_stats(const double *a_raw, const double *b_raw, uint32_t n, const PointStatsArgs &args,
                              PointStatsRecord *out , hipStream_t stream);
struct IngestGroupArgs {
    IngestSrc a, b;
    uint32_t n, pad;
    double *out_a, *out_b;
};
hipError_t launch_ingest_g(const IngestGroupArgs *tab, uint32_t G, uint32_t max_n, hipStream_t stream);
struct PointStatsGroupArgs {
    const double *a_raw, *b_raw;
    uint32_t n, pad;
    PointStatsArgs args;
    PointStatsRecord *out;
};
hipError_t launch_point_stats_g(const PointStatsGroupArgs *tab, uint32_t G, hipStream_t stream);
hipError_t launch_task_records(int est, const LMTask *tasks, const double *records_in, double *records_out,
                               uint32_t num_tasks, LMTask *host_tasks, hipStream_t stream);
hipError_t launch_select_record(const double *score_refined, double incumbent_score, const double *rec_refined,
                                const double *rec_incumbent, double *out, hipStream_t stream);
uint32_t abs16_point_rows(uint32_t n_points);
bool score_uses_mfma(int est, uint32_t n_points, const PrefilterArgs &pf);
hipError_t launch_sampson16(BatchCtl *ctl, const uint32_t *slots, const double *models, uint32_t capacity, void *out,
                            hipStream_t stream);
hipError_t launch_hom16(BatchCtl *ctl, const uint32_t *slots, const double *models, uint32_t capacity, float thr, void *out,
                        hipStream_t stream);
size_t lm2_state_bytes(uint32_t num_tasks);
size_t lm2_partial_bytes(uint32_t num_tasks, uint32_t slices);
hipError_t launch_lm2(int est, const PointSet &pts, LMTask *tasks, uint32_t num_tasks, uint32_t slices,
                      uint32_t max_iterations, void *states, double *partials, hipStream_t stream);
uint32_t score_chunks(int est, uint32_t n_points, bool prefilter, bool mfma = false);
int score_points_per_lane(int est, uint32_t n_points, bool streaming, bool mfma);
uint32_t score_slice_limit(int est, uint32_t chunks, bool mfma);
hipError_t launch_score(int est, const ScoreArgs &a, uint32_t slices, hipStream_t stream);
hipError_t launch_score_pruned(const ScoreArgs &a, uint32_t slices, hipStream_t stream);
hipError_t launch_score_count(const ScoreArgs &a, uint32_t slices, hipStream_t stream);
hipError_t launch_prune_label(const ScoreArgs &a, hipStream_t stream);
hipError_t launch_prune_lead(const ScoreArgs &a, hipStream_t stream);
hipError_t launch_prune_select(const ScoreArgs &a, hipStream_t stream);
int tangent_score_chunk();
int radial1d_score_chunk();
hipError_t launch_lm(int est, const PointSet &pts, LMTask *tasks, uint32_t num_tasks, hipStream_t stream);
hipError_t launch_mask(int est, const PointSet &pts, const double *model, double thr2, uint8_t *mask,
                       uint8_t *host_mask, hipStream_t stream);

struct Shadow16Params {
    void *out = nullptr;
    float g16 = 0.f, c16 = 0.f, thr = 0.f;
    int sampson = 0;
    uint32_t *live = nullptr;
    uint32_t *rank = nullptr;
    const uint32_t *nan_bits = nullptr;
    void *points16 = nullptr;
    uint32_t point_rows = 0;
};
constexpr size_t kSampson16Bytes = 96;
constexpr size_t kAbs16Bytes = 64;
constexpr size_t kAbs16Pad = 32;
constexpr size_t kAbs16PointBytes = 64;
constexpr size_t kSampson16Pad = 64;
constexpr size_t kHom16Bytes = 256;
constexpr size_t kHom16Pad = 8;
hipError_t launch_abs16(BatchCtl *ctl, const uint32_t *slots, const double *models, uint32_t capacity, const PointSet &pts,
                        const Shadow16Params &s16, hipStream_t stream);
hipError_t launch_gather_models(BatchCtl *ctl, const uint32_t *slots, const double *models, uint32_t capacity,
                                float *shadow_compact, double *compact64, hipStream_t stream);
hipError_t launch_finalize(const FinalizeArgs &f, hipStream_t stream);

struct SampleArgs {
    uint64_t seed, pos_base, N;
    uint32_t B, M;
    uint8_t *delta;
    uint64_t *flagbits;
    uint32_t *positions;
    BatchCtl *ctl;
    uint32_t zero_words, pad;
};
struct CompactArgs {
    const uint32_t *num_models;
    uint32_t B;
    int32_t maxm;
    uint32_t *blk_tot, *slots, *offsets;
    const double *models;
    float *shadow;
    double *compact64;
    BatchCtl *ctl;
    Shadow16Params s16;
    uint32_t *host_offsets;
};
struct RecordsArgs {
    FinalizeArgs f;
    const uint32_t *slots;
    const double *models;
    uint32_t *blk_max;
    double *blk_min;
    uint32_t init_max, rec_cap;
    double init_min;
    RecordMeta *rec_meta;
    double *rec_models;
    BatchCtl *ctl;
    RecordMeta *host_meta;
    double *host_models;
    uint32_t host_cap, pad;
};
hipError_t launch_sample_positions(int K, const SampleArgs &a, hipStream_t stream, int build = 0);
hipError_t launch_sample_orbit(int K, const SampleArgs &a, hipStream_t stream, int build = 0);
bool orbit_small_build(uint32_t M, uint64_t N, int K);
struct OrbitShape {
    uint32_t flags, doubling, segments, tile;
};
OrbitShape orbit_build_shape(bool small);
hipError_t launch_compact2(const CompactArgs &a, bool counted, const PointSet &pts, hipStream_t stream);
hipError_t launch_finalize_records(const RecordsArgs &a, hipStream_t stream);
struct MaskArgs {
    PointSet pts;
    const double *model;
    double thr2;
    uint8_t *mask, *host_mask;
};
struct SelectArgs {
    const double *score_refined;
    double incumbent_score;
    const double *rec_refined, *rec_incumbent;
    double *out;
    const uint32_t *count_refined;
    uint32_t count_incumbent;
    uint32_t pad;
    uint32_t *count_out;
    const uint32_t *fetch_src;
    uint32_t *fetch_dst;
};
struct GroupArgs {
    uint32_t active;
    uint32_t use_mfma;
    uint32_t chunks, slices;
    SampleArgs samp;
    GenerateArgs gen;
    CompactArgs comp;
    ScoreArgs score;
    RecordsArgs rec;
    SeqScoreArgs seq;
};
constexpr int group_mfma2_points_per_lane(int est) { return est == EST_REL ? 5 : 6; }
struct GroupDims {
    uint32_t G;
    uint32_t max_M;
    uint32_t min_n;
    uint32_t max_B;
    uint32_t max_hcap;
    uint32_t max_chunks, max_slices;
    uint32_t any_mfma, any_queue;
    uint32_t any_prune;
    int P;
};
hipError_t launch_group_batch(int est, const GroupArgs *args, const GroupDims &dims, hipStream_t stream,
                              hipEvent_t ev0 = nullptr, hipEvent_t ev1 = nullptr);
hipError_t launch_group_score(int est, const GroupArgs *args, const GroupDims &d, hipStream_t stream);
hipError_t launch_group_prune_lead(const GroupArgs *args, const GroupDims &d, hipStream_t stream);
hipError_t launch_group_prune_select(const GroupArgs *args, const GroupDims &d, hipStream_t stream);
hipError_t launch_group_score_count(const GroupArgs *args, const GroupDims &d, hipStream_t stream);
hipError_t launch_group_score_seq(int est, const SeqScoreArgs *args, uint32_t G, uint32_t max_cap, hipStream_t stream);
hipError_t launch_group_select(const SelectArgs *args, uint32_t G, hipStream_t stream);
hipError_t launch_group_mask(int est, const MaskArgs *args, uint32_t G, uint32_t max_n, hipStream_t stream);
struct PrepareGroupArgs {
    const double *a_raw, *b_raw;
    uint32_t n, pad;
    PrepareArgs args;
    double *soa;
    unsigned long long *absmax_bits;
};
hipError_t launch_group_prepare(const PrepareGroupArgs *args, uint32_t G, uint32_t max_n, hipStream_t stream);
hipError_t launch_group_positions(int K, const GroupArgs *args, const GroupDims &d, hipStream_t stream, int build = 0);
hipError_t launch_group_orbit(int K, const GroupArgs *args, const GroupDims &d, hipStream_t stream, int build = 0);
hipError_t launch_group_compact(const GroupArgs *args, const GroupDims &d, hipStream_t stream);
hipError_t launch_group_finalize_records(const GroupArgs *args, const GroupDims &d, hipStream_t stream);
hipError_t launch_lm_tasks(int est, LMTask *tasks, uint32_t num_tasks, uint32_t max_points, hipStream_t stream);
void set_lm_mode(int mode);
int get_lm_mode();
bool lm_sums_ordered(int est);
void set_lm_force_ordered(int on);
hipError_t launch_lm_cam(LMTask *tasks, uint32_t num_tasks, hipStream_t stream);
int group_points_per_lane(int est);

hipError_t launch_solve_batch(int est, const double *in, uint32_t num_problems, double *models, uint32_t *num_models,
                              hipStream_t stream);

}
```

### poselib_amd/csrc/pl_prefilter.h

```cpp
#pragma once
#include "pl_math.h"

#include <cmath>

namespace pl {

constexpr float kPfU = 5.9604644775390625e-08f;

struct PrefilterArgs {
    float thr;
    float gx;
    float thr2_up;
    int enabled;
    float g16;
    float c16;
    float t1;
    float w252;
    float t16;
    float h16;
};

PL_HD float pf_up(float v) { return v * 1.000001f + 1e-30f; }

inline PrefilterArgs make_prefilter_args(int est, double thr2, float xy_absmax) {
    PrefilterArgs a;
    a.thr = a.gx = a.thr2_up = a.g16 = a.c16 = a.t1 = a.w252 = a.t16 = a.h16 = 0.f;
    a.enabled = 0;
    if (!(thr2 >= 1e-30 && thr2 <= 1e30))
        return a;
    if (est == 0  && !(xy_absmax <= 3.0e38f))
        return a;
    const float inf = __builtin_huge_valf();
    const double thr = sqrt(thr2);
    const double u = 5.9604644775390625e-08;
    a.thr = nextafterf((float)thr, inf);
    a.thr2_up = nextafterf((float)(thr2 * (1.0 + 64.0 * u)), inf);
    a.t1 = nextafterf((float)((16.0 / 15.0) * (1.0 + 1.0 / 64.0) * thr2 * (1.0 + 96.0 * u)), inf);
    a.w252 = nextafterf((float)((16.0 / 15.0) * (1.0 + 96.0 * u) * 60.0), inf);
    if (est == 0) {
        a.gx = nextafterf((float)(32.0 * u * (1.0 + (double)xy_absmax + thr)), inf);
        a.g16 = nextafterf((float)(4.8828125e-4 * 1.015625), inf);
        a.c16 = nextafterf((float)((2e-7 + 5.0e-4) * (1.0 + 1.3661 * (double)xy_absmax + thr)), inf);
    }
    if (est == 1 || est == 2) {
        if (xy_absmax <= 8.0f && thr2 >= 1e-12 && thr2 <= 1e4)
            a.t16 = nextafterf((float)((16.0 / 15.0) * 32768.0 * thr2 * (1.0 + 256.0 * u)), inf);
    }
    if (est == 3) {
        if (xy_absmax <= 8.0f && thr >= 1e-9 && thr <= 8.0)
            a.h16 = a.thr;
    }
    a.enabled = 1;
    return a;
}

PL_HD float pf_point_abs(double X, double Y, double Z, float gx) {
    return pf_up(gx * pf_up((float)sqrt(X * X + Y * Y + Z * Z)));
}
PL_HD void pf_point_two_view(double a0, double a1, double b0, double b1, float thr, float &nanb, float &nsq,
                             float &nanb_thr) {
    const float na = pf_up((float)(1.0 + fabs(a0) + fabs(a1)));
    const float nb = pf_up((float)(1.0 + fabs(b0) + fabs(b1)));
    nanb = pf_up(na * nb);
    nsq = pf_up(130.f * pf_up(na * na + nb * nb));
    nanb_thr = pf_up(na * pf_up(nb + thr));
}
PL_HD float pf_point_sampson_w(float nanb, float nsq, const PrefilterArgs &pf) {
    return pf_up(pf_up(pf.t1 * nsq) + pf_up(pf.w252 * pf_up(nanb * nanb)));
}


PL_HD bool pf_abs_outlier(const float *r, float gt , float thr, float x, float y, float X, float Y,
                          float Z, float fw) {
    const float z0 = fmaf(r[0], X, fmaf(r[1], Y, fmaf(r[2], Z, r[9])));
    const float z1 = fmaf(r[3], X, fmaf(r[4], Y, fmaf(r[5], Z, r[10])));
    const float z2 = fmaf(r[6], X, fmaf(r[7], Y, fmaf(r[8], Z, r[11])));
    const float a0 = fmaf(-x, z2, z0);
    const float a1 = fmaf(-y, z2, z1);
    const float W = fw + gt;
    const float B = fmaf(thr, z2, W);
    return (fmaxf(fabsf(a0), fabsf(a1)) > B) | (z2 < -W);
}

PL_HD bool pf_hom_outlier(const float *r, float gh , float thr, float a0, float a1, float b0, float b1,
                          float nanb_thr) {
    const float h0 = fmaf(r[0], a0, fmaf(r[1], a1, r[2]));
    const float h1 = fmaf(r[3], a0, fmaf(r[4], a1, r[5]));
    const float h2 = fmaf(r[6], a0, fmaf(r[7], a1, r[8]));
    const float e0 = fmaf(-b0, h2, h0);
    const float e1 = fmaf(-b1, h2, h1);
    const float W = gh * nanb_thr;
    const float B = fmaf(thr, fabsf(h2), W);
    return fmaxf(fabsf(e0), fabsf(e1)) > B;
}

PL_HD bool pf_sampson_outlier(const float *r, float gf , float t1, float a0, float a1, float b0,
                              float b1, float w) {
    const float Ea0 = fmaf(r[0], a0, fmaf(r[1], a1, r[2]));
    const float Ea1 = fmaf(r[3], a0, fmaf(r[4], a1, r[5]));
    const float Ea2 = fmaf(r[6], a0, fmaf(r[7], a1, r[8]));
    const float Eb0 = fmaf(r[0], b0, fmaf(r[3], b1, r[6]));
    const float Eb1 = fmaf(r[1], b0, fmaf(r[4], b1, r[7]));
    const float C = fmaf(b0, Ea0, fmaf(b1, Ea1, Ea2));
    const float S = fmaf(Eb1, Eb1, fmaf(Eb0, Eb0, fmaf(Ea1, Ea1, Ea0 * Ea0)));
    return C * C > fmaf(t1, S, (gf * gf) * w);
}

constexpr float kPfTangentT = 1.08334f;
constexpr float kPfTangentW = 9.7014e-13f;
PL_HD float pf_tangent_scale(float fm) {
    union {
        float f;
        uint32_t u;
    } a, b;
    a.f = fm;
    b.u = (253u - ((a.u >> 23) & 0xffu)) << 23;
    return b.f;
}
PL_HD float pf_tangent_point(const double *pt , double thr, float *f) {
    double p1 = 0, p2 = 0, m1 = 0, m2 = 0, dmax = 0, nmax = 0;
    bool nan = false;
    PL_UNROLL
    for (int j = 0; j < 3; ++j) {
        const double a = fabs(pt[j]), b = fabs(pt[3 + j]);
        p1 += a, p2 += b;
        dmax = fmax(dmax, fmax(a, b));
        nan = nan || a != a || b != b;
        f[j] = (float)pt[j], f[3 + j] = (float)pt[3 + j];
    }
    PL_UNROLL
    for (int j = 0; j < 6; ++j) {
        const double n1 = thr * pt[6 + j], n2 = thr * pt[12 + j];
        const double a = fabs(n1), b = fabs(n2);
        m1 += a, m2 += b;
        nmax = fmax(nmax, fmax(a, b));
        nan = nan || a != a || b != b;
        f[6 + j] = (float)n1, f[12 + j] = (float)n2;
    }
    if (nan || !(dmax <= 16.0) || !(nmax >= 1e-6 && nmax <= 1e6))
        return __builtin_huge_valf();
    const float fp1 = pf_up((float)p1), fp2 = pf_up((float)p2), fm1 = pf_up((float)m1), fm2 = pf_up((float)m2);
    const float a = pf_up(fp1 * fm2), b = pf_up(fp2 * fm1), c = pf_up(fp1 * fp2);
    return pf_up(kPfTangentW * pf_up(pf_up(130.f * pf_up(pf_up(a * a) + pf_up(b * b))) + pf_up(16.f * pf_up(c * c))));
}
PL_HD bool pf_tangent_outlier(const float *e, const float *f, float W) {
    const float *d1 = f, *d2 = f + 3, *n1 = f + 6, *n2 = f + 12;
    const float v0 = fmaf(e[0], d1[0], fmaf(e[1], d1[1], e[2] * d1[2]));
    const float v1 = fmaf(e[3], d1[0], fmaf(e[4], d1[1], e[5] * d1[2]));
    const float v2 = fmaf(e[6], d1[0], fmaf(e[7], d1[1], e[8] * d1[2]));
    const float w0 = fmaf(e[0], d2[0], fmaf(e[3], d2[1], e[6] * d2[2]));
    const float w1 = fmaf(e[1], d2[0], fmaf(e[4], d2[1], e[7] * d2[2]));
    const float w2 = fmaf(e[2], d2[0], fmaf(e[5], d2[1], e[8] * d2[2]));
    const float C = fmaf(d2[0], v0, fmaf(d2[1], v1, d2[2] * v2));
    const float a0 = fmaf(n2[0], v0, fmaf(n2[2], v1, n2[4] * v2));
    const float a1 = fmaf(n2[1], v0, fmaf(n2[3], v1, n2[5] * v2));
    const float b0 = fmaf(n1[0], w0, fmaf(n1[2], w1, n1[4] * w2));
    const float b1 = fmaf(n1[1], w0, fmaf(n1[3], w1, n1[5] * w2));
    const float S = fmaf(b1, b1, fmaf(b0, b0, fmaf(a1, a1, a0 * a0)));
    return C * C > fmaf(kPfTangentT, S, W);
}

PL_HD uint16_t pf_half_rn(float f) {
#if defined(__HIP_DEVICE_COMPILE__)
    const _Float16 h = (_Float16)f;
    uint16_t b;
    __builtin_memcpy(&b, &h, 2);
    return b;
#endif
    uint32_t x;
    __builtin_memcpy(&x, &f, 4);
    const uint32_t sign = (x >> 16) & 0x8000u;
    x &= 0x7fffffffu;
    if (x >= 0x7f800000u)
        return (uint16_t)(sign | (x > 0x7f800000u ? 0x7e00u : 0x7c00u));
    if (x >= 0x477ff000u)
        return (uint16_t)(sign | 0x7c00u);
    if (x < 0x38800000u) {
        float af;
        __builtin_memcpy(&af, &x, 4);
        const float scaled = af * 16777216.0f;
        const float r = (scaled + 8388608.0f) - 8388608.0f;
        return (uint16_t)(sign | (uint32_t)r);
    }
    x += 0x0fffu + ((x >> 13) & 1u);
    return (uint16_t)(sign | ((x - 0x38000000u) >> 13));
}
PL_HD float pf_half_to_float(uint16_t h) {
#if defined(__HIP_DEVICE_COMPILE__)
    _Float16 v;
    __builtin_memcpy(&v, &h, 2);
    return (float)v;
#endif
    const uint32_t sign = (uint32_t)(h & 0x8000u) << 16;
    const uint32_t e = (h >> 10) & 31u, m = h & 1023u;
    uint32_t x;
    if (e == 0) {
        const float v = (float)m * 5.9604644775390625e-08f;
        __builtin_memcpy(&x, &v, 4);
        x |= sign;
    } else if (e == 31) {
        x = sign | 0x7f800000u | (m << 13);
    } else {
        x = sign | ((e + 112u) << 23) | (m << 13);
    }
    float f;
    __builtin_memcpy(&f, &x, 4);
    return f;
}
PL_HD uint16_t pf_half_up(float v) {
    uint16_t b = pf_half_rn(v);
    if (b < 0x7c00u && pf_half_to_float(b) < v)
        b = (uint16_t)(b + 1);
    return b;
}
PL_HD void pf_split16(double v, uint16_t &hi, uint16_t &lo) {
    hi = pf_half_rn((float)v);
    lo = pf_half_rn((float)(v - (double)pf_half_to_float(hi)));
}

struct Sampson16Operand {
    uint16_t c[32];
    uint16_t s[16];
};
constexpr double kS16PointMax = 8.0;

PL_HD void pf16_sampson_model(const double *F, bool nan_model, Sampson16Operand &o) {
    for (int k = 0; k < 32; ++k)
        o.c[k] = 0;
    for (int k = 0; k < 16; ++k)
        o.s[k] = 0;
    double fm = 0.0;
    bool bad = nan_model;
    for (int k = 0; k < 9; ++k) {
        const double a = fabs(F[k]);
// ... 283 lines not shown
```

Measured before the change: 1.221 billion hypotheses/s.

## Add float lower-bound scoring pass to prune hypotheses before exact MFMA scoring

Adds a bound-scoring stage to the pruned absolute-pose scoring path. It computes conservative float lower bounds on per-hypothesis inlier count and MSAC score from shadow models, then drops hypotheses that provably cannot beat the lead before the exact f64 MFMA scoring kernel runs. The aim is to cut exact-scoring work on losing hypotheses. In exchange it adds four extra kernel launches per scoring round, including a single-workgroup compaction kernel, and its correctness rests on the bounds staying rigorous.

```diff
diff --git a/__graft_entry__.py b/__graft_entry__.py
--- a/__graft_entry__.py
+++ b/__graft_entry__.py
@@ -17,6 +17,7 @@
     subprocess.check_call(["make", "-C", os.path.join(ROOT, "tests", "hostmath_trig"), "-s", "libhostmath_trig.so"])
     subprocess.check_call(["make", "-C", os.path.join(ROOT, "tests", "hostmath_tangent"), "-s", "libhostmath_tangent.so"])
     subprocess.check_call(["make", "-C", os.path.join(ROOT, "tests", "hostmath_radial1d"), "-s", "libhostmath_radial1d.so"])
+    subprocess.check_call(["make", "-C", os.path.join(ROOT, "tests", "hostmath_bound"), "-s", "libhostmath_bound.so"])
     if os.path.isdir("/root/reference/PoseLib"):
         subprocess.check_call(["make", "-C", os.path.join(ROOT, "oracle"), "-s", "-j8", "-f", "Makefile.ref"])
         subprocess.check_call(["make", "-C", os.path.join(ROOT, "oracle"), "-s", "-j8", "-f", "Makefile.ref", "VARIANT=fma"])
diff --git a/include/poselib_amd.h b/include/poselib_amd.h
--- a/include/poselib_amd.h
+++ b/include/poselib_amd.h
@@ -258,6 +258,8 @@
 int pl_debug_score_pruned(int route, pl_debug_prune_member *members, size_t num_members, uint32_t *idle_changed);
 int pl_debug_score_survivors(int route, pl_debug_prune_member *members, size_t num_members, uint32_t *const *survivors,
                              uint32_t *idle_changed, uint32_t *guard_changed);
+int pl_debug_score_bounded(int route, pl_debug_prune_member *members, size_t num_members, uint32_t *const *bound_counts,
+                           double *const *bound_scores, uint8_t *const *tiers, uint32_t *idle_changed, uint32_t *guard_changed);
 int pl_debug_score_prune_gate(int kind, uint32_t n_points, uint32_t iterations);
 typedef struct pl_debug_sampler_shape_info {
     uint64_t window;
diff --git a/poselib_amd/__init__.py b/poselib_amd/__init__.py
--- a/poselib_amd/__init__.py
+++ b/poselib_amd/__init__.py
@@ -4,7 +4,7 @@
     device_count, essential_matrix_5pt, estimate_absolute_pose, estimate_batch, last_batch_report, estimate_fundamental, estimate_homography,
     estimate_relative_pose, homography_4pt, p3p, p5p, ransac_fundamental, ransac_homography, ransac_pnp, ransac_pnpf,
     ransac_relpose, ransac_shared_focal_relpose, estimate_shared_focal_relative_pose, refine_shared_focal_relpose, ImagePair, p35pf, relpose_6pt_shared_focal, solve_focal_batch, relpose_5pt, relpose_7pt, set_device, set_lm_mode, solve_batch, undistort_points,
-    check_device_points, point_stats_dev, point_stats_group_dev, score_pruned, score_survivors, score_prune_gate, sampler_shape, sample_positions,
+    check_device_points, point_stats_dev, point_stats_group_dev, score_pruned, score_survivors, score_bounded, score_prune_gate, sampler_shape, sample_positions,
 )
 
 __version__ = "0.1.0"
diff --git a/poselib_amd/_lib.py b/poselib_amd/_lib.py
--- a/poselib_amd/_lib.py
+++ b/poselib_amd/_lib.py
@@ -209,6 +209,8 @@
         "pl_debug_score_stream_ex": (cint, [cint, P(DebugScoreMember), sz, P(C.c_uint32)]),
         "pl_debug_score_pruned": (cint, [cint, P(DebugPruneMember), sz, P(C.c_uint32)]),
         "pl_debug_score_survivors": (cint, [cint, P(DebugPruneMember), sz, P(C.c_void_p), P(C.c_uint32), P(C.c_uint32)]),
+        "pl_debug_score_bounded": (cint, [cint, P(DebugPruneMember), sz, P(C.c_void_p), P(C.c_void_p), P(C.c_void_p), P(C.c_uint32),
+                                           P(C.c_uint32)]),
         "pl_debug_score_prune_gate": (cint, [cint, C.c_uint32, C.c_uint32]),
         "pl_debug_sampler_shape": (cint, [cint, u64, C.c_uint32, u64, P(DebugSamplerShape)]),
         "pl_debug_sample_positions": (cint, [cint, cint, cint, P(DebugSamplerMember), sz, P(C.c_uint32)]),
@@ -252,6 +254,7 @@
     "pl_abi_version", "pl_problem_create_tangent", "pl_debug_inlier_mask", "pl_debug_tangent_chunk",
     "pl_p5lp_radial", "pl_debug_radial1d_chunk", "pl_debug_radial1d_generate", "pl_debug_group_slices", "pl_debug_generate",
     "pl_debug_score_shape", "pl_debug_score_stream_ex", "pl_debug_score_pruned", "pl_debug_score_survivors", "pl_debug_score_prune_gate",
+    "pl_debug_score_bounded",
     "pl_estimate_absolute_pose_dev", "pl_estimate_relative_pose_dev", "pl_estimate_fundamental_dev", "pl_estimate_homography_dev",
     "pl_problem_create_dev", "pl_problem_create_tangent_dev", "pl_debug_check_device_points", "pl_debug_point_stats_dev",
     "pl_debug_sampler_shape", "pl_debug_sample_positions", "pl_estimate_batch_dev", "pl_debug_point_stats_group_dev",
diff --git a/poselib_amd/api.py b/poselib_amd/api.py
--- a/poselib_amd/api.py
+++ b/poselib_amd/api.py
@@ -638,6 +638,37 @@
     return out, idle.value, guard.value
 
 
+def score_bounded(members, route=0):
+    arr = (L.DebugPruneMember * max(len(members), 1))()
+    bcs, bss, trs = ((C.c_void_p * max(len(members), 1))() for _ in range(3))
+    keep = []
+    cap = 4096
+    for i, (problem, models, max_error, init_max, init_min) in enumerate(members):
+        n, flat = problem._flat_models(models)
+        cnt = np.zeros(max(n, 1), dtype=np.uint32)
+        sc = np.zeros(max(n, 1), dtype=np.float64)
+        kp = np.zeros(max(n, 1), dtype=np.uint8)
+        cand = np.zeros(cap, dtype=np.uint32)
+        bc = np.zeros(max(n, 1), dtype=np.uint32)
+        bs = np.zeros(max(n, 1), dtype=np.float64)
+        tr = np.zeros(max(n, 1), dtype=np.uint8)
+        keep.append((n, flat, cnt, sc, kp, cand, bc, bs, tr))
+        arr[i] = L.DebugPruneMember(problem._h, _ptr(flat), n, float(max_error), float(init_min), int(init_max), cap, _ptr(cnt),
+                                    _ptr(sc), _ptr(kp), _ptr(cand))
+        bcs[i], bss[i], trs[i] = bc.ctypes.data, bs.ctypes.data, tr.ctypes.data
+    idle, guard = C.c_uint32(0), C.c_uint32(0)
+    L.check(L.lib().pl_debug_score_bounded(int(route), arr, C.c_size_t(len(members)), bcs, bss, trs, C.byref(idle), C.byref(guard)))
+    out = []
+    for i, (n, _, cnt, sc, kp, cand, bc, bs, tr) in enumerate(keep):
+        a = arr[i]
+        out.append({"counts": cnt[:n], "scores": sc[:n], "kept": kp[:n].astype(bool), "cand": cand[:min(a.num_cand, cap)].copy(),
+                    "num_cand": a.num_cand, "cstar": a.cstar, "chunks": a.chunks, "chunk_points": a.chunk_points, "lead": a.lead,
+                    "lead_max": a.lead_max, "lead_min": a.lead_min, "num_live": a.num_live, "num_selected": a.num_selected,
+                    "num_preselected": a.num_preselected, "slices": a.slices, "bound_counts": bc[:n], "bound_scores": bs[:n],
+                    "tiers": tr[:n]})
+    return out, idle.value, guard.value
+
+
 def ransac_batch(problems, opts, max_in_flight=4, group_size=16):
     b = RansacBatch(problems, opts)
     b.run(max_in_flight, group_size)
diff --git a/poselib_amd/csrc/driver.cc b/poselib_amd/csrc/driver.cc
--- a/poselib_amd/csrc/driver.cc
+++ b/poselib_amd/csrc/driver.cc
@@ -618,6 +618,7 @@
         pa.chunk_points = s.point_rows / s.chunks;
         pa.init_max = r.init_max, pa.init_min = r.init_min;
         pa.lead = kPruneLead;
+        pa.bound = 1;
     }
     RecordsArgs &ra = a.rec;
     ra.f.num_hyp = &b.ctl->num_hyp;
@@ -2612,8 +2613,13 @@
     }
     return PL_OK;
 }
+struct DebugBoundedOut {
+    uint32_t *const *bound_counts;
+    double *const *bound_scores;
+    uint8_t *const *tiers;
+};
 int debug_score_pruned(int route, pl_debug_prune_member *m, size_t count, uint32_t *idle_changed, uint32_t *const *survivors = nullptr,
-                       uint32_t *guard_changed = nullptr) {
+                       uint32_t *guard_changed = nullptr, const DebugBoundedOut *bounded = nullptr) {
     if (route != 0 && route != 2)
         return fail(PL_ERR_INVALID, "route: 0 single launch, 2 group form");
     if (!m || count == 0 || count > (route == 0 ? 1 : kDebugScoreMembers))
@@ -2651,7 +2657,7 @@
             if (p)
                 (void)hipFree(p);
         }
-    } dtable;
+    } dtable, dbound[kDebugScoreMembers];
     GroupArgs ha[1 + kDebugScoreMembers];
     GroupDims dims{};
     dims.G = (uint32_t)count + 1;
@@ -2692,6 +2698,14 @@
         t.b.nan_bits = nullptr;
         t.b.host_meta = nullptr, t.b.host_models = nullptr, t.b.host_ctl = nullptr;
         wire_batch_step(ha[k], t.run, t.s, t.b);
+        ha[k].score.prune.bound = bounded ? 1u : 0u;
+        if (bounded && k > 0) {
+            const size_t hcap = ha[k].score.hyp_capacity;
+            HIP_TRY(hipMalloc(&dbound[k - 1].p, hcap * 16));
+            HIP_TRY(hipMemsetAsync(dbound[k - 1].p, 0xff, hcap * 16, c->stream));
+            ha[k].score.prune.bnd_score = static_cast<double *>(dbound[k - 1].p);
+            ha[k].score.prune.bnd_count = reinterpret_cast<uint32_t *>(ha[k].score.prune.bnd_score + hcap);
+        }
     }
     ha[0].active = 0;
     for (size_t i = 0; i < count; ++i) {
@@ -2704,6 +2718,7 @@
         dims.max_chunks = std::max(dims.max_chunks, a.chunks);
         dims.max_slices = std::max(dims.max_slices, a.slices);
         dims.any_mfma = dims.any_prune = 1;
+        dims.any_bound = bounded ? 1u : 0u;
         std::vector<double> recs;
         std::vector<uint32_t> ident(H);
         for (uint32_t k = 0; k < H; ++k)
@@ -2724,7 +2739,8 @@
             HIP_TRY(launch_score_count(a.score, slices, c->stream));
         } else {
             HIP_TRY(launch_score_pruned(a.score, slices, c->stream));
-            HIP_TRY(launch_prune_label(a.score, c->stream));
+            if (!bounded)
+                HIP_TRY(launch_prune_label(a.score, c->stream));
             HIP_TRY(launch_finalize_records(a.rec, c->stream));
         }
     } else {
@@ -2735,7 +2751,7 @@
             HIP_TRY(launch_group_score_count(static_cast<const GroupArgs *>(dtable.p), dims, c->stream));
         } else {
             HIP_TRY(launch_group_score(EST_ABS, static_cast<const GroupArgs *>(dtable.p), dims, c->stream));
-            for (size_t i = 0; i < count; ++i)
+            for (size_t i = 0; i < count && !bounded; ++i)
                 HIP_TRY(launch_prune_label(ha[i + 1].score, c->stream));
             HIP_TRY(launch_group_finalize_records(static_cast<const GroupArgs *>(dtable.p), dims, c->stream));
         }
@@ -2746,9 +2762,17 @@
     std::vector<std::vector<RecordMeta>> meta(count);
     std::vector<PruneState> st(count);
     std::vector<BatchCtl> ctl(count);
+    std::vector<std::vector<uint32_t>> bcount(count);
+    std::vector<std::vector<double>> bscore(count);
     for (size_t i = 0; i < count; ++i) {
         const Slot &t = slot[i + 1];
         const uint32_t H = t.s.Bl;
+        if (bounded) {
+            const size_t hcap = ha[i + 1].score.hyp_capacity;
+            bcount[i].resize(hcap), bscore[i].resize(hcap);
+            HIP_TRY(hipMemcpyAsync(bcount[i].data(), ha[i + 1].score.prune.bnd_count, 4 * hcap, hipMemcpyDeviceToHost, c->stream));
+            HIP_TRY(hipMemcpyAsync(bscore[i].data(), ha[i + 1].score.prune.bnd_score, 8 * hcap, hipMemcpyDeviceToHost, c->stream));
+        }
         if (m[i].counts && !survivors)
             HIP_TRY(hipMemcpyAsync(m[i].counts, t.b.count, sizeof(uint32_t) * H, hipMemcpyDeviceToHost, c->stream));
         if (m[i].scores && !survivors)
@@ -2759,7 +2783,7 @@
         HIP_TRY(hipMemcpyAsync(meta[i].data(), t.b.rec_meta, sizeof(RecordMeta) * kRecordCap, hipMemcpyDeviceToHost, c->stream));
         HIP_TRY(hipMemcpyAsync(&st[i], t.b.prune_state, sizeof(PruneState), hipMemcpyDeviceToHost, c->stream));
         HIP_TRY(hipMemcpyAsync(&ctl[i], t.b.ctl, sizeof(BatchCtl), hipMemcpyDeviceToHost, c->stream));
-        if (survivors) {
+        if (survivors || bounded) {
             part[i].resize((size_t)t.s.chunks * ha[i + 1].score.hyp_capacity);
             HIP_TRY(hipMemcpyAsync(part[i].data(), t.b.part_count, sizeof(uint32_t) * part[i].size(), hipMemcpyDeviceToHost, c->stream));
         }
@@ -2790,6 +2814,20 @@
             }
             continue;
         }
+        if (bounded) {
+            const uint32_t hcap = ha[i + 1].score.hyp_capacity;
+            for (uint32_t ch = 0; ch < chunks; ++ch)
+                for (uint32_t p = ctl[i].num_live; p < hcap; ++p)
+                    guard += part[i][(size_t)ch * hcap + p] != 0xffffffffu ? 1u : 0u;
+            for (uint32_t k = 0; k < H; ++k) {
+                const uint32_t p = rank[i][k];
+                const bool live = p != kNoRank;
+                const bool has = live && bcount[i][p] != 0xffffffffu;
+                bounded->bound_counts[i][k] = has ? bcount[i][p] : 0xffffffffu;
+                bounded->bound_scores[i][k] = has ? bscore[i][p] : std::numeric_limits<double>::quiet_NaN();
+                bounded->tiers[i][k] = !live ? 3 : kept[i][p] == kKept ? 0 : has ? 2 : 1;
+            }
+        }
         const bool split = st[i].cstar < chunks;
         uint32_t selected = 0;
         for (uint32_t k = 0; k < H; ++k) {
@@ -2831,6 +2869,20 @@
         if (!survivors[i])
             return fail(PL_ERR_INVALID, "pl_debug_score_survivors: a member without an output array");
     return debug_score_pruned(route, members, num_members, idle_changed, survivors, guard_changed);
+}
+int pl_debug_score_bounded(int route, pl_debug_prune_member *members, size_t num_members, uint32_t *const *bound_counts,
+                           double *const *bound_scores, uint8_t *const *tiers, uint32_t *idle_changed, uint32_t *guard_changed) {
+    if (idle_changed)
+        *idle_changed = 0;
+    if (guard_changed)
+        *guard_changed = 0;
+    if (!bound_counts || !bound_scores || !tiers)
+        return fail(PL_ERR_INVALID, "pl_debug_score_bounded: output arrays missing");
+    for (size_t i = 0; i < num_members; ++i)
+        if (!bound_counts[i] || !bound_scores[i] || !tiers[i])
+            return fail(PL_ERR_INVALID, "pl_debug_score_bounded: a member without an output array");
+    const DebugBoundedOut out{bound_counts, bound_scores, tiers};
+    return debug_score_pruned(route, members, num_members, idle_changed, nullptr, guard_changed, &out);
 }
 int pl_debug_score_prune_gate(int kind, uint32_t n_points, uint32_t iterations) {
     PrefilterArgs pf{};
diff --git a/poselib_amd/csrc/driver_group.inc b/poselib_amd/csrc/driver_group.inc
--- a/poselib_amd/csrc/driver_group.inc
+++ b/poselib_amd/csrc/driver_group.inc
@@ -755,6 +755,7 @@
             dims.any_mfma |= a.use_mfma;
             dims.any_queue |= a.use_mfma ? 0u : 1u;
             dims.any_prune |= a.score.prune.st ? 1u : 0u;
+            dims.any_bound |= (a.score.prune.st && a.score.prune.bound) ? 1u : 0u;
             ++nactive;
         }
         if (nactive == 0)
diff --git a/poselib_amd/csrc/kernels.hip b/poselib_amd/csrc/kernels.hip
--- a/poselib_amd/csrc/kernels.hip
+++ b/poselib_amd/csrc/kernels.hip
@@ -1622,6 +1622,173 @@
     if (!g.active || !g.use_mfma || !g.score.prune.st)
         return;
     prune_list_body(globalised(g.score));
+}
+
+constexpr int kBoundThreads = 256;
+template <int P, bool RESID>
+__device__ __forceinline__ void score_bound_body(const ScoreArgs &a, uint32_t slice, uint32_t chunk, uint32_t nslices) {
+    constexpr int kWaves = kBoundThreads / 64;
+    constexpr uint32_t NPW = 64u * P;
+    const PruneArgs &pr = a.prune;
+    if (!pr.st || !pr.bound || *as_uniform(&pr.st->cstar) >= pr.chunks)
+        return;
+    const uint32_t first = RESID ? 0u : min(*as_uniform(a.num_hyp), pr.lead), len = *as_uniform(&pr.st->sel_len);
+    if (len <= first)
+        return;
+    const int lane = threadIdx.x & 63;
+    const int wave = __builtin_amdgcn_readfirstlane((int)(threadIdx.x >> 6));
+    const PrefilterArgs pf = a.pf;
+    float x[P], y[P], X[P], Y[P], Z[P], fw[P];
+    bool valid[P];
+    uint64_t vmask[P];
+#pragma unroll
+    for (int p = 0; p < P; ++p) {
+        const uint32_t i = chunk * NPW + (uint32_t)p * 64u + (uint32_t)lane;
+        valid[p] = i < a.pts.n;
+        vmask[p] = __builtin_amdgcn_ballot_w64(valid[p]);
+        const uint32_t ic = valid[p] ? i : 0u;
+        const double Xd = a.pts.a[2][ic], Yd = a.pts.a[3][ic], Zd = a.pts.a[4][ic];
+        x[p] = (float)a.pts.a[0][ic], y[p] = (float)a.pts.a[1][ic];
+        X[p] = (float)Xd, Y[p] = (float)Yd, Z[p] = (float)Zd;
+        fw[p] = pf_point_abs(Xd, Yd, Zd, pf.gx);
+    }
+    const uint32_t nent = len - first;
+    for (uint32_t u = slice * kWaves + (uint32_t)wave; u * 64u < nent; u += nslices * kWaves) {
+        const uint32_t e = first + u * 64u + (uint32_t)lane;
+        const uint32_t pos = pr.sel[min(e, len - 1u)];
+        const float4 *sh = reinterpret_cast<const float4 *>(a.models + (size_t)a.slots[pos] * kModelStride + kShadowOff);
+        float4 rv[4];
+#pragma unroll
+        for (int k = 0; k < 4; ++k)
+            rv[k] = sh[k];
+        const uint32_t n = min(64u, nent - u * 64u);
+        uint32_t my_c = 0, my_q = 0;
+        for (uint32_t j = 0; j < n; ++j) {
+            float r[16];
+#pragma unroll
+            for (int k = 0; k < 4; ++k) {
+                r[4 * k + 0] = __builtin_bit_cast(float, __builtin_amdgcn_readlane(__builtin_bit_cast(int, rv[k].x), (int)j));
+                r[4 * k + 1] = __builtin_bit_cast(float, __builtin_amdgcn_readlane(__builtin_bit_cast(int, rv[k].y), (int)j));
+                r[4 * k + 2] = __builtin_bit_cast(float, __builtin_amdgcn_readlane(__builtin_bit_cast(int, rv[k].z), (int)j));
+                r[4 * k + 3] = __builtin_bit_cast(float, __builtin_amdgcn_readlane(__builtin_bit_cast(int, rv[k].w), (int)j));
+            }
+            const float gt = pf_abs_bound_slack(r, pf.gx);
+            uint32_t c = 0, q = 0;
+            if constexpr (RESID) {
+#pragma unroll
+                for (int p = 0; p < P; ++p) {
+                    const float L = pf_abs_r2_lower(r, gt, x[p], y[p], X[p], Y[p], Z[p], fw[p]);
+                    c += (uint32_t)__popcll(__builtin_amdgcn_ballot_w64(valid[p] && L < pf.thr2_up));
+                    q += valid[p] ? pf_bound_quantum(L, pf.inv_thr2_dn) : 0u;
+                }
+                q = (uint32_t)__builtin_amdgcn_readlane((int)wave_scan_u32(q), 63);
+            } else {
+#pragma unroll
+                for (int p = 0; p + 1 < P; p += 2) {
+                    const v2f Xp = {X[p], X[p + 1]}, Yp = {Y[p], Y[p + 1]}, Zp = {Z[p], Z[p + 1]};
+                    const v2f xp = {x[p], x[p + 1]}, yp = {y[p], y[p + 1]}, w = {fw[p], fw[p + 1]};
+                    const v2f z0 = pk_fma(bc(r[0]), Xp, pk_fma(bc(r[1]), Yp, pk_fma(bc(r[2]), Zp, bc(r[9]))));
+                    const v2f z1 = pk_fma(bc(r[3]), Xp, pk_fma(bc(r[4]), Yp, pk_fma(bc(r[5]), Zp, bc(r[10]))));
+                    const v2f z2 = pk_fma(bc(r[6]), Xp, pk_fma(bc(r[7]), Yp, pk_fma(bc(r[8]), Zp, bc(r[11]))));
+                    const v2f a0 = pk_fma(-xp, z2, z0);
+                    const v2f a1 = pk_fma(-yp, z2, z1);
+                    const v2f W = w + bc(gt);
+                    const v2f B = pk_fma(bc(pf.thr), z2, W);
+#pragma unroll
+                    for (int e2 = 0; e2 < 2; ++e2) {
+                        const uint64_t out = vmask[p + e2] & (__builtin_amdgcn_ballot_w64(fmaxf(fabsf(a0[e2]), fabsf(a1[e2])) > B[e2]) |
+                                                              __builtin_amdgcn_ballot_w64(z2[e2] < -W[e2]));
+                        q += (uint32_t)__popcll(out);
+                        c += (uint32_t)__popcll(vmask[p + e2] & ~out);
+                    }
+                }
+                if constexpr (P & 1) {
+                    constexpr int p = P - 1;
+                    const uint64_t out = vmask[p] & __builtin_amdgcn_ballot_w64(pf_abs_outlier(r, gt, pf.thr, x[p], y[p], X[p], Y[p], Z[p], fw[p]));
+                    q += (uint32_t)__popcll(out);
+                    c += (uint32_t)__popcll(vmask[p] & ~out);
+                }
+                q <<= 20;
+            }
+            if ((uint32_t)lane == j)
+                my_c = c, my_q = q;
+        }
+        if ((uint32_t)lane < n) {
+            const size_t o = (size_t)chunk * a.hyp_capacity + pos;
+            a.part_count[o] = my_c;
+            a.part_score[o] = (double)my_q;
+        }
+    }
+}
+template <int P, bool RESID> __global__ __launch_bounds__(kBoundThreads) void k_score_bound(ScoreArgs a) {
+    uint32_t slice, chunk;
+    slice_chunk_of_workgroup(gridDim.x, gridDim.y, slice, chunk);
+    score_bound_body<P, RESID>(a, slice, chunk, gridDim.x);
+}
+template <bool RESID> __global__ __launch_bounds__(kBoundThreads) void k_score_bound_g(const GroupArgs *ga) {
+    const GroupArgs &g = ga[blockIdx.z];
+    uint32_t slice, chunk;
+    const uint32_t ns = pruned_slices<kScoreSel>(g.slices);
+    if (!g.active || !g.use_mfma || !g.score.prune.st || !slice_chunk_of_workgroup(ns, g.chunks, slice, chunk))
+        return;
+    score_bound_body<5, RESID>(globalised(g.score), slice, chunk, ns);
+}
+__device__ __forceinline__ void prune_bound_body(const ScoreArgs &a, int stage) {
+    __shared__ uint32_t wt[16];
+    const PruneArgs &pr = a.prune;
+    if (!pr.bound || pr.st->cstar >= pr.chunks)
+        return;
+    const uint32_t first = stage ? 0u : min(*a.num_hyp, pr.lead), len = pr.st->sel_len;
+    const uint32_t lead_max = pr.st->lead_max;
+    const double beat = pr.st->lead_min * (1.0 + kPruneScoreMargin);
+    const int lane = threadIdx.x & 63, wave = threadIdx.x >> 6;
+    uint32_t base = 0;
+    __syncthreads();
+    for (uint32_t t0 = first; t0 < len; t0 += 1024u) {
+        const uint32_t e = t0 + threadIdx.x;
+        uint32_t keep = 0, p = 0;
+        if (e < len) {
+            p = pr.sel[e];
+            uint32_t c = 0;
+            uint64_t q = 0;
+#pragma unroll 8
+            for (uint32_t ch = 0; ch < pr.chunks; ++ch) {
+                c += a.part_count[(size_t)ch * a.hyp_capacity + p];
+                q += (uint64_t)a.part_score[(size_t)ch * a.hyp_capacity + p];
+            }
+            const double qd = (double)q * 9.5367431640625e-07;
+            double s_lb = a.thr2 * qd;
+            if (fma(a.thr2, qd, -s_lb) < 0.0)
+                s_lb = __longlong_as_double(__double_as_longlong(s_lb) - 1);
+            keep = (c <= lead_max && s_lb > beat) ? 0u : 1u;
+            if (!keep)
+                pr.kept[p] = kDropped;
+            if (pr.bnd_count)
+                pr.bnd_count[p] = c, pr.bnd_score[p] = s_lb;
+        }
+        const uint32_t inc = wave_scan_u32(keep);
+        if (lane == 63)
+            wt[wave] = inc;
+        __syncthreads();
+        uint32_t at = base + inc - keep, tot = 0;
+        for (int w = 0; w < 16; ++w) {
+            at += w < wave ? wt[w] : 0u;
+            tot += wt[w];
+        }
+        if (keep)
+            pr.sel[at] = p;
+        base += tot;
+        __syncthreads();
+    }
+    if (threadIdx.x == 0)
+        pr.st->sel_len = base;
+}
+__global__ __launch_bounds__(1024) void k_prune_bound(ScoreArgs a, int stage) { prune_bound_body(a, stage); }
+__global__ __launch_bounds__(1024) void k_prune_bound_g(const GroupArgs *ga, int stage) {
+    const GroupArgs &g = ga[blockIdx.z];
+    if (!g.active || !g.use_mfma || !g.score.prune.st)
+        return;
+    prune_bound_body(globalised(g.score), stage);
 }
 
 
@@ -3721,6 +3888,12 @@
     e = launch_prune_select(a, stream);
     if (e != hipSuccess)
         return e;
+    if (a.prune.bound) {
+        k_score_bound<PG / 2, false><<<sel_grid, dim3(kBoundThreads), 0, stream>>>(a);
+        k_prune_bound<<<dim3(1), dim3(1024), 0, stream>>>(a, 0);
+        k_score_bound<PG / 2, true><<<sel_grid, dim3(kBoundThreads), 0, stream>>>(a);
+        k_prune_bound<<<dim3(1), dim3(1024), 0, stream>>>(a, 1);
+    }
     k_score_mfma_pr<PG, kScoreSel><<<sel_grid, block, 0, stream>>>(a);
     return hipGetLastError();
 }
@@ -3936,6 +4109,12 @@
             e = launch_group_prune_select(args, d, stream);
             if (e != hipSuccess)
                 return e;
+            if (d.any_bound) {
+                k_score_bound_g<false><<<sel_grid, dim3(kBoundThreads), 0, stream>>>(args);
+                k_prune_bound_g<<<dim3(1, 1, d.G), dim3(1024), 0, stream>>>(args, 0);
+                k_score_bound_g<true><<<sel_grid, dim3(kBoundThreads), 0, stream>>>(args);
+                k_prune_bound_g<<<dim3(1, 1, d.G), dim3(1024), 0, stream>>>(args, 1);
+            }
             k_score_mfma_pr_g<10, kScoreSel><<<sel_grid, dim3(kMfmaThreads), 0, stream>>>(args);
         } else if (d.any_mfma)
             k_score_mfma_g<10><<<grid, dim3(kMfmaThreads), 0, stream>>>(args);
diff --git a/poselib_amd/csrc/pl_global.h b/poselib_amd/csrc/pl_global.h
--- a/poselib_amd/csrc/pl_global.h
+++ b/poselib_amd/csrc/pl_global.h
@@ -70,6 +70,8 @@
     a.prune.blk_kept = as_global(a.prune.blk_kept);
     a.prune.sel = as_global(a.prune.sel);
     a.prune.kept = as_global(a.prune.kept);
+    a.prune.bnd_count = as_global(a.prune.bnd_count);
+    a.prune.bnd_score = as_global(a.prune.bnd_score);
     return a;
 }
 __device__ __forceinline__ FinalizeArgs globalised(FinalizeArgs f) {
diff --git a/poselib_amd/csrc/pl_kernels.h b/poselib_amd/csrc/pl_kernels.h
--- a/poselib_amd/csrc/pl_kernels.h
+++ b/poselib_amd/csrc/pl_kernels.h
@@ -62,6 +62,9 @@
     uint32_t chunks = 0, chunk_points = 0;
     uint32_t init_max = 0, lead = 0;
     double init_min = 0.0;
+    uint32_t bound = 0, pad = 0;
+    uint32_t *bnd_count = nullptr;
+    double *bnd_score = nullptr;
 };
 constexpr uint8_t kDropped = 0, kKept = 1, kPrunedExact = 2;
 
@@ -339,6 +342,7 @@
     uint32_t max_chunks, max_slices;
     uint32_t any_mfma, any_queue;
     uint32_t any_prune;
+    uint32_t any_bound;
     int P;
 };
 hipError_t launch_group_batch(int est, const GroupArgs *args, const GroupDims &dims, hipStream_t stream,
diff --git a/poselib_amd/csrc/pl_prefilter.h b/poselib_amd/csrc/pl_prefilter.h
--- a/poselib_amd/csrc/pl_prefilter.h
+++ b/poselib_amd/csrc/pl_prefilter.h
@@ -18,13 +18,14 @@
     float w252;
     float t16;
     float h16;
+    float inv_thr2_dn;
 };
 
 PL_HD float pf_up(float v) { return v * 1.000001f + 1e-30f; }
 
 inline PrefilterArgs make_prefilter_args(int est, double thr2, float xy_absmax) {
     PrefilterArgs a;
-    a.thr = a.gx = a.thr2_up = a.g16 = a.c16 = a.t1 = a.w252 = a.t16 = a.h16 = 0.f;
+    a.thr = a.gx = a.thr2_up = a.g16 = a.c16 = a.t1 = a.w252 = a.t16 = a.h16 = a.inv_thr2_dn = 0.f;
     a.enabled = 0;
     if (!(thr2 >= 1e-30 && thr2 <= 1e30))
         return a;
@@ -39,6 +40,7 @@
     a.w252 = nextafterf((float)((16.0 / 15.0) * (1.0 + 96.0 * u) * 60.0), inf);
     if (est == 0) {
         a.gx = nextafterf((float)(32.0 * u * (1.0 + (double)xy_absmax + thr)), inf);
+        a.inv_thr2_dn = nextafterf((float)((1.0 / thr2) * (1.0 - 8.0 * u)), 0.f);
         a.g16 = nextafterf((float)(4.8828125e-4 * 1.015625), inf);
         a.c16 = nextafterf((float)((2e-7 + 5.0e-4) * (1.0 + 1.3661 * (double)xy_absmax + thr)), inf);
     }
@@ -80,6 +82,43 @@
     const float W = fw + gt;
     const float B = fmaf(thr, z2, W);
     return (fmaxf(fabsf(a0), fabsf(a1)) > B) | (z2 < -W);
+}
+
+constexpr float kPfBoundDown = 0.9999847412109375f;
+constexpr float kPfBoundScale = 1048576.f;
+constexpr float kPfFltMin = 1.17549435e-38f;
+PL_HD float pf_rcp(float v) {
+#if defined(__HIP_DEVICE_COMPILE__)
+    return __builtin_amdgcn_rcpf(v);
+#else
+    return 1.f / v;
+#endif
+}
+PL_HD float pf_abs_bound_slack(const float *r, float gx) {
+    const bool covered = (r[13] == 0.f) & (r[14] <= 1.0001f);
+    return covered ? pf_up(gx * r[12]) : __builtin_huge_valf();
+}
+PL_HD float pf_abs_r2_lower(const float *r, float gt, float x, float y, float X, float Y, float Z, float fw) {
+    const float z0 = fmaf(r[0], X, fmaf(r[1], Y, fmaf(r[2], Z, r[9])));
+    const float z1 = fmaf(r[3], X, fmaf(r[4], Y, fmaf(r[5], Z, r[10])));
+    const float z2 = fmaf(r[6], X, fmaf(r[7], Y, fmaf(r[8], Z, r[11])));
+    const float a0 = fmaf(-x, z2, z0);
+    const float a1 = fmaf(-y, z2, z1);
+    const float W = fw + gt;
+    const float n0 = fmaxf(fabsf(a0) - W, 0.f), n1 = fmaxf(fabsf(a1) - W, 0.f);
+    const float d = z2 + W;
+    const float num = fmaf(n1, n1, n0 * n0), dd = d * d;
+    const float L = (num * pf_rcp(dd)) * kPfBoundDown;
+    if (z2 < -W)
+        return __builtin_huge_valf();
+    const bool known = (z2 > W) & (L < __builtin_huge_valf()) & (num >= kPfFltMin) & (dd >= kPfFltMin);
+    return known ? L : 0.f;
+}
+PL_HD float pf_abs_verdict_lower(const float *r, float gt, float thr, float x, float y, float X, float Y, float Z, float fw) {
+    return pf_abs_outlier(r, gt, thr, x, y, X, Y, Z, fw) ? __builtin_huge_valf() : 0.f;
+}
+PL_HD uint32_t pf_bound_quantum(float L, float inv_thr2_dn) {
+    return (uint32_t)(fminf(L * inv_thr2_dn, 1.f) * kPfBoundScale);
 }
 
 PL_HD bool pf_hom_outlier(const float *r, float gh , float thr, float a0, float a1, float b0, float b1,
```

Result: faster. 1.265 billion hypotheses/s (median of 6 runs) (+3.6%).
